# rasd3/TODA

Hardware: AMD Instinct MI355X
Metric: LiDAR training samples/sec (higher is better)
Workload: dtype f32

## Files before the change

include/toda.h:

```cpp
#ifndef TODA_H_
#define TODA_H_

#include <stddef.h>
#include <stdint.h>

#ifdef __cplusplus
extern "C" {
#endif

#define TODA_OK 0
#define TODA_EINVAL (-1)
#define TODA_EWORKSPACE (-2)
#define TODA_ELAUNCH (-3)
#define TODA_EFAULT (-4)

#define TODA_FAULT_BN2D 1u
#define TODA_FAULT_WINO 2u
#define TODA_FAULT_FPS 4u

const char* toda_last_error(void);
int toda_abi_version(void);
int toda_device_fault(void);

size_t toda_voxelize_workspace_bytes(int n_points, int max_voxels);
int toda_voxelize_hard(const float* points, int n, int c,
                       const float* range_host ,
                       const float* vsize_host ,
                       const int32_t* grid_host ,
                       int max_pts, int max_voxels,
                       float* voxels, int32_t* coords_zyx, int32_t* num_pts,
                       int32_t* m_dev, void* ws, size_t ws_bytes, void* stream);
size_t toda_voxelize_batch_workspace_bytes(int batch, int n_cap);
int toda_voxelize_batch(const float* const* points_host, const int32_t* n_points_host, int batch, int n_cap,
                        int c, int row_stride,
                        const float* range_host, const float* vsize_host, const int32_t* grid_host,
                        int max_pts, int max_voxels,
                        float* voxels, int32_t* coords_bzyx, int32_t* num_pts, int32_t* counts_dev,
                        void* ws, size_t ws_bytes, int ws_clean, void* stream);

int toda_mean_vfe_fwd(const float* voxels, const float* num_pts, int m, int p, int c,
                      float* out, void* stream);
int toda_mean_vfe_bwd(const float* grad_out, const float* num_pts, int m, int p, int c,
                      float* grad_voxels, void* stream);

size_t toda_dynvox_workspace_bytes(int n, int batch, const int32_t* grid_host, int pillar);
int toda_dynvox_count(const float* points, int n, int width, int batch, const float* range_host, const float* vsize_host,
                      const int32_t* grid_host, int pillar, int32_t* counts_dev, void* ws, size_t ws_bytes, void* stream);
int toda_dynvox_index(const float* points, int n, int width, int batch, const float* range_host, const float* vsize_host,
                      const int32_t* grid_host, int pillar, int m, int k, uint8_t* keep, int32_t* rows, int32_t* inv,
                      int32_t* seg_pts, int32_t* seg_off, int32_t* cnt, int32_t* coords, void* ws, size_t ws_bytes,
                      void* stream);
int toda_dynvox_seg_sum(const float* src, int ld, int col0, int ncol, const int32_t* rowmap, const int32_t* seg_off,
                        const int32_t* seg_pts, int m, int divide, float* out, void* stream);
int toda_dynvox_pillar_decorate(const float* points, int width, const int32_t* rows, const int32_t* inv,
                                const int32_t* coords, const float* mean, int k, const float* vsize_host,
                                const float* offset_host, int use_abs_xyz, int with_dist, float* out, int f, void* stream);
int toda_dynvox_seg_max_fwd(const float* x, int c, const int32_t* seg_off, const int32_t* seg_pts, int m, float* out,
                            int32_t* arg, void* stream);
int toda_dynvox_seg_max_bwd(const float* gout, const int32_t* arg, int m, int c, int k, float* gx, void* stream);
int toda_dynvox_gather_concat(const float* x, const float* xmax, const int32_t* inv, int k, int c, float* out, void* stream);

size_t toda_gridindex_bytes(int batch, const int32_t* shape_host );
int toda_gridindex_from_coords(const int32_t* idx, int n, const int32_t* n_dev,
                               int batch, const int32_t* shape_host,
                               void* gi, int32_t* rowof, void* stream);
int toda_gridindex_from_coords_unordered(const int32_t* idx, int n, const int32_t* n_dev,
                                         int batch, const int32_t* shape_host,
                                         void* gi, int32_t* rowof, int gi_clean, void* stream);
int toda_gridindex_clear(const int32_t* idx, int n, const int32_t* n_dev, int batch,
                         const int32_t* shape_host, void* gi, void* stream);
int toda_gridindex_from_conv(const int32_t* idx_in, int n_in, const int32_t* n_in_dev,
                             int batch, const int32_t* shape_in_host,
                             const int32_t* ksize_host, const int32_t* stride_host,
                             const int32_t* pad_host, const int32_t* shape_out_host,
                             void* gi_out, int32_t* idx_out, int32_t* n_out_dev,
                             int out_cap, void* stream);
int toda_gridindex_from_bitmap(const void* gi_in, int batch, const int32_t* shape_in_host,
                               const int32_t* ksize_host, const int32_t* stride_host,
                               const int32_t* pad_host, const int32_t* shape_out_host,
                               void* gi_out, int32_t* idx_out, int32_t* n_out_dev,
                               int out_cap, int in_rows_marked, void* stream);

int toda_rulebook_subm(const int32_t* idx, int n, int batch, const int32_t* shape_host,
                       const int32_t* ksize_host, const int32_t* dilation_host,
                       const void* gi, const int32_t* rowof,
                       int32_t* nbr, int32_t* pair_cnt, int cnt_zeroed, void* stream);
int toda_rulebook_conv(const int32_t* idx_in, int n_in, int batch,
                       const int32_t* shape_in_host, const int32_t* ksize_host,
                       const int32_t* stride_host, const int32_t* pad_host,
                       const int32_t* shape_out_host, const void* gi_out, int n_out,
                       int32_t* nbr_o2i, int32_t* nbr_i2o, int32_t* pair_cnt,
                       const int32_t* idx_out, const void* gi_in, const int32_t* rowof_in,
                       int cnt_zeroed, void* stream);

size_t toda_spconv_packed_weight_floats(int k_vol, int c_gather, int c_produce);
int toda_matrix_path(void);
int toda_set_matrix_path(int mode);
int toda_spconv_split_supported(int c_gather, int c_produce);
int toda_spconv_pack_weight(const float* w, int cout, int k_vol, int cin,
                            int transpose, int flip_k, float* wp, void* stream);
int toda_spconv_pack_weights(int n, const float* const* w_host, const int32_t* cout_host, const int32_t* k_vol_host,
                             const int32_t* cin_host, const int32_t* transpose_host, const int32_t* flip_k_host,
                             float* const* wp_host, void* stream);
int toda_spconv_gather_gemm(const float* in, int n_in, int c_gather, const float* wp,
                            const int32_t* nbr, int n_out, int k_vol, int c_produce,
                            const float* bias , float* out, void* stream);
int toda_spconv_gather_gemm_ordered(const float* in, int n_in, int c_gather, const float* wp,
                                    const int32_t* nbr, int n_out, int k_vol, int c_produce,
                                    const float* bias, float* out, const int32_t* order, void* stream);

int toda_rulebook_class_order(const int32_t* in_coords, int n_in, const int32_t* stride_host, const int32_t* padding_host,
                              int32_t* order, unsigned char* cls_sorted, void* stream);
int toda_spconv_gather_gemm_classed(const float* in, int n_in, int c_gather, const float* wp, const int32_t* nbr, int n_out,
                                    int k_vol, int c_produce, const float* bias, float* out, const int32_t* order,
                                    const unsigned char* cls_sorted, const int32_t* ksize_host, const int32_t* stride_host,
                                    const int32_t* padding_host, void* stream);
int toda_spconv_gather_gemm_compact_supported(int c_gather, int c_produce, int k_vol);
int toda_spconv_gather_gemm_compact(const float* in, int n_in, int c_gather, const float* w, int w_cout, int w_cin,
                                    int transpose, int flip_k, const int32_t* nbr, int n_out, int k_vol, int c_produce,
                                    const float* bias , float* out, void* stream);
size_t toda_spconv_gather_gemm_compact_stats_doubles(int n_out, int c_produce);
int toda_spconv_gather_gemm_compact_stats(const float* in, int n_in, int c_gather, const float* w, int w_cout, int w_cin,
                                          int transpose, int flip_k, const int32_t* nbr, int n_out, int k_vol,
                                          int c_produce, const float* bias , float* out, double* sums,
                                          size_t sums_doubles, int* blocks_out , void* stream);

size_t toda_spconv_wgrad_workspace_bytes(int n_out, int k_vol, int cin, int cout);
int toda_spconv_wgrad(const float* in, int n_in, const float* dout, const int32_t* nbr,
                      int n_out, int k_vol, int cin, int cout, float* dw,
                      void* ws, size_t ws_bytes, void* stream);
int toda_sparse_to_dense_fwd(const float* feat, const int32_t* idx, int n, int c,
                             int batch, const int32_t* shape_host, float* dense, void* stream);
int toda_sparse_to_dense_bwd(const float* grad_dense, const int32_t* idx, int n, int c,
                             int batch, const int32_t* shape_host, float* grad_feat, void* stream);

int toda_pillar_scatter_fwd(const float* feat, const int32_t* idx, int n, int c,
                            int batch, int ny, int nx, float* canvas, void* stream);
int toda_pillar_scatter_bwd(const float* grad_canvas, const int32_t* idx, int n, int c,
                            int batch, int ny, int nx, float* grad_feat, void* stream);

size_t toda_rows_reduce_doubles(int n, int c);
int toda_rows_moments(const float* x, int n, int c, double* sums ,
                      void* stream);
int toda_rows_affine_act(const float* x, const float* scale, const float* shift,
                         const float* residual , int n, int c, int relu,
                         float* y, void* stream);

int toda_bn_finalize(const double* sums , int n, int c,
                     const float* gamma, const float* beta, float* running_mean ,
                     float* running_var , float momentum, float eps, int training,
                     float* mean, float* invstd, float* scale, float* shift, void* stream);
int toda_bn_finalize_partials(double* sums, int blocks, int n, int c, const float* gamma, const float* beta,
                              float* running_mean , float* running_var , float momentum, float eps,
                              float* mean, float* invstd, float* scale, float* shift, void* stream);
int toda_rows_bn_bwd(const float* dy, const float* x, const float* stats, const float* gamma,
                     int n, int c, int relu, double* sums , float* dx,
                     void* stream);

int toda_rows_bn_bwd_res(const float* dy, const float* x, const float* residual , const float* stats,
                         const float* gamma, int n, int c, int relu, double* sums, float* dx,
                         float* dres , void* stream);
size_t toda_rows_bn_bwd_colsum_doubles(int n, int c);
int toda_rows_bn_bwd_res_colsum(const float* dy, const float* x, const float* residual , const float* stats,
                                const float* gamma, int n, int c, int relu, double* sums, float* dx,
                                float* dres , double* colsum_ws , float* dx_colsum ,
                                void* stream);

int toda_bn2d_supported(int batch, int c, int hw);
size_t toda_bn2d_sync_bytes(void);
int toda_bn2d_fwd(const float* x, int batch, int c, int hw, const float* gamma, const float* beta,
                  float* running_mean , float* running_var , float momentum, float eps, int relu,
                  float* y, float* save, void* sync , unsigned epoch, void* stream);
int toda_bn2d_bwd(const float* x, const float* dy, int batch, int c, int hw, const float* gamma, const float* beta,
                  const float* save, int relu, float* dx, float* dgamma, float* dbeta, void* sync ,
                  unsigned epoch, void* stream);
int toda_bn2d_fwd_into(const float* x, int batch, int c, int hw, const float* gamma, const float* beta,
                       float* running_mean , float* running_var , float momentum, float eps, int relu,
                       float* y, int y_channels, int y_channel0, float* save, void* sync , unsigned epoch,
                       void* stream);
int toda_bn2d_bwd_from(const float* x, const float* dy, int dy_channels, int dy_channel0, int batch, int c, int hw,
                       const float* gamma, const float* beta, const float* save, int relu, float* dx, float* dgamma,
                       float* dbeta, void* sync , unsigned epoch, void* stream);

int toda_center_assign(const float* gt_boxes, int batch, int n_gt, int code_size,
                       int num_classes, int fm_w, int fm_h,
                       const float* range_host , const float* vsize_host ,
                       int fm_stride, int max_objs, double gaussian_overlap, int min_radius,
                       float* heatmap ,
                       float* ret_boxes ,
                       int64_t* inds , int64_t* mask ,
                       void* stream);

size_t toda_anchor_assign_workspace_bytes(int batch, int n_gt);
int toda_anchor_assign(const void* const* anchors_host, const int32_t* locs_host, const int32_t* per_loc_host,
                       const float* matched_host, const float* unmatched_host, int n_classes, int anchor_stride,
                       const float* gt_boxes, int batch, int n_gt, int gt_stride, const int32_t* slot_of, int n_ids,
                       int code_size, int encode_angle_by_sincos, int multihead_order,
                       int32_t* labels , float* targets , float* weights ,
                       void* ws, size_t ws_bytes, void* stream);

int toda_boxes_iou_bev(const float* boxes_a, int na, const float* boxes_b, int nb,
                       float* iou , void* stream);
int toda_boxes_overlap_bev(const float* boxes_a, int na, const float* boxes_b, int nb,
                           float* overlap , void* stream);
size_t toda_nms_workspace_bytes(int n);
int toda_nms_rotated(const float* boxes_sorted, int n, float thresh, int64_t* keep ,
                     int32_t* n_keep_dev, void* ws, size_t ws_bytes, void* stream);

int toda_roi_grid_pool_bev(const float* feat, int B, int C, int H, int W, const float* rois, int N, int roi_stride,
                           float min_x, float min_y, float step_x, float step_y, int grid_size, float* out, void* stream);
int toda_roi_iou3d_max(const float* rois, int B, int N, int roi_stride, const int64_t* roi_labels, const float* gt, int M,
                       int gt_stride, int by_class, float* max_iou , int64_t* argmax , void* stream);

int toda_voxel_query(const float* new_xyz, const int32_t* new_coords, int M, const float* xyz, int N, const void* gi, const int32_t* rowof,
                     int batch, const int32_t* shape_host, float radius, const int32_t* ranges_host, int nsample, int32_t* idx,
                     uint8_t* empty, void* stream);
size_t toda_voxel_pool_moments_doubles(void);
int toda_voxel_pool_moments(const int32_t* idx, const uint8_t* empty, int M, int nsample, const float* xyz, int N, const float* new_xyz,
                            double* ws, void* stream);
int toda_voxel_pool_fwd(const float* f, int N, int C, const int32_t* idx, const uint8_t* empty, int M, int nsample, const float* xyz,
                        const float* new_xyz, const float* ab, float* out, uint8_t* arg, void* stream);
size_t toda_voxel_pool_table_bytes(int M, int nsample, int N);
int toda_voxel_pool_table(const int32_t* idx, const uint8_t* empty, int M, int nsample, int N, int32_t* off, int32_t* ent, void* ws,
                          size_t ws_bytes, void* stream);
int toda_voxel_pool_bwd_feat(const float* gout, const uint8_t* arg, int M, int nsample, int C, const int32_t* off, const int32_t* ent,
                             int N, float* gf, void* stream);
size_t toda_voxel_pool_bwd_pos_doubles(int C);
int toda_voxel_pool_bwd_pos(const float* gout, const uint8_t* arg, const int32_t* idx, const uint8_t* empty, int M, int nsample, int C,
                            const float* xyz, int N, const float* new_xyz, double* ws, float* gab, void* stream);

int toda_fps_resident_blocks(void);
size_t toda_fps_workspace_bytes(int batch, int npoint);
int toda_fps(const float* xyz, const int32_t* starts_host, int batch, int npoint, int mode, float* temp, int32_t* idx, void* ws,
             size_t ws_bytes, void* stream);
int toda_ball_query_stack(const float* xyz, int N, const int32_t* xyz_start, const float* new_xyz, const int32_t* new_start, int batch,
                          int M, int nr, const float* radii_host, const int32_t* nsample_host, int32_t* const* idx_host,
                          uint8_t* const* empty_host, void* stream);
int toda_sa_gather_fwd(const float* P, int N, int C, const float* wd, const int32_t* idx, const uint8_t* empty, int M, int nsample,
                       const float* xyz, const float* new_xyz, float* z, void* stream);
int toda_sa_gather_bwd_feat(const float* gz, int M, int nsample, int C, const int32_t* off, const int32_t* ent, int N, float* gP,
                            void* stream);
size_t toda_sa_gather_bwd_pos_doubles(int C);
int toda_sa_gather_bwd_pos(const float* gz, const int32_t* idx, const uint8_t* empty, int M, int nsample, int C, const float* xyz, int N,
                           const float* new_xyz, double* ws, float* gwd, void* stream);
int toda_sa_max_fwd(const float* y, int M, int nsample, int C, float* out, uint8_t* arg, void* stream);
int toda_sa_max_bwd(const float* g, const uint8_t* arg, int M, int nsample, int C, float* gy, void* stream);
int toda_bev_interp_fwd(const float* map, int B, int C, int H, int W, const float* xy, const int32_t* bidx, int K, float* out,
                        int32_t* taps, float* wts, void* stream);
int toda_bev_interp_bwd(const float* g, int K, int C, const int32_t* off, const int32_t* ent, const float* wts, int B, int H, int W,
                        float* gmap, void* stream);

int toda_points_in_boxes(const float* points, int n, const int32_t* n_dev, int c, const float* boxes,
                         int k, int box_stride, int mode, int32_t* flags, void* stream);
int toda_points_sector(const float* points, int n, const int32_t* n_dev, int c, double lo, double hi,
                       int32_t* flags, void* stream);
int toda_points_rect(const float* points, int n, const int32_t* n_dev, int c, const double* lo_xy_host,
                     const double* hi_xy_host, int closed, int32_t* flags, void* stream);
int toda_points_polar_cell(const float* points, int n, const int32_t* n_dev, int c, float phase,
                           const double* yaw_edges_host, int n_yaw, const double* dis_edges_host, int n_dis,
                           float dis_lo, float dis_hi, int32_t* cell, void* stream);
int toda_points_polar_select(const float* points, int n, const int32_t* n_dev, int c, double lo, double hi, int yaw_mode,
                             int dis_mode, double dis_th, const float* pitch_range_dev, int32_t* flags, void* stream);
size_t toda_points_pitch_range_workspace_bytes(void);
int toda_points_pitch_range(const float* points, int n, const int32_t* n_dev, int c, float* range_dev, void* ws,
                            size_t ws_bytes, void* stream);
int toda_points_pitch_band(const float* points, int n, const int32_t* n_dev, int c, float z_offset, float clip_lo,
                           float clip_hi, const double* edges_host, int n_bands, int32_t* band, void* stream);
size_t toda_rows_select_workspace_bytes(int n);
int toda_rows_select_append(const float* src, int n, const int32_t* n_dev, int c, const int32_t* keys,
                            int match, int invert, float* dst, int cap_rows, int32_t* cursor_dev,
                            void* ws, size_t ws_bytes, void* stream);
int toda_points_rotate_z(const float* src, int n, const int32_t* n_dev, int c, double cosv, double sinv,
                         float* dst, void* stream);
int toda_points_world_transform(const float* src, int n, const int32_t* n_dev, int c, int flip_x, int flip_y,
                                int rotate, float cosv, float sinv, int rescale, float scale, float* dst,
                                void* stream);

int toda_points_box_steps_chunk(void);
int toda_points_box_steps(const float* src, int n, const int32_t* n_dev, int c, const double* steps, int n_steps,
                          float* dst, int32_t* keep, void* stream);
size_t toda_points_column_range_workspace_bytes(void);
int toda_points_column_range(const float* points, int n, const int32_t* n_dev, int c, int col, float* range_dev,
                             void* ws, size_t ws_bytes, void* stream);
int toda_points_in_pyramids(const float* points, int n, const int32_t* n_dev, int c, const double* pyramids, int np,
                            uint32_t* bits, int32_t* counts, void* stream);

int toda_points_fov_flags(const float* points, int n, const int32_t* n_dev, int c, const float* m_host,
                          const float* p2_host, int img_h, int img_w, int32_t* flags, void* stream);

int toda_sweeps_merge_max_sweeps(void);
int toda_sweeps_merge(const float* rows, int n, int n_sweeps, const int32_t* offsets_host, const double* matrices_host,
                      const int32_t* has_matrix_host, const int32_t* drop_ego_host, const double* time_lags_host,
                      float radius, const float* shift_host, float* out, int32_t* flags, void* stream);

int toda_waymo_frame(const float* rows, int n, int c_in, int use_nlz, float* out, int32_t* flags, void* stream);

int toda_adv_edit_max_boxes(void);
int toda_adv_edit_chunk(void);
size_t toda_adv_edit_workspace_bytes(int n, int k);
int toda_adv_edit(const float* points, int n, int c, const double* table_host, const double* table_dev, int k,
                  const int64_t* keys, const float* grads, int m, const float* range_lo_host, const float* voxel_host,
                  const int32_t* grid_host, float eps, float* dst, int cap_rows, int32_t* cursor_dev, int32_t* counts,
                  void* ws, size_t ws_bytes, void* stream);

int toda_spconv_gather_gemm_stats_supported(int c_gather, int c_produce);
size_t toda_spconv_gather_gemm_stats_doubles(int n_out, int c_produce);
int toda_spconv_gather_gemm_stats(const float* in, int n_in, int c_gather, const float* packed_w, const int32_t* nbr,
                                  int n_out, int k_vol, int c_produce, const float* bias, float* out, double* sums,
                                  size_t sums_doubles, void* stream);
int toda_spconv_gather_gemm_stats_partials(const float* in, int n_in, int c_gather, const float* wp, const int32_t* nbr,
                                           int n_out, int k_vol, int c_produce, const float* bias , float* out,
                                           double* sums, size_t sums_doubles, int* blocks_out, void* stream);

int toda_conv3x3_supported(int batch, int cin, int cout, int H, int W);
size_t toda_conv3x3_weight_floats(int cout, int cin);
int toda_conv3x3_transform_weight(const float* w, int cout, int cin, int mode, float* u, void* stream);
typedef struct toda_conv3x3_weight_entry {
    const float* w;
    int32_t cout, cin, mode, reserved;
    float* u;
} toda_conv3x3_weight_entry;
int toda_conv3x3_transform_weight_batch(const toda_conv3x3_weight_entry* table_host, int n, void* stream);
size_t toda_conv3x3_workspace_bytes(void);
size_t toda_conv3x3_wgrad_workspace_bytes(int batch, int cin, int cout, int H, int W);
int toda_conv3x3_wgrad(const float* x, const float* dy, int batch, int cin, int cout, int H, int W, float* dw,
                       void* ws, size_t ws_bytes, void* stream);
int toda_conv3x3_fwd(const float* x, const float* u, const float* bias, int batch, int cin, int cout, int H,
                     int W, float* y, void* ws, size_t ws_bytes, void* stream);

int toda_conv3x3s2_supported(int batch, int cin, int cout, int H, int W);
int toda_conv3x3s2_fwd(const float* x, const float* w, int batch, int cin, int cout, int H, int W, float* y, void* stream);
int toda_conv3x3s2_dgrad(const float* dy, const float* w, int batch, int cin, int cout, int H, int W, float* dx, void* stream);
size_t toda_conv3x3s2_wgrad_workspace_bytes(int batch, int cin, int cout, int H, int W);
int toda_conv3x3s2_wgrad(const float* x, const float* dy, int batch, int cin, int cout, int H, int W, float* dw, void* ws,
                         size_t ws_bytes, void* stream);
int toda_deconv_supported(int batch, int cin, int cout, int H, int W, int s);
int toda_deconv_fwd(const float* x, const float* w, int batch, int cin, int cout, int H, int W, int s, float* y, void* stream);
int toda_deconv_dgrad(const float* dy, const float* w, int batch, int cin, int cout, int H, int W, int s, float* dx, void* stream);
size_t toda_deconv_wgrad_workspace_bytes(int batch, int cin, int cout, int H, int W, int s);
int toda_deconv_wgrad(const float* x, const float* dy, int batch, int cin, int cout, int H, int W, int s, float* dw, void* ws,
                      size_t ws_bytes, void* stream);

size_t toda_center_loss_workspace_bytes(int batch, int classes, int H, int W, int max_objs, int code_size);
int toda_center_loss_fwd(const float* hm_logits, const float* heatmap, int batch, int classes, int H, int W, int n_branch,
                         const float* const* reg_maps_host, const int32_t* reg_channels_host, const int64_t* inds,
                         const int64_t* mask, const float* target_boxes, int max_objs, int code_size,
                         const float* code_weights_host, float cls_weight, float loc_weight, float* hm_prob, float* out4,
                         void* ws, size_t ws_bytes, void* stream);
int toda_center_loss_bwd(const float* out4, const float* up_hm, const float* up_loc, int batch, int classes, int H, int W,
                         int n_branch, float* const* reg_grads_host, const int32_t* reg_channels_host, const int64_t* inds,
                         const int64_t* mask, int max_objs, int code_size, const float* code_weights_host, float cls_weight, float loc_weight,
                         float* hm_grad, const void* ws, size_t ws_bytes, void* stream);

int toda_conv3x3_narrow_supported(int batch, int cin, int cout, int H, int W);
int toda_conv3x3_narrow_fwd(int n, const float* const* x_host, const float* const* w_host, const float* const* bias_host,
                            const int32_t* cout_host, int batch, int cin, int H, int W, long long x_image_stride,
                            float* const* y_host, void* stream);
int toda_conv3x3_narrow_dgrad(int n, const float* const* dy_host, const float* const* w_host, const int32_t* cout_host,
                              int batch, int cin, int H, int W, long long dx_image_stride, float* const* dx_host, void* stream);
size_t toda_conv3x3_narrow_wgrad_workspace_bytes(int n, int batch, int cin, int H);
int toda_conv3x3_narrow_wgrad(int n, const float* const* x_host, const float* const* dy_host, const int32_t* cout_host,
                              int batch, int cin, int H, int W, long long x_image_stride, float* out, void* ws, size_t ws_bytes,
                              void* stream);

int toda_timing_begin(int capacity);
int toda_timing_end(float* ms_out_host, int cap, int* n_out_host);

int toda_clip_adam_chunk(void);
int toda_clip_adam_step(const unsigned long long* param, const unsigned long long* grad, const unsigned long long* exp_avg,
                        const unsigned long long* exp_avg_sq, const long long* numel, const int* chunk_tensor,
                        const long long* chunk_off, int n_chunks, double* partial, float* norm_out, float max_norm,
                        float lr, float beta1, float beta2, float eps, float weight_decay, int step, void* stream);

int toda_eval_overlaps(const float* box3d, const float* bbox, const int32_t* box_off, const float* query3d,
                       const float* query_bbox, const int32_t* query_off, const long long* out_off, int n_frames,
                       long long n_pairs, int metric, int criterion, float* out, void* stream);
size_t toda_eval_match_workspace_bytes(int n_frames, int n_thresh, int n_det_total);
int toda_eval_match_scores(const float* overlaps, const long long* ov_off, const int32_t* det_off, const int32_t* gt_off,
                           const int32_t* ign_det, const int32_t* ign_gt, const double* det_score, int n_frames,
                           int n_det_total, double min_overlap, double* scores_out, int32_t* count_out, void* ws,
                           size_t ws_bytes, void* stream);
int toda_eval_match(const float* overlaps, const long long* ov_off, const int32_t* det_off, const int32_t* gt_off,
                    const int32_t* ign_det, const int32_t* ign_gt, const double* det_score, const double* det_alpha,
                    const double* gt_alpha, const double* det_bbox, const double* dc_bbox, const int32_t* dc_off, int n_frames,
                    int n_det_total, const double* thresholds, int n_thresh, double min_overlap, int metric, int compute_aos,
                    double* pr, void* ws, size_t ws_bytes, void* stream);

#define TODA_NUSC_MAX_PRED 500
#define TODA_NUSC_MAX_GT 2048
int toda_nusc_eval_prepare(const double* rows, const int32_t* sample, const int32_t* cls, int n, const double* G,
                           const double* ego, int n_samples, double* out, int32_t* keep, void* stream);
size_t toda_nusc_eval_match_workspace_bytes(int n_seg);
int toda_nusc_eval_match(const double* pred, const double* pred_score, const int32_t* pred_attr, int n_pred, const double* gt,
                         const int32_t* gt_attr, int n_gt, const int32_t* pred_off_host, const int32_t* gt_off_host,
                         const int32_t* seg_cls_host, int n_seg, const double* thresholds_host, int tp_threshold,
                         int32_t* match, double* err, void* ws, size_t ws_bytes, void* stream);

#define TODA_WAYMO_MAX_PRED 512
#define TODA_WAYMO_MAX_GT 512
#define TODA_WAYMO_CUTOFFS 101
size_t toda_waymo_eval_match_workspace_bytes(int n_seg);
int toda_waymo_eval_iou(const double* pred, int n_pred, const double* gt, int n_gt, const int32_t* pred_off_host,
                        const int32_t* gt_off_host, const long long* iou_off_host, int n_seg, long long n_pairs, double* iou,
                        void* ws, size_t ws_bytes, void* stream);
int toda_waymo_eval_match(const double* iou, const float* pred_score, const double* pred_heading, int n_pred,
                          const double* gt_heading, const int32_t* gt_level, int n_gt, const int32_t* pred_off_host,
                          const int32_t* gt_off_host, const long long* iou_off_host, const int32_t* seg_type_host, int n_seg,
                          long long n_pairs, const float* cutoffs_host, long long* tp, long long* fn, long long* fp,
                          double* sum_ha, int32_t* match_dbg, void* ws, size_t ws_bytes, void* stream);

size_t toda_consistency_workspace_bytes(int batch, int na, int no);
int toda_consistency_loss(const float* adv, const uint8_t* adv_sel, int na, const float* org, const uint8_t* org_sel, int no,
                          int batch, int cols, float match_dist2, float* out, void* ws, size_t ws_bytes, void* stream);

#ifdef __cplusplus
}
#endif
#endif
```

toda_amd/csrc/bn_fold.cuh:

```cuda
#pragma once
#include "common.h"

namespace toda {

constexpr int DN_BLOCK = 256;

__device__ __forceinline__ double fold_column(const double* __restrict__ src, int blocks, double* part) {
    double acc = 0.0;
    for (int g = threadIdx.x; g < blocks; g += DN_BLOCK) acc += src[g];
    part[threadIdx.x] = acc;
    __syncthreads();
    for (int w = DN_BLOCK / 2; w > 0; w >>= 1) {
        if (threadIdx.x < w) part[threadIdx.x] += part[threadIdx.x + w];
        __syncthreads();
    }
    return part[0];
}

__device__ __forceinline__ void bn_write_channel(int ch, float mean, float var, float eps, const float* __restrict__ gamma,
                                                 const float* __restrict__ beta, float* __restrict__ mean_out,
                                                 float* __restrict__ invstd_out, float* __restrict__ scale_out,
                                                 float* __restrict__ shift_out) {
    const float invstd = 1.0f / sqrtf(var + eps);
    const float g = gamma ? gamma[ch] : 1.0f, b = beta ? beta[ch] : 0.0f;
    mean_out[ch] = mean;
    invstd_out[ch] = invstd;
    scale_out[ch] = g * invstd;
    shift_out[ch] = b - mean * g * invstd;
}

__device__ __forceinline__ void bn_train_channel(int ch, double sum, double sumsq, int n, const float* __restrict__ gamma,
                                                 const float* __restrict__ beta, float* __restrict__ running_mean,
                                                 float* __restrict__ running_var, float momentum, float eps,
                                                 float* __restrict__ mean_out, float* __restrict__ invstd_out,
                                                 float* __restrict__ scale_out, float* __restrict__ shift_out) {
    const double m = sum / (double)n;
    double v = sumsq / (double)n - m * m;
    if (v < 0.0) v = 0.0;
    const float mean = (float)m, var = (float)v;
    if (running_mean) {
        const double unbiased = n > 1 ? v * (double)n / (double)(n - 1) : v;
        running_mean[ch] = (1.0f - momentum) * running_mean[ch] + momentum * mean;
        running_var[ch] = (1.0f - momentum) * running_var[ch] + momentum * (float)unbiased;
    }
    bn_write_channel(ch, mean, var, eps, gamma, beta, mean_out, invstd_out, scale_out, shift_out);
}

__global__ void __launch_bounds__(DN_BLOCK) fold_partials_kernel(double* __restrict__ sums, int blocks, int cols);

}
```

toda_amd/csrc/dense.hip:

```cpp
#include "bn_fold.cuh"
#include "common.h"

namespace toda {

typedef float f32x4 __attribute__((ext_vector_type(4)));

constexpr int DN_ROWS = 64;
constexpr int DN_CH = 32;

struct DenseGeom {
    int D, H, W;
    int pillar;
};

__device__ __forceinline__ long long spatial_offset(const int4 q, const DenseGeom& g) {
    if (g.pillar) return (long long)q.y + (long long)q.z * g.W + q.w;
    return ((long long)q.y * g.H + q.z) * g.W + q.w;
}

template <bool FWD>
__global__ void __launch_bounds__(DN_BLOCK)
dense_tile_kernel(float* __restrict__ feat, const int4* __restrict__ idx, int n, int c, DenseGeom g,
                  float* __restrict__ dense) {
    __shared__ float tile[DN_CH][DN_ROWS + 1];
// ... 5 lines not shown
        long long b = -1;
        if (r < n) {
            const int4 q = idx[r];
            b = (long long)q.x * c * vol + spatial_offset(q, g);
        }
        base[threadIdx.x] = b;
    }
    const int fr = threadIdx.x >> 2, fc = (threadIdx.x & 3) * 8;
    const int dr = threadIdx.x & 63, dc = threadIdx.x >> 6;
    if (FWD) {
        if (row0 + fr < n) {
#pragma unroll
            for (int j = 0; j < 8; ++j) {
                const int ch = c0 + fc + j;
                tile[fc + j][fr] = ch < c ? feat[(size_t)(row0 + fr) * c + ch] : 0.f;
            }
        }
        __syncthreads();
        const long long b = base[dr];
        if (b >= 0) {
#pragma unroll
            for (int j = 0; j < DN_CH / 4; ++j) {
                const int ch = dc + 4 * j;
                if (c0 + ch < c) dense[b + (long long)(c0 + ch) * vol] = tile[ch][dr];
            }
        }
    } else {
        __syncthreads();
        const long long b = base[dr];
#pragma unroll
        for (int j = 0; j < DN_CH / 4; ++j) {
            const int ch = dc + 4 * j;
            tile[ch][dr] = (b >= 0 && c0 + ch < c) ? dense[b + (long long)(c0 + ch) * vol] : 0.f;
        }
        __syncthreads();
        if (row0 + fr < n) {
#pragma unroll
            for (int j = 0; j < 8; ++j) {
                const int ch = c0 + fc + j;
                if (ch < c) feat[(size_t)(row0 + fr) * c + ch] = tile[fc + j][fr];
            }
        }
    }
}

#ifndef TODA_MOM_ROWS
#define TODA_MOM_ROWS 256
#endif
constexpr int MOM_ROWS = TODA_MOM_ROWS;
constexpr int MOM_MAX_BLOCKS = 2048;

template <class Load>
__device__ __forceinline__ void rows_reduce2(int n, int c, int rows_per_block, Load load, double* __restrict__ sums) {
    __shared__ float sh[2][DN_BLOCK][4];
    const int lanes = c >> 2;
    const int rows_par = DN_BLOCK / lanes;
    const int cl = threadIdx.x % lanes, rsub = threadIdx.x / lanes;
    const int row_begin = blockIdx.x * rows_per_block;
    const int row_end = min(n, row_begin + rows_per_block);
    f32x4 s0 = f32x4{0.f, 0.f, 0.f, 0.f}, t0 = s0, s1 = s0, t1 = s0;
    int r = row_begin + rsub;
    for (; r + rows_par < row_end; r += 2 * rows_par) {
        f32x4 a, b, a2, b2;
        load(r, cl, a, b);
        load(r + rows_par, cl, a2, b2);
        s0 += a;
        t0 += b;
        s1 += a2;
        t1 += b2;
    }
    if (r < row_end) {
        f32x4 a, b;
        load(r, cl, a, b);
        s0 += a;
        t0 += b;
    }
    s0 += s1;
    t0 += t1;
#pragma unroll
    for (int j = 0; j < 4; ++j) {
        sh[0][threadIdx.x][j] = s0[j];
        sh[1][threadIdx.x][j] = t0[j];
    }
    __syncthreads();
    if (threadIdx.x < 2 * c) {
        const int q = threadIdx.x / c, ch = threadIdx.x % c;
        double acc = 0.0;
        for (int j = 0; j < rows_par; ++j) acc += sh[q][j * lanes + (ch >> 2)][ch & 3];
        sums[2 * c + (size_t)(q * c + ch) * gridDim.x + blockIdx.x] = acc;
    }
}

__global__ void __launch_bounds__(DN_BLOCK)
fold_partials_kernel(double* __restrict__ sums, int blocks, int cols) {
    __shared__ double part[DN_BLOCK];
    const double total = fold_column(sums + cols + (size_t)blockIdx.x * blocks, blocks, part);
    if (threadIdx.x == 0) sums[blockIdx.x] = total;
}

static inline void reduce_plan(int n, int* blocks, int* rows_per_block) {
    const int g = cdiv(n > 0 ? n : 1, MOM_ROWS);
    *blocks = g < MOM_MAX_BLOCKS ? g : MOM_MAX_BLOCKS;
    *rows_per_block = cdiv(n > 0 ? n : 1, *blocks);
}

__global__ void __launch_bounds__(DN_BLOCK)
rows_moments_kernel(const float* __restrict__ x, int n, int c, int rows_per_block, double* __restrict__ sums) {
    const f32x4* x4 = reinterpret_cast<const f32x4*>(x);
    const int lanes = c >> 2;
    rows_reduce2(n, c, rows_per_block, [&](int r, int cl, f32x4& a, f32x4& b) {
        a = x4[(size_t)r * lanes + cl];
        b = a * a;
    }, sums);
}

constexpr int EW_BLOCKS = 2048;

__global__ void __launch_bounds__(DN_BLOCK)
rows_affine_act_kernel(const f32x4* __restrict__ x, const float* __restrict__ scale, const float* __restrict__ shift,
                       const f32x4* __restrict__ res, long long n4, int c, int relu, f32x4* __restrict__ y) {
    const long long t0 = (long long)blockIdx.x * DN_BLOCK + threadIdx.x;
    const long long stride = (long long)gridDim.x * DN_BLOCK;
    const int ch = (int)((t0 * 4) % c);
    const f32x4 sc = *reinterpret_cast<const f32x4*>(scale + ch), sf = *reinterpret_cast<const f32x4*>(shift + ch);
    for (long long t = t0; t < n4; t += stride) {
        f32x4 v = x[t] * sc + sf;
        if (res) v += res[t];
        if (relu) {
#pragma unroll
            for (int j = 0; j < 4; ++j) v[j] = fmaxf(v[j], 0.f);
        }
        y[t] = v;
    }
}

__global__ void __launch_bounds__(DN_BLOCK)
rows_bn_bwd_reduce_kernel(const float* __restrict__ dy, const float* __restrict__ x, const float* __restrict__ res,
                          const float* __restrict__ stats, int n, int c, int relu, int rows_per_block,
                          double* __restrict__ sums) {
    const f32x4* dy4 = reinterpret_cast<const f32x4*>(dy);
    const f32x4* x4 = reinterpret_cast<const f32x4*>(x);
    const f32x4* r4 = reinterpret_cast<const f32x4*>(res);
    const int lanes = c >> 2;
    const int cl0 = threadIdx.x % lanes;
    const f32x4 mu = reinterpret_cast<const f32x4*>(stats)[cl0];
    const f32x4 is = reinterpret_cast<const f32x4*>(stats + c)[cl0];
    const f32x4 sc = reinterpret_cast<const f32x4*>(stats + 2 * c)[cl0];
    const f32x4 sf = reinterpret_cast<const f32x4*>(stats + 3 * c)[cl0];
    rows_reduce2(n, c, rows_per_block, [&](int r, int cl, f32x4& a, f32x4& b) {
        const f32x4 g = dy4[(size_t)r * lanes + cl], xv = x4[(size_t)r * lanes + cl];
        const f32x4 rv = r4 ? r4[(size_t)r * lanes + cl] : f32x4{0.f, 0.f, 0.f, 0.f};
#pragma unroll
        for (int j = 0; j < 4; ++j) {
            float pre = xv[j] * sc[j] + sf[j];
            if (r4) pre += rv[j];
            const float dz = (relu && !(pre > 0.f)) ? 0.f : g[j];
            a[j] = dz;
            b[j] = dz * ((xv[j] - mu[j]) * is[j]);
        }
    }, sums);
}

__global__ void __launch_bounds__(DN_BLOCK)
rows_bn_bwd_apply_kernel(const f32x4* __restrict__ dy, const f32x4* __restrict__ x, const f32x4* __restrict__ res,
                         const float* __restrict__ stats, const float* __restrict__ gamma, double* __restrict__ sums,
                         long long n4, int c, int n, int relu, f32x4* __restrict__ dx, f32x4* __restrict__ dres,
                         double* __restrict__ colsum_part) {
    if (blockIdx.x == 0 && threadIdx.x < 2 * c) reinterpret_cast<float*>(sums + 2 * c)[threadIdx.x] = (float)sums[threadIdx.x];
    const long long t0 = (long long)blockIdx.x * DN_BLOCK + threadIdx.x;
    const long long stride = (long long)gridDim.x * DN_BLOCK;
    const int ch = (int)((t0 * 4) % c);
    const float inv_n = 1.0f / (float)n;
    const f32x4 mu = *reinterpret_cast<const f32x4*>(stats + ch);
    const f32x4 is = *reinterpret_cast<const f32x4*>(stats + c + ch);
    const f32x4 sc = *reinterpret_cast<const f32x4*>(stats + 2 * c + ch);
    const f32x4 sf = *reinterpret_cast<const f32x4*>(stats + 3 * c + ch);
    const f32x4 ga = *reinterpret_cast<const f32x4*>(gamma + ch);
    f32x4 m1, m2;
#pragma unroll
    for (int j = 0; j < 4; ++j) {
        m1[j] = (float)(sums[ch + j] * (double)inv_n);
        m2[j] = (float)(sums[c + ch + j] * (double)inv_n);
    }
    const f32x4 k1 = ga * is, k2 = is * m2;
    f32x4 csum = {0.f, 0.f, 0.f, 0.f};
    for (long long t = t0; t < n4; t += stride) {
        const f32x4 g = dy[t], xv = x[t];
        const f32x4 rv = res ? res[t] : f32x4{0.f, 0.f, 0.f, 0.f};
        f32x4 out, dzv;
#pragma unroll
        for (int j = 0; j < 4; ++j) {
            float pre = xv[j] * sc[j] + sf[j];
            if (res) pre += rv[j];
            const float dz = (relu && !(pre > 0.f)) ? 0.f : g[j];
            dzv[j] = dz;
            out[j] = k1[j] * (dz - m1[j] - (xv[j] - mu[j]) * k2[j]);
        }
        dx[t] = out;
        csum += out;
        if (dres) dres[t] = dzv;
    }
    if (colsum_part) {
        __shared__ float cs[DN_BLOCK][4];
#pragma unroll
        for (int j = 0; j < 4; ++j) cs[threadIdx.x][j] = csum[j];
        __syncthreads();
        if (threadIdx.x < c) {
            const int lanes = c >> 2, cl = threadIdx.x >> 2, j = threadIdx.x & 3;
            double acc = 0.0;
            for (int t = cl; t < DN_BLOCK; t += lanes) acc += (double)cs[t][j];
            colsum_part[(size_t)threadIdx.x * gridDim.x + blockIdx.x] = acc;
        }
    }
}

__global__ void __launch_bounds__(DN_BLOCK)
colsum_fold_kernel(const double* __restrict__ part, int blocks, float* __restrict__ out) {
    __shared__ double sh[DN_BLOCK];
    const double total = fold_column(part + (size_t)blockIdx.x * blocks, blocks, sh);
    if (threadIdx.x == 0) out[blockIdx.x] = (float)total;
}

__global__ void __launch_bounds__(DN_BLOCK)
bn_finalize_kernel(const double* __restrict__ sums, int n, int c, const float* __restrict__ gamma,
                   const float* __restrict__ beta, float* __restrict__ running_mean, float* __restrict__ running_var,
                   float momentum, float eps, int training, float* __restrict__ mean_out, float* __restrict__ invstd_out,
                   float* __restrict__ scale_out, float* __restrict__ shift_out) {
    const int ch = threadIdx.x;
    if (ch >= c) return;
    if (training)
        bn_train_channel(ch, sums[ch], sums[c + ch], n, gamma, beta, running_mean, running_var, momentum, eps, mean_out, invstd_out,
                         scale_out, shift_out);
    else
        bn_write_channel(ch, running_mean[ch], running_var[ch], eps, gamma, beta, mean_out, invstd_out, scale_out, shift_out);
}

__global__ void __launch_bounds__(DN_BLOCK)
bn_fold_finalize_kernel(double* __restrict__ sums, int blocks, int n, int c, const float* __restrict__ gamma,
                        const float* __restrict__ beta, float* __restrict__ running_mean, float* __restrict__ running_var,
                        float momentum, float eps, float* __restrict__ mean_out, float* __restrict__ invstd_out,
                        float* __restrict__ scale_out, float* __restrict__ shift_out) {
    __shared__ double part[DN_BLOCK];
    const int ch = blockIdx.x;
    const double sum = fold_column(sums + 2 * c + (size_t)ch * blocks, blocks, part);
    __syncthreads();
    const double sumsq = fold_column(sums + 2 * c + (size_t)(c + ch) * blocks, blocks, part);
    if (threadIdx.x != 0) return;
    sums[ch] = sum;
    sums[c + ch] = sumsq;
    bn_train_channel(ch, sum, sumsq, n, gamma, beta, running_mean, running_var, momentum, eps, mean_out, invstd_out, scale_out,
                     shift_out);
}

static int ew_grid(long long n4, int c) {
    long long blocks = (n4 + DN_BLOCK - 1) / DN_BLOCK;
    if (blocks > EW_BLOCKS) blocks = EW_BLOCKS;
    while ((blocks * DN_BLOCK * 4) % c != 0) ++blocks;
    return (int)blocks;
}

static int scatter_common(bool fwd, float* feat, const int32_t* idx, int n, int c, int batch, DenseGeom g,
                          float* dense, hipStream_t s) {
    TODA_CHECK_ARG(n >= 0 && c >= 1 && batch >= 1, "sparse<->dense: bad sizes n=%d c=%d batch=%d", n, c, batch);
    const size_t total = (size_t)batch * c * g.D * g.H * g.W;
    if (fwd) TODA_HIP(hipMemsetAsync(dense, 0, total * sizeof(float), s));
    if (n == 0) return TODA_OK;
    const dim3 grid(cdiv(n, DN_ROWS), cdiv(c, DN_CH));
    if (fwd)
        hipLaunchKernelGGL(HIP_KERNEL_NAME(dense_tile_kernel<true>), grid, dim3(DN_BLOCK), 0, s, feat, (const int4*)idx, n,
                           c, g, dense);
    else
        hipLaunchKernelGGL(HIP_KERNEL_NAME(dense_tile_kernel<false>), grid, dim3(DN_BLOCK), 0, s, feat, (const int4*)idx, n,
                           c, g, dense);
    TODA_LAUNCH_CHECK();
    return TODA_OK;
}

}

using namespace toda;

extern "C" int toda_sparse_to_dense_fwd(const float* feat, const int32_t* idx, int n, int c, int batch,
                                        const int32_t* shape_host, float* dense, void* stream) {
    const DenseGeom g{shape_host[0], shape_host[1], shape_host[2], 0};
    return scatter_common(true, const_cast<float*>(feat), idx, n, c, batch, g, dense, (hipStream_t)stream);
}
extern "C" int toda_sparse_to_dense_bwd(const float* grad_dense, const int32_t* idx, int n, int c, int batch,
                                        const int32_t* shape_host, float* grad_feat, void* stream) {
    const DenseGeom g{shape_host[0], shape_host[1], shape_host[2], 0};
    return scatter_common(false, grad_feat, idx, n, c, batch, g, const_cast<float*>(grad_dense), (hipStream_t)stream);
}
extern "C" int toda_pillar_scatter_fwd(const float* feat, const int32_t* idx, int n, int c, int batch, int ny, int nx,
                                       float* canvas, void* stream) {
    const DenseGeom g{1, ny, nx, 1};
    return scatter_common(true, const_cast<float*>(feat), idx, n, c, batch, g, canvas, (hipStream_t)stream);
}
extern "C" int toda_pillar_scatter_bwd(const float* grad_canvas, const int32_t* idx, int n, int c, int batch, int ny,
                                       int nx, float* grad_feat, void* stream) {
    const DenseGeom g{1, ny, nx, 1};
    return scatter_common(false, grad_feat, idx, n, c, batch, g, const_cast<float*>(grad_canvas), (hipStream_t)stream);
}

extern "C" size_t toda_rows_reduce_doubles(int n, int c) {
    int blocks, rpb;
    reduce_plan(n, &blocks, &rpb);
    return (size_t)2 * c * (1 + (size_t)blocks);
}

extern "C" int toda_rows_moments(const float* x, int n, int c, double* sums, void* stream) {
    hipStream_t s = (hipStream_t)stream;
    TODA_CHECK_ARG(c >= 4 && c % 4 == 0 && c <= DN_BLOCK / 2 && DN_BLOCK % c == 0,
                   "rows_moments: channels must be a multiple of 4 dividing 256, <= 128 (got %d)", c);
    if (n <= 0) {
        TODA_HIP(hipMemsetAsync(sums, 0, 2 * c * sizeof(double), s));
        return TODA_OK;
    }
    int blocks, rpb;
    reduce_plan(n, &blocks, &rpb);
    hipLaunchKernelGGL(rows_moments_kernel, dim3(blocks), dim3(DN_BLOCK), 0, s, x, n, c, rpb, sums);
    hipLaunchKernelGGL(fold_partials_kernel, dim3(2 * c), dim3(DN_BLOCK), 0, s, sums, blocks, 2 * c);
    TODA_LAUNCH_CHECK();
    return TODA_OK;
}

extern "C" int toda_rows_affine_act(const float* x, const float* scale, const float* shift, const float* residual,
                                    int n, int c, int relu, float* y, void* stream) {
    TODA_CHECK_ARG(c >= 4 && c % 4 == 0 && c <= 1024, "rows_affine_act: channels must be a multiple of 4, <= 1024 (got %d)", c);
    if (n <= 0) return TODA_OK;
    const long long n4 = (long long)n * c / 4;
    hipLaunchKernelGGL(rows_affine_act_kernel, dim3(ew_grid(n4, c)), dim3(DN_BLOCK), 0, (hipStream_t)stream,
                       (const f32x4*)x, scale, shift, (const f32x4*)residual, n4, c, relu, (f32x4*)y);
    TODA_LAUNCH_CHECK();
    return TODA_OK;
}

extern "C" size_t toda_rows_bn_bwd_colsum_doubles(int n, int c) {
    if (n <= 0 || c < 4) return 1;
    return (size_t)c * ew_grid((long long)n * c / 4, c);
}

extern "C" int toda_rows_bn_bwd_res_colsum(const float* dy, const float* x, const float* residual, const float* stats,
                                           const float* gamma, int n, int c, int relu, double* sums, float* dx, float* dres,
                                           double* colsum_ws, float* dx_colsum, void* stream) {
    hipStream_t s = (hipStream_t)stream;
    TODA_CHECK_ARG((colsum_ws == nullptr) == (dx_colsum == nullptr), "rows_bn_bwd: colsum workspace and result go together");
    TODA_CHECK_ARG(c >= 4 && c % 4 == 0 && c <= DN_BLOCK / 2 && DN_BLOCK % c == 0,
                   "rows_bn_bwd: channels must be a multiple of 4 dividing 256, <= 128 (got %d)", c);
    if (n <= 0) {
        TODA_HIP(hipMemsetAsync(sums, 0, 3 * c * sizeof(double), s));
        if (dx_colsum) TODA_HIP(hipMemsetAsync(dx_colsum, 0, c * sizeof(float), s));
        return TODA_OK;
    }
    int blocks, rpb;
    reduce_plan(n, &blocks, &rpb);
    hipLaunchKernelGGL(rows_bn_bwd_reduce_kernel, dim3(blocks), dim3(DN_BLOCK), 0, s, dy, x, residual, stats, n, c, relu, rpb, sums);
    hipLaunchKernelGGL(fold_partials_kernel, dim3(2 * c), dim3(DN_BLOCK), 0, s, sums, blocks, 2 * c);
    const long long n4 = (long long)n * c / 4;
    const int grid = ew_grid(n4, c);
    hipLaunchKernelGGL(rows_bn_bwd_apply_kernel, dim3(grid), dim3(DN_BLOCK), 0, s, (const f32x4*)dy,
                       (const f32x4*)x, (const f32x4*)residual, stats, gamma, sums, n4, c, n, relu, (f32x4*)dx, (f32x4*)dres, colsum_ws);
    if (dx_colsum) hipLaunchKernelGGL(colsum_fold_kernel, dim3(c), dim3(DN_BLOCK), 0, s, (const double*)colsum_ws, grid, dx_colsum);
    TODA_LAUNCH_CHECK();
    return TODA_OK;
}

extern "C" int toda_rows_bn_bwd_res(const float* dy, const float* x, const float* residual, const float* stats,
                                    const float* gamma, int n, int c, int relu, double* sums, float* dx, float* dres,
                                    void* stream) {
    return toda_rows_bn_bwd_res_colsum(dy, x, residual, stats, gamma, n, c, relu, sums, dx, dres, nullptr, nullptr, stream);
}

extern "C" int toda_rows_bn_bwd(const float* dy, const float* x, const float* stats, const float* gamma, int n, int c,
                                int relu, double* sums, float* dx, void* stream) {
    return toda_rows_bn_bwd_res(dy, x, nullptr, stats, gamma, n, c, relu, sums, dx, nullptr, stream);
}

extern "C" int toda_bn_finalize_partials(double* sums, int blocks, int n, int c, const float* gamma, const float* beta,
                                         float* running_mean, float* running_var, float momentum, float eps, float* mean,
                                         float* invstd, float* scale, float* shift, void* stream) {
    TODA_CHECK_ARG(sums && mean && invstd && scale && shift, "bn_finalize_partials: null argument");
    TODA_CHECK_ARG(c >= 1 && c <= DN_BLOCK && blocks >= 1 && n >= 1, "bn_finalize_partials: channels must be <= 256, blocks and rows >= 1 (got %d, %d, %d)", c,
                   blocks, n);
    TODA_CHECK_ARG((running_mean == nullptr) == (running_var == nullptr), "bn_finalize_partials: running_mean and running_var go together");
    hipLaunchKernelGGL(bn_fold_finalize_kernel, dim3(c), dim3(DN_BLOCK), 0, (hipStream_t)stream, sums, blocks, n, c, gamma, beta, running_mean,
                       running_var, momentum, eps, mean, invstd, scale, shift);
    TODA_LAUNCH_CHECK();
    return TODA_OK;
}

extern "C" int toda_bn_finalize(const double* sums, int n, int c, const float* gamma, const float* beta,
                                float* running_mean, float* running_var, float momentum, float eps, int training,
                                float* mean, float* invstd, float* scale, float* shift, void* stream) {
    TODA_CHECK_ARG(c >= 1 && c <= DN_BLOCK, "bn_finalize: channels must be <= 256 (got %d)", c);
    TODA_CHECK_ARG(training || (running_mean && running_var), "bn_finalize: eval mode needs running statistics");
    TODA_CHECK_ARG(!training || n >= 1, "bn_finalize: training mode needs rows >= 1 (got %d)", n);
    hipLaunchKernelGGL(bn_finalize_kernel, dim3(1), dim3(DN_BLOCK), 0, (hipStream_t)stream, sums, n, c, gamma, beta,
                       running_mean, running_var, momentum, eps, training, mean, invstd, scale, shift);
    TODA_LAUNCH_CHECK();
    return TODA_OK;
}
```

toda_amd/csrc/spconv.hip:

```cpp
#include <stdlib.h>

#include <type_traits>

#include <hip/hip_ext.h>

#include <mutex>
#include <vector>

#include "bn_fold.cuh"
#include "common.h"


namespace toda {

typedef float f32x4 __attribute__((ext_vector_type(4)));

constexpr int SC_BLOCK = 256;

static int tiles_pow2(int channels) {
    int t = (channels + 15) / 16, p = 1;
    while (p < t) p <<= 1;
    return p;
}

// ... 24 lines not shown
}

constexpr int PACK_MAX_SEG = 48;
struct PackBatch {
    const float* w[PACK_MAX_SEG];
    float* wp[PACK_MAX_SEG];
    int cout[PACK_MAX_SEG], K[PACK_MAX_SEG], cin[PACK_MAX_SEG];
    unsigned char transpose[PACK_MAX_SEG], flip[PACK_MAX_SEG], Q[PACK_MAX_SEG], NT[PACK_MAX_SEG];
};

__global__ void __launch_bounds__(SC_BLOCK)
pack_weight_batch_kernel(const PackBatch b) {
    const int sg = blockIdx.y;
    const int K = b.K[sg], Q = b.Q[sg], NT = b.NT[sg], cin = b.cin[sg], cout = b.cout[sg];
    const long long e = (long long)blockIdx.x * SC_BLOCK + threadIdx.x;
    if (e >= (long long)K * Q * NT * 256) return;
    const int j = (int)(e & 3);
    const int lane = (int)((e >> 2) & 63);
    long long t = e >> 8;
    const int n = (int)(t % NT);
    t /= NT;
    const int q = (int)(t % Q);
    const int k = (int)(t / Q);
    const int c = lane & 15, g = lane >> 4;
    const int gch = 16 * q + 4 * g + j, pch = NT * c + n;
    const int kk = b.flip[sg] ? K - 1 - k : k;
    const float* __restrict__ w = b.w[sg];
    float v = 0.0f;
    if (!b.transpose[sg]) {
        if (gch < cin && pch < cout) v = w[((size_t)pch * K + kk) * cin + gch];
    } else {
        if (gch < cout && pch < cin) v = w[((size_t)gch * K + kk) * cin + pch];
    }
    b.wp[sg][e] = v;
}

typedef unsigned int u32x4 __attribute__((ext_vector_type(4)));
typedef int i32x4 __attribute__((ext_vector_type(4)));

__device__ __forceinline__ __amdgpu_buffer_rsrc_t table_rsrc(const float* base, unsigned bytes) {
    return __builtin_amdgcn_make_buffer_rsrc(const_cast<float*>(base), 0, bytes, 0x00020000);
}
constexpr unsigned OOB = 0xFFFFFFF0u;

template <int Q, int RT, bool VEC>
__device__ __forceinline__ void gather_rows(__amdgpu_buffer_rsrc_t rsrc, int cg, int g, const int (&src)[RT],
                                            f32x4 (&a)[RT][Q]) {
#pragma unroll
    for (int rt = 0; rt < RT; ++rt) {
        const unsigned row_off = (unsigned)src[rt] * (unsigned)cg * 4u;
#pragma unroll
        for (int q = 0; q < Q; ++q) {
            const int col = 16 * q + 4 * g;
            const bool ok = src[rt] >= 0 && col < cg;
            const unsigned off = row_off + (unsigned)col * 4u;
            f32x4 v;
            if constexpr (VEC) {
                v = __builtin_bit_cast(f32x4, __builtin_amdgcn_raw_buffer_load_b128(rsrc, ok ? off : OOB, 0, 0));
            } else {
#pragma unroll
                for (int j = 0; j < 4; ++j)
                    v[j] = __builtin_bit_cast(float, __builtin_amdgcn_raw_buffer_load_b32(
                                                         rsrc, (ok && col + j < cg) ? off + 4u * j : OOB, 0, 0));
            }
            a[rt][q] = v;
        }
    }
}

template <int RT, int NT>
__device__ __forceinline__ void gg_prologue(const float* bias, int cp, int row0, int n_out, const int* order, int r,
                                            f32x4 (&acc)[RT][NT], int (&rows)[RT], bool (&live)[RT]) {
#pragma unroll
    for (int n = 0; n < NT; ++n) {
        float b = 0.0f;
        if (bias && NT * r + n < cp) b = bias[NT * r + n];
#pragma unroll
        for (int rt = 0; rt < RT; ++rt) acc[rt][n] = f32x4{b, b, b, b};
    }
#pragma unroll
    for (int rt = 0; rt < RT; ++rt) {
        live[rt] = row0 + rt * 16 + r < n_out;
        rows[rt] = live[rt] ? (order ? order[row0 + rt * 16 + r] : row0 + rt * 16 + r) : n_out - 1;
    }
}

template <int RT, int NT>
__device__ __forceinline__ void gg_store_rows(const f32x4 (&acc)[RT][NT], const int (&rows)[RT], int row0, int n_out, int cp,
                                              float* out, int r, int g) {
    const bool full = cp == 16 * NT;
#pragma unroll
    for (int rt = 0; rt < RT; ++rt) {
#pragma unroll
        for (int reg = 0; reg < 4; ++reg) {
            const int pos = row0 + rt * 16 + 4 * g + reg;
            const int row = __shfl(rows[rt], 4 * g + reg, 64);
            if (pos >= n_out) continue;
            float* dst = out + (size_t)row * cp + NT * r;
            if (full) {
                if constexpr (NT == 1) {
                    dst[0] = acc[rt][0][reg];
                } else if constexpr (NT == 2) {
                    *reinterpret_cast<float2*>(dst) = make_float2(acc[rt][0][reg], acc[rt][1][reg]);
                } else {
#pragma unroll
                    for (int n = 0; n < NT; n += 4)
                        *reinterpret_cast<f32x4*>(dst + n) =
                            f32x4{acc[rt][n][reg], acc[rt][n + 1][reg], acc[rt][n + 2][reg], acc[rt][n + 3][reg]};
                }
            } else {
#pragma unroll
                for (int n = 0; n < NT; ++n)
                    if (NT * r + n < cp) dst[n] = acc[rt][n][reg];
            }
        }
    }
}

template <int NT, int RT, int WAVES>
__device__ __forceinline__ void gg_moments(float (*st_sh)[2][16 * NT], int wv, int blk, const f32x4 (&acc)[RT][NT], int row0, int n_out,
                                           int cp, double* stats, int r, int g) {
    float sm[NT], sq[NT];
#pragma unroll
    for (int n = 0; n < NT; ++n) {
        sm[n] = sq[n] = 0.0f;
#pragma unroll
        for (int rt = 0; rt < RT; ++rt)
#pragma unroll
            for (int reg = 0; reg < 4; ++reg)
                if (row0 + rt * 16 + 4 * g + reg < n_out) {
                    const float v = acc[rt][n][reg];
                    sm[n] += v;
                    sq[n] += v * v;
                }
        sm[n] += __shfl_xor(sm[n], 16, 64);
        sq[n] += __shfl_xor(sq[n], 16, 64);
        sm[n] += __shfl_xor(sm[n], 32, 64);
        sq[n] += __shfl_xor(sq[n], 32, 64);
        if (g == 0) {
            st_sh[wv][0][NT * r + n] = sm[n];
            st_sh[wv][1][NT * r + n] = sq[n];
        }
    }
    __syncthreads();
    if ((int)threadIdx.x < 2 * cp) {
        const int qq = threadIdx.x / cp, ch = threadIdx.x - qq * cp;
        double a = 0.0;
#pragma unroll
        for (int w = 0; w < WAVES; ++w) a += (double)st_sh[w][qq][ch];
        stats[2 * cp + (size_t)(qq * cp + ch) * gridDim.x + blk] = a;
    }
}

__device__ __forceinline__ void wg_block(int K, int& chunk, int& k) {
    const int b = blockIdx.x;
    const int xcd = b & 7, t = (b >> 3) / K;
    k = (b >> 3) - t * K;
    chunk = t * 8 + xcd;
}

template <int ROUND, class FullTag, class Round>
__device__ __forceinline__ void wg_pair_walk(int* qi, int* qo, int base0, int row_end, int bstep, const int* nbr_k, int n_out,
                                             unsigned row_a, unsigned row_b, int lane, FullTag full_tag, Round&& round) {
    int qn = 0;
    int iv_next = nbr_k[min(base0 + lane, n_out - 1)];
    for (int base = base0; base < row_end; base += bstep) {
        const int o = base + lane;
        const int iv = iv_next;
        iv_next = nbr_k[min(o + bstep, n_out - 1)];
        const int i = o < row_end ? iv : -1;
        const unsigned long long vote = __ballot(i >= 0);
        if (vote == 0) continue;
        if (i >= 0) {
            const int pos = qn + __popcll(vote & ((1ull << lane) - 1));
            qi[pos] = (int)((unsigned)i * row_a);
            qo[pos] = (int)((unsigned)o * row_b);
        }
        qn += __popcll(vote);
        __builtin_amdgcn_wave_barrier();
        int done = 0;
        while (qn - done >= ROUND) {
            round(done, qn, full_tag);
            done += ROUND;
        }
        const int left = qn - done;
        if (done > 0 && left > 0) {
            int ti = 0, to = 0;
            if (lane < left) {
                ti = qi[done + lane];
                to = qo[done + lane];
            }
            __builtin_amdgcn_wave_barrier();
            if (lane < left) {
                qi[lane] = ti;
                qo[lane] = to;
            }
        }
        qn = left;
        __builtin_amdgcn_wave_barrier();
    }
    if (qn > 0) round(0, qn, std::false_type{});
}

template <bool BOUND, int MTB, int NTB>
__device__ __forceinline__ void wg_store_slab(const f32x4 (&acc)[MTB][NTB], float* slab, int chunk, int k, int K, int MT, int NT,
                                              int m0, int n0, int cin, int cout, int ii, int g) {
    float* dst = slab + (size_t)chunk * cout * K * cin;
#pragma unroll
    for (int m = 0; m < MTB; ++m)
#pragma unroll
        for (int n = 0; n < NTB; ++n)
#pragma unroll
            for (int reg = 0; reg < 4; ++reg) {
                const int ci = MT * (4 * g + reg) + m0 + m;
                const int co = NT * ii + n0 + n;
                if (!BOUND || (ci < cin && co < cout)) dst[((size_t)co * K + k) * cin + ci] = acc[m][n][reg];
            }
}

struct GatherClasses {
    unsigned char count[8];
    unsigned char k[8][27];
};

template <int Q, int NT, int RT, bool VEC, bool CLS = false>
__global__ void __launch_bounds__(SC_BLOCK)
gather_gemm_kernel(const float* __restrict__ in, int n_in, int cg, const float* __restrict__ wp,
                   const int* __restrict__ nbr, int n_out, int K, int cp, const float* __restrict__ bias,
                   float* __restrict__ out, const int* __restrict__ order,
                   const unsigned char* __restrict__ cls_sorted, const GatherClasses classes) {
    const int lane = threadIdx.x & 63;
    const int wave = (int)blockIdx.x * (SC_BLOCK / 64) + (threadIdx.x >> 6);
    const int r = lane & 15, g = lane >> 4;
    const int row0 = wave * (16 * RT);
    if (row0 >= n_out) return;

    f32x4 acc[RT][NT];
#pragma unroll
    for (int n = 0; n < NT; ++n) {
        float b = 0.0f;
        if (bias && NT * r + n < cp) b = bias[NT * r + n];
#pragma unroll
        for (int rt = 0; rt < RT; ++rt) acc[rt][n] = f32x4{b, b, b, b};
    }
    const f32x4* __restrict__ wp4 = reinterpret_cast<const f32x4*>(wp);
    const __amdgpu_buffer_rsrc_t in_rsrc = table_rsrc(in, (unsigned)n_in * (unsigned)cg * 4u);
    int rows[RT];
    bool live[RT];
#pragma unroll
    for (int rt = 0; rt < RT; ++rt) {
        live[rt] = row0 + rt * 16 + r < n_out;
        rows[rt] = live[rt] ? (order ? order[row0 + rt * 16 + r] : row0 + rt * 16 + r) : n_out - 1;
    }

    auto load_ids = [&](int k, int (&dst)[RT]) {
        const int kk = k < K ? k : K - 1;
#pragma unroll
        for (int rt = 0; rt < RT; ++rt) {
            const int v = nbr[(size_t)kk * n_out + rows[rt]];
            dst[rt] = (k < K && live[rt]) ? v : -1;
        }
    };
    auto mma_masked = [&](auto mask_tag, int k, const f32x4 (&a)[RT][Q]) {
        constexpr unsigned MASK = decltype(mask_tag)::value;
#pragma unroll
        for (int q = 0; q < Q; ++q) {
            f32x4 b[NT];
#pragma unroll
            for (int n = 0; n < NT; ++n) b[n] = wp4[(((size_t)k * Q + q) * NT + n) * 64 + lane];
#pragma unroll
            for (int j = 0; j < 4; ++j) {
#pragma unroll
                for (int n = 0; n < NT; ++n) {
#pragma unroll
                    for (int rt = 0; rt < RT; ++rt) {
                        if ((MASK >> rt) & 1u)
                            acc[rt][n] = __builtin_amdgcn_mfma_f32_16x16x4f32(a[rt][q][j], b[n][j], acc[rt][n], 0, 0, 0);
                    }
                }
            }
        }
    };
    auto mma = [&](int k, const f32x4 (&a)[RT][Q], const bool (&hit)[RT]) {
        if constexpr (RT == 1) {
            mma_masked(std::integral_constant<unsigned, 1u>{}, k, a);
        } else if constexpr (RT == 2) {
            if (hit[0] && hit[1]) mma_masked(std::integral_constant<unsigned, 3u>{}, k, a);
            else if (hit[0]) mma_masked(std::integral_constant<unsigned, 1u>{}, k, a);
            else mma_masked(std::integral_constant<unsigned, 2u>{}, k, a);
        } else {
            mma_masked(std::integral_constant<unsigned, (1u << RT) - 1u>{}, k, a);
        }
    };

    auto offset = [&](int k) {
        int src[RT];
        load_ids(k, src);
        bool hit[RT];
        bool any = false;
#pragma unroll
        for (int rt = 0; rt < RT; ++rt) {
            hit[rt] = __any(src[rt] >= 0);
            any = any || hit[rt];
        }
        if (!any) return;
        f32x4 a[RT][Q];
        gather_rows<Q, RT, VEC>(in_rsrc, cg, g, src, a);
        mma(k, a, hit);
    };
    const unsigned char* klist = nullptr;
    int n_k = 0;
    if constexpr (CLS) {
        const int p = row0 + (lane & (16 * RT - 1) & 63);
        const int c = cls_sorted[p < n_out ? p : n_out - 1];
        const int c0 = __builtin_amdgcn_readfirstlane(c);
        if (__all(c == c0 || p >= n_out) && classes.count[c0 & 7] > 0) {
            klist = classes.k[c0 & 7];
            n_k = classes.count[c0 & 7];
        }
    }
    if (CLS && klist) {
        for (int t = 0; t < n_k; ++t) offset(klist[t]);
    } else {
        for (int k = 0; k < K; ++k) offset(k);
    }
    gg_store_rows<RT, NT>(acc, rows, row0, n_out, cp, out, r, g);
}

#ifndef GG_XCD_CHUNK
#define GG_XCD_CHUNK 32
#endif
__device__ __forceinline__ int xcd_chunked_block(int b, int nblk) {
    constexpr int C = GG_XCD_CHUNK;
    if (C <= 0) return b;
    const int per = 8 * C, full = (nblk / per) * per;
    if (b >= full) return b;
    const int xcd = b & 7, local = b >> 3;
    return ((local / C) * 8 + xcd) * C + local % C;
}

#ifndef GG_LDS_WAVES_WIDE
#define GG_LDS_WAVES_WIDE 4
#endif
#ifndef GG_LDS_WAVES_NARROW
#define GG_LDS_WAVES_NARROW 4
#endif
#ifndef GG_LDS_WAVES
#define GG_LDS_WAVES 4
#endif
template <int Q, int NT, int RT, bool VEC, bool DB = true, int BLK = SC_BLOCK, bool IDPF = false>
__global__ void __launch_bounds__(BLK, (Q * NT <= 4 && RT <= 2) ? GG_LDS_WAVES_NARROW : (Q * NT * RT <= 32 && Q * NT <= 16) ? GG_LDS_WAVES : (BLK > SC_BLOCK ? GG_LDS_WAVES_WIDE : 1))
gather_gemm_lds_kernel(const float* __restrict__ in, int n_in, int cg, const float* __restrict__ wp,
                       const int* __restrict__ nbr, int n_out, int K, int cp, const float* __restrict__ bias,
                       float* __restrict__ out, const int* __restrict__ order, double* __restrict__ stats) {
    constexpr int SLICE = Q * NT * 64;
    constexpr int PER_THREAD = (SLICE + BLK - 1) / BLK;
    __shared__ f32x4 wl[DB ? 2 : 1][SLICE];
    const int lane = threadIdx.x & 63;
    const int blk = xcd_chunked_block(blockIdx.x, gridDim.x);
    const int wave = blk * (BLK / 64) + (threadIdx.x >> 6);
    const int r = lane & 15, g = lane >> 4;
    const int row0 = wave * (16 * RT);
    const f32x4* __restrict__ wp4 = reinterpret_cast<const f32x4*>(wp);

    f32x4 acc[RT][NT];
    int rows[RT];
    bool live[RT];
    gg_prologue<RT, NT>(bias, cp, row0, n_out, order, r, acc, rows, live);
    const __amdgpu_buffer_rsrc_t in_rsrc = table_rsrc(in, (unsigned)n_in * (unsigned)cg * 4u);

#pragma unroll
    for (int t = 0; t < PER_THREAD; ++t) {
        const int e = t * BLK + threadIdx.x;
        if (e < SLICE) wl[0][e] = wp4[e];
    }
    __syncthreads();
    int id_next[RT];
    if constexpr (IDPF) {
#pragma unroll
        for (int rt = 0; rt < RT; ++rt) id_next[rt] = __builtin_nontemporal_load(nbr + rows[rt]);
    }
    for (int k = 0; k < K; ++k) {
        const int cur = DB ? (k & 1) : 0;
        int src[RT];
        if constexpr (IDPF) {
            const int kn = k + 1 < K ? k + 1 : K - 1;
#pragma unroll
            for (int rt = 0; rt < RT; ++rt) {
                src[rt] = live[rt] ? id_next[rt] : -1;
                id_next[rt] = __builtin_nontemporal_load(nbr + (size_t)kn * n_out + rows[rt]);
            }
        } else {
#pragma unroll
            for (int rt = 0; rt < RT; ++rt) {
                const int v = __builtin_nontemporal_load(nbr + (size_t)k * n_out + rows[rt]);
                src[rt] = live[rt] ? v : -1;
            }
        }
        asm volatile("" ::: "memory");
        f32x4 stage[PER_THREAD];
        {
            const int kn = k + 1 < K ? k + 1 : K - 1;
#pragma unroll
            for (int t = 0; t < PER_THREAD; ++t) {
                const int e = t * BLK + threadIdx.x;
                if (SLICE % BLK == 0 || e < SLICE) stage[t] = wp4[(size_t)kn * SLICE + e];
            }
        }
        bool hit[RT];
        bool any = false;
#pragma unroll
        for (int rt = 0; rt < RT; ++rt) {
            hit[rt] = __any(src[rt] >= 0);
            any = any || hit[rt];
        }
        if (any) {
            f32x4 a[RT][Q];
            gather_rows<Q, RT, VEC>(in_rsrc, cg, g, src, a);
#pragma unroll
            for (int q = 0; q < Q; ++q) {
                f32x4 b[NT];
#pragma unroll
                for (int n = 0; n < NT; ++n) b[n] = wl[cur][(q * NT + n) * 64 + lane];
#pragma unroll
                for (int j = 0; j < 4; ++j) {
#pragma unroll
                    for (int n = 0; n < NT; ++n) {
#pragma unroll
                        for (int rt = 0; rt < RT; ++rt) {
                            if (hit[rt])
                                acc[rt][n] = __builtin_amdgcn_mfma_f32_16x16x4f32(a[rt][q][j], b[n][j], acc[rt][n], 0, 0, 0);
                        }
                    }
                }
            }
        }
        if (!DB) __syncthreads();
        if (k + 1 < K) {
#pragma unroll
            for (int t = 0; t < PER_THREAD; ++t) {
                const int e = t * BLK + threadIdx.x;
                if (e < SLICE) wl[DB ? (cur ^ 1) : 0][e] = stage[t];
            }
        }
        __syncthreads();
    }
    if (row0 >= n_out && !stats) return;

    if (stats) {
        __shared__ float st_sh[BLK / 64][2][16 * NT];
        gg_moments<NT, RT, BLK / 64>(st_sh, threadIdx.x >> 6, blk, acc, row0, n_out, cp, stats, r, g);
    }
    gg_store_rows<RT, NT>(acc, rows, row0, n_out, cp, out, r, g);
}

#ifndef WG_WAVES
#define WG_WAVES 4
#endif
typedef float f32x2w __attribute__((ext_vector_type(2)));
template <int MTB, int NTB, bool COOP = false, bool EXACT = false>
__global__ void __launch_bounds__(SC_BLOCK, (MTB * NTB <= 16) ? WG_WAVES : 1)
wgrad_kernel(const float* __restrict__ in, int n_in, int cin, const float* __restrict__ dout, int cout,
             const int* __restrict__ nbr, int n_out, int K, int rows_per_chunk, int MT, int NT, float* __restrict__ slab) {
    constexpr int QCAP = 64 + 16;
    constexpr bool STAGE_A = EXACT && !COOP && MTB < 4, STAGE_B = EXACT && !COOP && NTB < 4;
    __shared__ float red[MTB * NTB * 4 * 64];
    __shared__ __attribute__((aligned(16))) float stage[(STAGE_A || STAGE_B) ? SC_BLOCK / 64 : 1][(STAGE_A || STAGE_B) ? 1024 : 4];
    __shared__ int q_in[SC_BLOCK / 64][QCAP], q_out[SC_BLOCK / 64][QCAP];
    const int lane = threadIdx.x & 63, wv = threadIdx.x >> 6;
    const int ii = lane & 15, g = lane >> 4;
    int chunk, k;
    wg_block(K, chunk, k);
    const int m0 = COOP ? (wv / 2) * MTB : 0, n0 = COOP ? (wv % 2) * NTB : 0;
    const int row_begin = chunk * rows_per_chunk;
    if (row_begin >= n_out) return;
    const int row_end = min(n_out, row_begin + rows_per_chunk);
    const bool exact_a = cin == 16 * MT, exact_b = cout == 16 * NT;
    int* qi = q_in[wv];
    int* qo = q_out[wv];

    f32x4 acc[MTB][NTB];
#pragma unroll
    for (int m = 0; m < MTB; ++m)
#pragma unroll
        for (int n = 0; n < NTB; ++n) acc[m][n] = f32x4{0.f, 0.f, 0.f, 0.f};

    const __amdgpu_buffer_rsrc_t in_rsrc = table_rsrc(in, (unsigned)n_in * (unsigned)cin * 4u);
    const __amdgpu_buffer_rsrc_t dout_rsrc = table_rsrc(dout, (unsigned)n_out * (unsigned)cout * 4u);
    const unsigned lane_a = (unsigned)(MT * ii + m0) * 4u, lane_b = (unsigned)(NT * ii + n0) * 4u;
    const unsigned row_a = (unsigned)cin * 4u, row_b = (unsigned)cout * 4u;
    auto round16 = [&](int d, int limit, auto full_tag) {
        constexpr bool FULL = decltype(full_tag)::value;
        float a[4][MTB], b[4][NTB];
        if constexpr (STAGE_A || STAGE_B) {
            float* const st = stage[wv];
            constexpr int LA = 4 * MTB, LB = 4 * NTB;
            constexpr int IA = STAGE_A ? LA / 4 : 0, IB = STAGE_B ? LB / 4 : 0;
            f32x4 ra[STAGE_A ? IA : 1], rb[STAGE_B ? IB : 1];
            if constexpr (STAGE_A) {
#pragma unroll
                for (int j = 0; j < IA; ++j) {
                    const int p = d + lane / LA + (64 / LA) * j;
                    const bool ok = FULL || p < limit;
                    ra[j] = __builtin_bit_cast(f32x4, __builtin_amdgcn_raw_buffer_load_b128(in_rsrc, ok ? (unsigned)qi[ok ? p : d] + (unsigned)(lane % LA) * 16u : OOB, 0, 0));
                }
            }
            if constexpr (STAGE_B) {
#pragma unroll
                for (int j = 0; j < IB; ++j) {
                    const int p = d + lane / LB + (64 / LB) * j;
                    const bool ok = FULL || p < limit;
                    rb[j] = __builtin_bit_cast(f32x4, __builtin_amdgcn_raw_buffer_load_b128(dout_rsrc, ok ? (unsigned)qo[ok ? p : d] + (unsigned)(lane % LB) * 16u : OOB, 0, 0));
                }
            }
#pragma unroll
            for (int t = 0; t < 4; ++t) {
                const int p = d + 4 * t + g;
                const bool ok = FULL || p < limit;
                const int pc = ok ? p : d;
                if constexpr (!STAGE_A) {
#pragma unroll
                    for (int m4 = 0; m4 < MTB; m4 += 4) {
                        const f32x4 v = __builtin_bit_cast(f32x4, __builtin_amdgcn_raw_buffer_load_b128(in_rsrc, ok ? (unsigned)qi[pc] + lane_a + 4u * m4 : OOB, 0, 0));
#pragma unroll
                        for (int m = 0; m < 4; ++m) a[t][m4 + m] = v[m];
                    }
                }
                if constexpr (!STAGE_B) {
#pragma unroll
                    for (int n4 = 0; n4 < NTB; n4 += 4) {
                        const f32x4 v = __builtin_bit_cast(f32x4, __builtin_amdgcn_raw_buffer_load_b128(dout_rsrc, ok ? (unsigned)qo[pc] + lane_b + 4u * n4 : OOB, 0, 0));
#pragma unroll
                        for (int n = 0; n < 4; ++n) b[t][n4 + n] = v[n];
                    }
                }
            }
            if constexpr (STAGE_A) {
#pragma unroll
                for (int j = 0; j < IA; ++j) *reinterpret_cast<f32x4*>(st + (lane / LA + (64 / LA) * j) * (16 * MTB) + (lane % LA) * 4) = ra[j];
            }
            if constexpr (STAGE_B) {
#pragma unroll
                for (int j = 0; j < IB; ++j) *reinterpret_cast<f32x4*>(st + 512 + (lane / LB + (64 / LB) * j) * (16 * NTB) + (lane % LB) * 4) = rb[j];
            }
            __builtin_amdgcn_wave_barrier();
#pragma unroll
            for (int t = 0; t < 4; ++t) {
                if constexpr (STAGE_A) {
#pragma unroll
                    for (int m = 0; m < MTB; ++m) a[t][m] = st[(4 * t + g) * (16 * MTB) + MTB * ii + m];
                }
                if constexpr (STAGE_B) {
#pragma unroll
                    for (int n = 0; n < NTB; ++n) b[t][n] = st[512 + (4 * t + g) * (16 * NTB) + NTB * ii + n];
                }
            }
            __builtin_amdgcn_wave_barrier();
        } else
#pragma unroll
        for (int t = 0; t < 4; ++t) {
            const int p = d + 4 * t + g;
            const bool ok = FULL || p < limit;
            const int pc = ok ? p : d;
            const unsigned ia = (unsigned)qi[pc] + lane_a;
            const unsigned ib = (unsigned)qo[pc] + lane_b;
            if constexpr (EXACT && MTB == 2) {
                const f32x2w v = __builtin_bit_cast(f32x2w, __builtin_amdgcn_raw_buffer_load_b64(in_rsrc, ok ? ia : OOB, 0, 0));
                a[t][0] = v[0], a[t][1] = v[1];
            } else if ((EXACT || exact_a) && MTB % 4 == 0) {
#pragma unroll
                for (int m4 = 0; m4 < MTB; m4 += 4) {
                    const f32x4 v = __builtin_bit_cast(f32x4, __builtin_amdgcn_raw_buffer_load_b128(in_rsrc, ok ? ia + 4u * m4 : OOB, 0, 0));
#pragma unroll
                    for (int m = 0; m < 4; ++m) a[t][m4 + m] = v[m];
                }
            } else {
#pragma unroll
                for (int m = 0; m < MTB; ++m)
                    a[t][m] = __builtin_bit_cast(float, __builtin_amdgcn_raw_buffer_load_b32(
                                  in_rsrc, (ok && (EXACT || MT * ii + m0 + m < cin)) ? ia + 4u * m : OOB, 0, 0));
            }
            if constexpr (EXACT && NTB == 2) {
                const f32x2w v = __builtin_bit_cast(f32x2w, __builtin_amdgcn_raw_buffer_load_b64(dout_rsrc, ok ? ib : OOB, 0, 0));
                b[t][0] = v[0], b[t][1] = v[1];
            } else if ((EXACT || exact_b) && NTB % 4 == 0) {
#pragma unroll
                for (int n4 = 0; n4 < NTB; n4 += 4) {
                    const f32x4 v = __builtin_bit_cast(f32x4, __builtin_amdgcn_raw_buffer_load_b128(dout_rsrc, ok ? ib + 4u * n4 : OOB, 0, 0));
#pragma unroll
                    for (int n = 0; n < 4; ++n) b[t][n4 + n] = v[n];
                }
            } else {
#pragma unroll
                for (int n = 0; n < NTB; ++n)
                    b[t][n] = __builtin_bit_cast(float, __builtin_amdgcn_raw_buffer_load_b32(
                                  dout_rsrc, (ok && (EXACT || NT * ii + n0 + n < cout)) ? ib + 4u * n : OOB, 0, 0));
            }
        }
#pragma unroll
        for (int t = 0; t < 4; ++t) {
            if (FULL || d + 4 * t < limit) {
#pragma unroll
                for (int m = 0; m < MTB; ++m)
#pragma unroll
// ... 432 lines not shown
            ++mine[cl & 7];
        }
        c[i] = (unsigned char)cl;
    }
#pragma unroll
    for (int k = 0; k < 8; ++k) cnt[k][t] = mine[k];
    __syncthreads();
    if (t < 8) {
        int run = 0;
        for (int j = 0; j < 256; ++j) {
            const int v = cnt[t][j];
            cnt[t][j] = run;
            run += v;
        }
        cnt[t][256] = run;
    }
    __syncthreads();
    int cls_base[8], run = 0;
#pragma unroll
    for (int k = 0; k < 8; ++k) {
        cls_base[k] = run + cnt[k][t];
        run += cnt[k][256];
    }
#pragma unroll
    for (int i = 0; i < CLS_PER; ++i) {
        const int r = base + t * CLS_PER + i;
        if (r >= n) break;
        const int k = c[i] & 7;
        int pos = 0;
#pragma unroll
        for (int q = 0; q < 8; ++q)
            if (q == k) pos = cls_base[q]++;
        order[base + pos] = r;
        cls_sorted[base + pos] = c[i];
    }
}

static int class_table(const int32_t* ksize, const int32_t* stride, const int32_t* pad, GatherClasses* out) {
    const int n_class = stride[0] * stride[1] * stride[2];
    if (n_class < 1 || n_class > 8 || ksize[0] * ksize[1] * ksize[2] > 27) return -1;
    *out = GatherClasses{};
    for (int rz = 0; rz < stride[0]; ++rz)
        for (int ry = 0; ry < stride[1]; ++ry)
            for (int rx = 0; rx < stride[2]; ++rx) {
                const int c = (rz * stride[1] + ry) * stride[2] + rx;
                int m = 0;
                for (int kz = 0; kz < ksize[0]; ++kz)
                    for (int ky = 0; ky < ksize[1]; ++ky)
                        for (int kx = 0; kx < ksize[2]; ++kx)
                            if (kz % stride[0] == rz && ky % stride[1] == ry && kx % stride[2] == rx)
                                out->k[c][m++] = (unsigned char)((kz * ksize[1] + ky) * ksize[2] + kx);
                out->count[c] = (unsigned char)m;
            }
    return 0;
}
}

extern "C" int toda_rulebook_class_order(const int32_t* in_coords, int n_in, const int32_t* stride, const int32_t* padding, int32_t* order,
                                         unsigned char* cls_sorted, void* stream) {
    TODA_CHECK_ARG(in_coords && stride && padding && order && cls_sorted && n_in >= 0, "rulebook_class_order: null argument");
    ClassGeom gm;
    for (int a = 0; a < 3; ++a) {
        TODA_CHECK_ARG(stride[a] >= 1 && stride[a] <= 2 && padding[a] >= 0, "rulebook_class_order: stride 1 or 2 per axis (got %d)", stride[a]);
        gm.stride[a] = stride[a], gm.pad[a] = padding[a];
    }
    if (n_in == 0) return TODA_OK;
    hipLaunchKernelGGL(class_order_kernel, dim3(cdiv(n_in, CLS_ROWS)), dim3(256), 0, (hipStream_t)stream, (const int4*)in_coords, n_in, gm, order,
                       cls_sorted);
    TODA_LAUNCH_CHECK();
    return TODA_OK;
}

namespace toda {
struct LaunchTimer {
    std::vector<hipEvent_t> ev;
    int used = 0;
    bool on = false;
};
static LaunchTimer g_timer;
static std::mutex g_timer_mu;
static inline void timer_next(hipEvent_t* start, hipEvent_t* stop) {
    *start = *stop = nullptr;
    if (!g_timer.on) return;
    std::lock_guard<std::mutex> lock(g_timer_mu);
    if (!g_timer.on || 2 * (g_timer.used + 1) > (int)g_timer.ev.size()) return;
    *start = g_timer.ev[2 * g_timer.used];
    *stop = g_timer.ev[2 * g_timer.used + 1];
    g_timer.used++;
}
}

#define GG_LAUNCH(kernel, grid, block, shmem, stream, ...)                                              \
    do {                                                                                               \
        hipEvent_t t0_, t1_;                                                                           \
        toda::timer_next(&t0_, &t1_);                                                                  \
        hipExtLaunchKernelGGL(kernel, grid, block, shmem, stream, t0_, t1_, 0, __VA_ARGS__);           \
    } while (0)

extern "C" int toda_timing_begin(int capacity) {
    TODA_CHECK_ARG(capacity > 0 && capacity <= (1 << 20), "timing_begin: capacity in (0, 2^20]");
    std::lock_guard<std::mutex> lock(toda::g_timer_mu);
    for (hipEvent_t e : g_timer.ev) (void)hipEventDestroy(e);
    g_timer.ev.assign((size_t)2 * capacity, nullptr);
    for (auto& e : g_timer.ev) TODA_HIP(hipEventCreate(&e));
    g_timer.used = 0;
    g_timer.on = true;
    return TODA_OK;
}

extern "C" int toda_timing_end(float* ms_out, int cap, int* n_out) {
    std::lock_guard<std::mutex> lock(toda::g_timer_mu);
    g_timer.on = false;
    const int n = g_timer.used < cap ? g_timer.used : cap;
    for (int i = 0; i < n; ++i) {
        TODA_HIP(hipEventSynchronize(g_timer.ev[2 * i + 1]));
        TODA_HIP(hipEventElapsedTime(&ms_out[i], g_timer.ev[2 * i], g_timer.ev[2 * i + 1]));
    }
    if (n_out) *n_out = g_timer.used;
    for (hipEvent_t e : g_timer.ev) (void)hipEventDestroy(e);
    g_timer.ev.clear();
    g_timer.used = 0;
    return TODA_OK;
}

namespace toda {
static bool gg_stats_supported(int c_gather, int c_produce) {
    const int Q = tiles_pow2(c_gather), NT = tiles_pow2(c_produce);
    return (c_gather & 3) == 0 && Q >= 2 && NT >= Q && Q * NT <= 32 && !(Q == 8 && NT == 8) && c_produce % 4 == 0 && c_produce == 16 * NT;
}

template <int V>
using tile_c = std::integral_constant<int, V>;
template <class F>
static void with_tiles(int tiles, F&& f) {
    switch (tiles) {
        case 1: f(tile_c<1>{}); break;
        case 2: f(tile_c<2>{}); break;
        case 4: f(tile_c<4>{}); break;
        default: f(tile_c<8>{}); break;
    }
}
template <class F>
static void with_tiles(int a, int b, F&& f) {
    with_tiles(a, [&](auto ta) { with_tiles(b, [&](auto tb) { f(ta, tb); }); });
}

struct GatherRoute {
    enum Family { SPLIT, LDS_128, LDS, REG } family;
    int rt, block, grid;
    bool vec;
};
}

static int gather_route(int c_gather, int c_produce, int n_out, bool stats, bool cls_sorted, GatherRoute* r) {
    const int Q = tiles_pow2(c_gather), NT = tiles_pow2(c_produce);
    const bool vec_ok = (c_gather & 3) == 0;
    const bool lds_faster = Q >= 2 && NT >= Q;
    r->rt = 2, r->block = SC_BLOCK, r->vec = vec_ok;
    if (use_split(c_gather, c_produce)) {
        TODA_CHECK_ARG(!(cls_sorted && stats), "gather_gemm (split path): no statistics on a class-sorted launch");
        r->family = GatherRoute::SPLIT;
    } else if (vec_ok && Q == 8 && NT == 8 && !cls_sorted) {
        r->family = GatherRoute::LDS_128, r->rt = 1, r->block = 512;
    } else if ((lds_faster || stats) && !cls_sorted && vec_ok && Q * NT <= 32) {
        r->family = GatherRoute::LDS, r->rt = NT < 8 ? 2 : 1;
    } else {
        TODA_CHECK_ARG(!stats, "gather_gemm: statistics requested on a launch shape without the fused epilogue");
        TODA_CHECK_ARG(vec_ok || Q == 1, "gather_gemm: gathered channel counts above 16 must be multiples of 4 (got %d)", c_gather);
        r->family = GatherRoute::REG;
        r->rt = NT < 8 ? 2 : (Q < 8 ? 1 : 2);
    }
    r->grid = cdiv(cdiv(n_out, 16 * r->rt), r->block / 64);
    return TODA_OK;
}

static int gather_gemm_impl(const float* in, int n_in, int c_gather, const float* wp, const int32_t* nbr, int n_out, int k_vol,
                            int c_produce, const float* bias, float* out, const int32_t* order, double* stats, int* blocks_out, void* stream,
                            const unsigned char* cls_sorted = nullptr, const toda::GatherClasses* cls_table = nullptr) {
    toda::GatherClasses classes = {};
    if (cls_sorted && cls_table) classes = *cls_table;
    else cls_sorted = nullptr;
    TODA_CHECK_ARG(c_gather >= 1 && c_gather <= 128 && c_produce >= 1 && c_produce <= 128,
                   "gather_gemm: channels must be in [1,128] (gather %d, produce %d)", c_gather, c_produce);
    TODA_CHECK_ARG(n_out >= 0 && n_in >= 0 && k_vol >= 1, "gather_gemm: bad sizes");
    TODA_CHECK_ARG((unsigned long long)n_in * c_gather * 4ull < 0xFFFFFFF0ull, "gather_gemm: gathered table must be < 4 GiB");
    if (n_out == 0) return TODA_OK;
    if (n_in == 0) {
        TODA_CHECK_ARG(bias == nullptr, "gather_gemm: empty input with bias is unsupported");
        TODA_HIP(hipMemsetAsync(out, 0, (size_t)n_out * c_produce * sizeof(float), (hipStream_t)stream));
        return TODA_OK;
    }
    GatherRoute r;
    const int rc = gather_route(c_gather, c_produce, n_out, stats != nullptr, cls_sorted != nullptr, &r);
    if (rc != TODA_OK) return rc;
    hipStream_t s = (hipStream_t)stream;
    const dim3 grid(r.grid), block(r.block);
    switch (r.family) {
        case GatherRoute::SPLIT:
            with_tiles(c_gather / 32, c_produce / 16, [&](auto kc, auto nt) {
                constexpr int KC = decltype(kc)::value, NT = decltype(nt)::value;
                if constexpr (KC <= 4 && NT >= 2)
                    GG_LAUNCH(HIP_KERNEL_NAME(gg_split_kernel<KC, NT, (NT == 8 ? 3 : 4), (NT == 2)>), grid, block, 0, s, in, n_in,
                              reinterpret_cast<const toda::u32x4*>(wp), nbr, n_out, k_vol, c_produce, bias, out, order, stats, cls_sorted, classes);
            });
            break;
        case GatherRoute::LDS_128:
            GG_LAUNCH(HIP_KERNEL_NAME(gather_gemm_lds_kernel<8, 8, 1, true, false, 512>), grid, block, 0, s, in, n_in, c_gather, wp, nbr, n_out,
                      k_vol, c_produce, bias, out, order, stats);
            break;
        case GatherRoute::LDS:
            with_tiles(tiles_pow2(c_gather), tiles_pow2(c_produce), [&](auto q, auto nt) {
                constexpr int Q = decltype(q)::value, NT = decltype(nt)::value, RT = NT < 8 ? 2 : 1;
                GG_LAUNCH(HIP_KERNEL_NAME(gather_gemm_lds_kernel<Q, NT, RT, true, true, SC_BLOCK, (Q <= 4 && NT <= 4 && RT == 2)>), grid, block, 0,
                          s, in, n_in, c_gather, wp, nbr, n_out, k_vol, c_produce, bias, out, order, stats);
            });
            break;
        case GatherRoute::REG: {
            auto reg = [&](auto q, auto nt, auto rt, auto vec) {
                constexpr int Q = decltype(q)::value, NT = decltype(nt)::value, RT = decltype(rt)::value;
                constexpr bool VEC = decltype(vec)::value;
                if (cls_sorted && VEC)
                    GG_LAUNCH(HIP_KERNEL_NAME(gather_gemm_kernel<Q, NT, RT, true, true>), grid, block, 0, s, in, n_in, c_gather, wp, nbr, n_out,
                              k_vol, c_produce, bias, out, order, cls_sorted, classes);
                else
                    GG_LAUNCH(HIP_KERNEL_NAME(gather_gemm_kernel<Q, NT, RT, VEC>), grid, block, 0, s, in, n_in, c_gather, wp, nbr, n_out, k_vol,
                              c_produce, bias, out, order, nullptr, classes);
            };
            if (!r.vec) {
                with_tiles(tiles_pow2(c_produce), [&](auto nt) {
                    reg(tile_c<1>{}, nt, tile_c<(decltype(nt)::value < 8 ? 2 : 1)>{}, std::false_type{});
                });
            } else {
                with_tiles(tiles_pow2(c_gather), tiles_pow2(c_produce), [&](auto q, auto nt) {
                    if constexpr (decltype(nt)::value < 8) reg(q, nt, tile_c<2>{}, std::true_type{});
                    else if (r.rt == 2) reg(q, nt, tile_c<2>{}, std::true_type{});
                    else reg(q, nt, tile_c<1>{}, std::true_type{});
                });
            }
            break;
        }
    }
    TODA_LAUNCH_CHECK();
    if (stats) {
        if (blocks_out) {
            *blocks_out = r.grid;
        } else {
            hipLaunchKernelGGL(toda::fold_partials_kernel, dim3(2 * c_produce), dim3(256), 0, s, stats, r.grid, 2 * c_produce);
            TODA_LAUNCH_CHECK();
        }
    }
    return TODA_OK;
}

extern "C" int toda_spconv_gather_gemm_ordered(const float* in, int n_in, int c_gather, const float* wp, const int32_t* nbr,
                                               int n_out, int k_vol, int c_produce, const float* bias, float* out,
                                               const int32_t* order, void* stream) {
    return gather_gemm_impl(in, n_in, c_gather, wp, nbr, n_out, k_vol, c_produce, bias, out, order, nullptr, nullptr, stream);
}

extern "C" int toda_spconv_gather_gemm_classed(const float* in, int n_in, int c_gather, const float* wp, const int32_t* nbr, int n_out, int k_vol,
                                               int c_produce, const float* bias, float* out, const int32_t* order,
                                               const unsigned char* cls_sorted, const int32_t* ksize, const int32_t* stride,
                                               const int32_t* padding, void* stream) {
    TODA_CHECK_ARG(order && cls_sorted && ksize && stride && padding, "gather_gemm_classed: null argument");
    TODA_CHECK_ARG(ksize[0] * ksize[1] * ksize[2] == k_vol, "gather_gemm_classed: kernel size does not match the table's %d offsets", k_vol);
    GatherClasses table;
    TODA_CHECK_ARG(class_table(ksize, stride, padding, &table) == 0, "gather_gemm_classed: needs <= 8 residue classes and <= 27 offsets");
    return gather_gemm_impl(in, n_in, c_gather, wp, nbr, n_out, k_vol, c_produce, bias, out, order, nullptr, nullptr, stream, cls_sorted, &table);
}

extern "C" int toda_spconv_gather_gemm_stats_supported(int c_gather, int c_produce) {
    return gg_stats_supported(c_gather, c_produce) ? 1 : 0;
}

extern "C" size_t toda_spconv_gather_gemm_stats_doubles(int n_out, int c_produce) {
    return (size_t)2 * c_produce * (1 + (size_t)cdiv(n_out > 0 ? n_out : 1, 64));
}

extern "C" int toda_spconv_gather_gemm_stats(const float* in, int n_in, int c_gather, const float* wp, const int32_t* nbr,
                                             int n_out, int k_vol, int c_produce, const float* bias, float* out, double* sums,
                                             size_t sums_doubles, void* stream) {
    TODA_CHECK_ARG(sums != nullptr && gg_stats_supported(c_gather, c_produce) && n_out > 0 && n_in > 0,
                   "gather_gemm_stats: unsupported channel pair (%d -> %d) or empty table", c_gather, c_produce);
    TODA_CHECK_ARG(sums_doubles >= toda_spconv_gather_gemm_stats_doubles(n_out, c_produce), "gather_gemm_stats: statistics buffer too small");
    return gather_gemm_impl(in, n_in, c_gather, wp, nbr, n_out, k_vol, c_produce, bias, out, nullptr, sums, nullptr, stream);
}

extern "C" int toda_spconv_gather_gemm_stats_partials(const float* in, int n_in, int c_gather, const float* wp, const int32_t* nbr,
                                                      int n_out, int k_vol, int c_produce, const float* bias, float* out, double* sums,
                                                      size_t sums_doubles, int* blocks_out, void* stream) {
    TODA_CHECK_ARG(sums != nullptr && blocks_out != nullptr && gg_stats_supported(c_gather, c_produce) && n_out > 0 && n_in > 0,
                   "gather_gemm_stats_partials: unsupported channel pair (%d -> %d), empty table or null argument", c_gather, c_produce);
    TODA_CHECK_ARG(sums_doubles >= toda_spconv_gather_gemm_stats_doubles(n_out, c_produce), "gather_gemm_stats_partials: statistics buffer too small");
    *blocks_out = 0;
    const int rc = gather_gemm_impl(in, n_in, c_gather, wp, nbr, n_out, k_vol, c_produce, bias, out, nullptr, sums, blocks_out, stream);
    if (rc == TODA_OK && *blocks_out <= 0) {
        set_error("gather_gemm_stats_partials: the launch took no statistics");
        return TODA_EINVAL;
    }
    return rc;
}

extern "C" int toda_spconv_gather_gemm(const float* in, int n_in, int c_gather, const float* wp, const int32_t* nbr,
                                       int n_out, int k_vol, int c_produce, const float* bias, float* out,
                                       void* stream) {
    return toda_spconv_gather_gemm_ordered(in, n_in, c_gather, wp, nbr, n_out, k_vol, c_produce, bias, out, nullptr, stream);
}

extern "C" int toda_spconv_gather_gemm_compact_supported(int c_gather, int c_produce, int k_vol) {
    return k_vol == CG_K && c_gather >= 1 && c_gather <= 32 && c_produce >= 1 && c_produce <= 32 && c_produce % 4 == 0;
}

static int gather_gemm_compact_impl(const float* in, int n_in, int c_gather, const float* w, int w_cout, int w_cin, int transpose,
                                    int flip_k, const int32_t* nbr, int n_out, int k_vol, int c_produce, const float* bias,
                                    float* out, double* stats, void* stream) {
    TODA_CHECK_ARG(toda_spconv_gather_gemm_compact_supported(c_gather, c_produce, k_vol),
                   "gather_gemm_compact: needs K = 27, <= 32 gathered and <= 32 produced channels (a multiple of 4) (got K %d, %d -> %d)", k_vol, c_gather,
                   c_produce);
    TODA_CHECK_ARG((transpose ? w_cout : w_cin) == c_gather && (transpose ? w_cin : w_cout) == c_produce,
                   "gather_gemm_compact: weight [%d][27][%d] (transpose %d) does not map %d -> %d channels", w_cout, w_cin, transpose, c_gather, c_produce);
    TODA_CHECK_ARG(n_out >= 0 && n_in >= 0, "gather_gemm_compact: bad sizes");
    TODA_CHECK_ARG((unsigned long long)n_in * c_gather * 4ull < 0xFFFFFFF0ull && (unsigned long long)n_out * CG_K * 4ull < 0xFFFFFFF0ull,
                   "gather_gemm_compact: gathered table and neighbour table must be < 4 GiB each");
    if (n_out == 0) return TODA_OK;
    hipStream_t s = (hipStream_t)stream;
    const dim3 grid(cdiv(n_out, CG_ROWS), cdiv(c_produce, 16));
    const bool vec = c_gather % 4 == 0;
#define CG_LAUNCH(QQ, VV)                                                                                                       \
    hipLaunchKernelGGL(HIP_KERNEL_NAME(gather_gemm_compact_kernel<QQ, VV>), grid, dim3(CG_BLOCK), 0, s, in, n_in, c_gather, w, w_cout, w_cin, \
                       transpose, flip_k, nbr, n_out, c_produce, bias, out, stats)
    if (c_gather <= 16) {
        if (vec) CG_LAUNCH(1, true);
        else CG_LAUNCH(1, false);
    } else {
        if (vec) CG_LAUNCH(2, true);
        else CG_LAUNCH(2, false);
    }
#undef CG_LAUNCH
    TODA_LAUNCH_CHECK();
    return TODA_OK;
}

extern "C" int toda_spconv_gather_gemm_compact(const float* in, int n_in, int c_gather, const float* w, int w_cout, int w_cin, int transpose,
                                               int flip_k, const int32_t* nbr, int n_out, int k_vol, int c_produce, const float* bias,
                                               float* out, void* stream) {
    return gather_gemm_compact_impl(in, n_in, c_gather, w, w_cout, w_cin, transpose, flip_k, nbr, n_out, k_vol, c_produce, bias, out, nullptr, stream);
}

extern "C" size_t toda_spconv_gather_gemm_compact_stats_doubles(int n_out, int c_produce) {
    return (size_t)2 * c_produce * (1 + (size_t)cdiv(n_out > 0 ? n_out : 1, CG_ROWS));
}

extern "C" int toda_spconv_gather_gemm_compact_stats(const float* in, int n_in, int c_gather, const float* w, int w_cout, int w_cin,
                                                     int transpose, int flip_k, const int32_t* nbr, int n_out, int k_vol, int c_produce,
                                                     const float* bias, float* out, double* sums, size_t sums_doubles, int* blocks_out,
                                                     void* stream) {
    TODA_CHECK_ARG(sums != nullptr && n_out > 0, "gather_gemm_compact_stats: null statistics buffer or no output rows");
    TODA_CHECK_ARG(sums_doubles >= toda_spconv_gather_gemm_compact_stats_doubles(n_out, c_produce), "gather_gemm_compact_stats: statistics buffer too small");
    const int rc = gather_gemm_compact_impl(in, n_in, c_gather, w, w_cout, w_cin, transpose, flip_k, nbr, n_out, k_vol, c_produce, bias, out, sums, stream);
    if (rc != TODA_OK) return rc;
    const int blocks = cdiv(n_out, CG_ROWS);
    if (blocks_out) {
        *blocks_out = blocks;
        return TODA_OK;
    }
    hipLaunchKernelGGL(toda::fold_partials_kernel, dim3(2 * c_produce), dim3(256), 0, (hipStream_t)stream, sums, blocks, 2 * c_produce);
    TODA_LAUNCH_CHECK();
    return TODA_OK;
}

extern "C" size_t toda_spconv_wgrad_workspace_bytes(int n_out, int k_vol, int cin, int cout) {
    int chunks, rpc;
    wgrad_plan(n_out, k_vol, cin, cout, &chunks, &rpc);
    return align_up((size_t)chunks * k_vol * cin * cout * sizeof(float), 256);
}

extern "C" int toda_spconv_wgrad(const float* in, int n_in, const float* dout, const int32_t* nbr, int n_out, int k_vol,
                                 int cin, int cout, float* dw, void* ws, size_t ws_bytes, void* stream) {
    TODA_CHECK_ARG(cin >= 1 && cin <= 128 && cout >= 1 && cout <= 128, "wgrad: channels must be in [1,128]");
    TODA_CHECK_ARG(n_out >= 0 && n_in >= 0 && k_vol >= 1, "wgrad: bad sizes");
    TODA_CHECK_ARG((unsigned long long)n_in * cin * 4ull < 0xFFFFFFF0ull && (unsigned long long)n_out * cout * 4ull < 0xFFFFFFF0ull,
                   "wgrad: feature tables must be < 4 GiB");
    hipStream_t s = (hipStream_t)stream;
    const long long elems = (long long)cout * k_vol * cin;
    if (n_out == 0 || n_in == 0) {
        TODA_HIP(hipMemsetAsync(dw, 0, elems * sizeof(float), s));
        return TODA_OK;
    }
    int chunks, rpc;
    wgrad_plan(n_out, k_vol, cin, cout, &chunks, &rpc);
    const size_t need = (size_t)chunks * elems * sizeof(float);
    if (ws_bytes < need) {
        set_error("wgrad: workspace %zu < required %zu", ws_bytes, need);
        return TODA_EWORKSPACE;
    }
    const int MT = tiles_pow2(cin), NT = tiles_pow2(cout);
    const int chunks_launch = (chunks + 7) / 8 * 8;
    const int grid = chunks_launch * k_vol;
    const bool exact = cin == 16 * MT && cout == 16 * NT;
    float* slab = (float*)ws;
    auto split = [&](auto kernel) {
        hipLaunchKernelGGL(kernel, dim3(grid), dim3(SC_BLOCK), 0, s, in, n_in, dout, nbr, n_out, k_vol, rpc, slab);
    };
    auto native = [&](auto kernel) {
        hipLaunchKernelGGL(kernel, dim3(grid), dim3(SC_BLOCK), 0, s, in, n_in, cin, dout, cout, nbr, n_out, k_vol, rpc, MT, NT, slab);
    };
    if (matrix_path() == 1 && toda::wgrad_split_shape_ok(cin, cout)) {
        if (cin == 128 && cout == 128) split(wgrad_split_kernel<4, 4, 2, 2>);
        else if (cin == 64 && cout == 128) split(wgrad_split_kernel<4, 4, 1, 2>);
        else if (cin == 128 && cout == 64) split(wgrad_split_kernel<4, 4, 2, 1>);
        else if (cin == 32 && cout == 32) split(wgrad_split_kernel<2, 2>);
        else if (cin == 32) split(wgrad_split_kernel<2, 4>);
        else if (cout == 32) split(wgrad_split_kernel<4, 2>);
        else split(wgrad_split_kernel<4, 4>);
    } else if (MT == 8 && NT == 8) {
        if (exact) native(wgrad_kernel<4, 4, true, true>);
        else native(wgrad_kernel<4, 4, true>);
    } else {
        with_tiles(MT, NT, [&](auto m, auto n) {
            constexpr int MTB = decltype(m)::value, NTB = decltype(n)::value;
            if constexpr (MTB < 8 || NTB < 8) {
                if (exact) native(wgrad_kernel<MTB, NTB, false, true>);
                else native(wgrad_kernel<MTB, NTB>);
            }
        });
    }
    hipLaunchKernelGGL(wgrad_reduce_kernel, dim3(cdiv(elems, SC_BLOCK)), dim3(SC_BLOCK), 0, s, slab, chunks, elems, dw);
    TODA_LAUNCH_CHECK();
    return TODA_OK;
}
```

toda_amd/csrc/spconv_split.cuh:

```cuda
#pragma once
#include "split_common.cuh"

namespace toda {

#ifndef WGS_ACCS
#define WGS_ACCS 2
#endif
#ifndef SP_STAMPS
#define SP_STAMPS 0
#endif
#if SP_STAMPS
#define SP_STAMP(i)                                                                               \
    do {                                                                                          \
        unsigned long long t_;                                                                    \
        __builtin_amdgcn_sched_barrier(0);                                                        \
        asm volatile("s_memtime %0\n\ts_waitcnt lgkmcnt(0)" : "=s"(t_)::"memory");                \
        __builtin_amdgcn_sched_barrier(0);                                                        \
        seg[i] += t_ - t_prev;                                                                    \
        t_prev = t_;                                                                              \
    } while (0)
#else
#define SP_STAMP(i)
#endif
#ifndef SP_ABLATE
#define SP_ABLATE 0
#endif
__device__ __forceinline__ void sp_split8(const f32x4& v0, const f32x4& v1, u32x4& h, u32x4& m, u32x4& l) {
#pragma unroll
    for (int p = 0; p < 4; ++p) {
        const float x0 = p < 2 ? v0[2 * p] : v1[2 * p - 4], x1 = p < 2 ? v0[2 * p + 1] : v1[2 * p - 3];
        h[p] = sp_pack_hi(x0, x1);
#if SP_ABLATE & 1
        m[p] = h[p] ^ 0x00010001u, l[p] = h[p] ^ 0x00020002u;
        continue;
#endif
        const float r0 = x0 - sp_trunc(x0), r1 = x1 - sp_trunc(x1);
        m[p] = sp_pack_hi(r0, r1);
        const float l0 = r0 - sp_trunc(r0), l1 = r1 - sp_trunc(r1);
        l[p] = sp_pack_hi(l0, l1);
    }
}
template <bool XOR_ONLY, int RT, int NT>
__device__ __forceinline__ void sp_six_terms(f32x4 (&acc)[RT][NT], int n, const u32x4 (&ah)[RT], const u32x4 (&am)[RT], const u32x4 (&al)[RT],
                                             const bf16x8& bh, const bf16x8& bm, const bf16x8& bl) {
    auto term = [&](const u32x4 (&a)[RT], const bf16x8& b) {
#pragma unroll
        for (int rt = 0; rt < RT; ++rt) {
            if constexpr (XOR_ONLY) acc[rt][n][0] += __builtin_bit_cast(float, a[rt][0] ^ __builtin_bit_cast(u32x4, b)[0]);
            else acc[rt][n] = __builtin_amdgcn_mfma_f32_16x16x32_bf16(__builtin_bit_cast(bf16x8, a[rt]), b, acc[rt][n], 0, 0, 0);
        }
    };
    term(al, bh);
    term(ah, bl);
    term(am, bm);
    term(am, bh);
    term(ah, bm);
    term(ah, bh);
}
__device__ __forceinline__ unsigned short sp_plane_of(float v, int plane) {
    const float h = sp_trunc(v), r = v - h, m = sp_trunc(r), l = r - m;
    const float pick = plane == 0 ? h : (plane == 1 ? m : l);
    return (unsigned short)(__builtin_bit_cast(unsigned, pick) >> 16);
}

constexpr int SPLIT_PACK_MAX_SEG = 48;
struct SplitPackBatch {
    const float* w[SPLIT_PACK_MAX_SEG];
    u32x4* wps[SPLIT_PACK_MAX_SEG];
    int cout[SPLIT_PACK_MAX_SEG], K[SPLIT_PACK_MAX_SEG], cin[SPLIT_PACK_MAX_SEG];
    unsigned char transpose[SPLIT_PACK_MAX_SEG], flip[SPLIT_PACK_MAX_SEG], KC[SPLIT_PACK_MAX_SEG], NT[SPLIT_PACK_MAX_SEG];
};
__global__ void __launch_bounds__(SC_BLOCK)
split_pack_batch_kernel(const SplitPackBatch b) {
    const int sg = blockIdx.y;
    const int K = b.K[sg], KC = b.KC[sg], NT = b.NT[sg], cin = b.cin[sg], cout = b.cout[sg];
    const long long e = (long long)blockIdx.x * SC_BLOCK + threadIdx.x;
    if (e >= (long long)K * KC * NT * 192) return;
    const int lane = (int)(e & 63);
    long long t = e >> 6;
    const int plane = (int)(t % 3);
    t /= 3;
    const int n = (int)(t % NT);
    t /= NT;
    const int kc = (int)(t % KC);
    const int k = (int)(t / KC);
    const int c = lane & 15, g = lane >> 4;
    const int pch = NT * c + n;
    const int kk = b.flip[sg] ? K - 1 - k : k;
    const float* __restrict__ w = b.w[sg];
    unsigned short v[8];
#pragma unroll
    for (int j = 0; j < 8; ++j) {
        const int gch = 32 * kc + 16 * (j >> 2) + 4 * g + (j & 3);
        float x = 0.0f;
        if (!b.transpose[sg]) {
            if (gch < cin && pch < cout) x = w[((size_t)pch * K + kk) * cin + gch];
        } else {
            if (gch < cout && pch < cin) x = w[((size_t)gch * K + kk) * cin + pch];
        }
        v[j] = sp_plane_of(x, plane);
    }
    b.wps[sg][e] = u32x4{(unsigned)v[0] | ((unsigned)v[1] << 16), (unsigned)v[2] | ((unsigned)v[3] << 16), (unsigned)v[4] | ((unsigned)v[5] << 16),
                         (unsigned)v[6] | ((unsigned)v[7] << 16)};
}

template <int KC, int NT, int WAVES, bool IL = false>
__global__ void __launch_bounds__(SC_BLOCK, WAVES)
gg_split_kernel(const float* __restrict__ in, int n_in, const u32x4* __restrict__ wps, const int* __restrict__ nbr, int n_out, int K, int cp,
                const float* __restrict__ bias, float* __restrict__ out, const int* __restrict__ order, double* __restrict__ stats,
                const unsigned char* __restrict__ cls_sorted, const GatherClasses classes) {
    constexpr int RT = 2;
    constexpr int CG = 32 * KC;
    constexpr int UNITS = NT * 3;
    constexpr int SLICE = UNITS * 64;
    static_assert(2 * SLICE * 16 >= (SC_BLOCK / 64) * 2 * 16 * NT * 4, "the statistics scratch aliases the weight buffers");
    __shared__ u32x4 wl[2 * SLICE];
    const int lane = threadIdx.x & 63, wv = threadIdx.x >> 6;
    const int blk = xcd_chunked_block(blockIdx.x, gridDim.x);
    const int wave = blk * (SC_BLOCK / 64) + wv;
    const int r = lane & 15, g = lane >> 4;
    const int row0 = wave * (16 * RT);

    f32x4 acc[RT][NT];
    int rows[RT];
    bool live[RT];
    gg_prologue<RT, NT>(bias, cp, row0, n_out, order, r, acc, rows, live);
    const __amdgpu_buffer_rsrc_t in_rsrc = table_rsrc(in, (unsigned)n_in * (unsigned)CG * 4u);
    int KE = K;
    bool listed = false;
    unsigned long long kpack = 0;
    if (cls_sorted) {
        const int p = row0 + (lane & (16 * RT - 1));
        const int c = cls_sorted[p < n_out ? p : n_out - 1], c0 = __builtin_amdgcn_readfirstlane(c);
        const bool same = __all(c == c0 || p >= n_out);
        int* cw = reinterpret_cast<int*>(wl);
        if (lane == 0) cw[wv] = same ? c0 : -1;
        __syncthreads();
        int cb = cw[0];
#pragma unroll
        for (int w = 1; w < SC_BLOCK / 64; ++w) cb = (cw[w] == cb) ? cb : -1;
        __syncthreads();
        if (cb >= 0 && classes.count[cb & 7] > 0 && classes.count[cb & 7] <= 8) {
            listed = true;
            KE = classes.count[cb & 7];
#pragma unroll
            for (int i = 0; i < 8; ++i) kpack |= (unsigned long long)classes.k[cb & 7][i] << (8 * i);
            kpack = ((unsigned long long)__builtin_amdgcn_readfirstlane((int)(kpack >> 32)) << 32) | (unsigned)__builtin_amdgcn_readfirstlane((int)kpack);
        }
    }
    auto kof = [&](int j) { return listed ? (int)((kpack >> (8 * j)) & 0xFF) : j; };
    auto load_ids = [&](int j, int (&dst)[RT]) {
        const int kk = kof(j < KE ? j : KE - 1);
#pragma unroll
        for (int rt = 0; rt < RT; ++rt) {
            dst[rt] = __builtin_nontemporal_load(nbr + (size_t)kk * n_out + rows[rt]);
        }
    };
    auto gather_rt = [&](const int (&src)[RT], int part, bool valid, f32x4 (&raw)[RT][2], int rt) {
        const bool ok = src[rt] >= 0 && valid;
        const unsigned base = (unsigned)src[rt] * (unsigned)(CG * 4) + (unsigned)(16 * g) + 128u * (unsigned)part;
#pragma unroll
        for (int i = 0; i < 2; ++i)
            raw[rt][i] = __builtin_bit_cast(f32x4, __builtin_amdgcn_raw_buffer_load_b128(in_rsrc, ok ? base + 64u * i : OOB, 0, 0));
    };
    auto gather = [&](const int (&src)[RT], int part, bool valid, f32x4 (&raw)[RT][2]) {
#pragma unroll
        for (int rt = 0; rt < RT; ++rt) gather_rt(src, part, valid, raw, rt);
    };
    auto stage = [&](int st, int buf) {
        const int sc = st < KE * KC ? st : KE * KC - 1;
        const int ss = kof(sc / KC) * KC + sc % KC;
#pragma unroll
        for (int t = 0; t < (UNITS + SC_BLOCK / 64 - 1) / (SC_BLOCK / 64); ++t) {
            const int u = t * (SC_BLOCK / 64) + wv;
            if (UNITS % (SC_BLOCK / 64) == 0 || u < UNITS)
                __builtin_amdgcn_global_load_lds(reinterpret_cast<const float*>(wps + (size_t)ss * SLICE + u * 64 + lane),
                                                 reinterpret_cast<float*>(&wl[buf * SLICE + u * 64]), 16, 0, 0);
        }
    };

    int idA[RT], idB[RT], idC[RT];
    f32x4 raw[RT][2];
    load_ids(0, idA);
    load_ids(1, idB);
    stage(0, 0);
    gather(idA, 0, true, raw);
    __syncthreads();

#if SP_STAMPS
    unsigned long long seg[6] = {0, 0, 0, 0, 0, 0}, t_prev;
    asm volatile("s_memtime %0\n\ts_waitcnt lgkmcnt(0)" : "=s"(t_prev)::"memory");
#endif
    auto body = [&](int k, const int (&ids_cur)[RT], const int (&ids_nxt)[RT], int (&ids_new)[RT]) {
        SP_STAMP(5);
        bool any = false;
#pragma unroll
        for (int rt = 0; rt < RT; ++rt) any = any || __any(ids_cur[rt] >= 0);
#pragma unroll
        for (int part = 0; part < KC; ++part) {
            const int cur = (k * KC + part) & 1;
            u32x4 ah[RT], am[RT], al[RT];
            f32x4 (&rw)[RT][2] = raw;
            if (any) {
#pragma unroll
                for (int rt = 0; rt < RT; ++rt) sp_split8(rw[rt][0], rw[rt][1], ah[rt], am[rt], al[rt]);
            }
            SP_STAMP(0);
            if constexpr (IL) {
                constexpr int PIECES = RT + 2;
                auto piece = [&](int p) {
                    if (p == 0) {
#if !(SP_ABLATE & 4)
                        stage(k * KC + part + 1, cur ^ 1);
#endif
                    } else if (p <= RT) {
                        if (part + 1 < KC) gather_rt(ids_cur, part + 1, true, raw, p - 1);
                        else gather_rt(ids_nxt, 0, k + 1 < KE, raw, p - 1);
                    } else if (part == KC - 1) load_ids(k + 2, ids_new);
                    asm volatile("" ::: "memory");
                };
                if (any) {
                    const u32x4* __restrict__ wb = wl + cur * SLICE + lane;
#pragma unroll
                    for (int n = 0; n < NT; ++n) {
                        const bf16x8 bh = __builtin_bit_cast(bf16x8, wb[(n * 3 + 0) * 64]), bm = __builtin_bit_cast(bf16x8, wb[(n * 3 + 1) * 64]),
                                     bl = __builtin_bit_cast(bf16x8, wb[(n * 3 + 2) * 64]);
#pragma unroll
                        for (int p = 0; p < PIECES; ++p)
                            if (p * NT / PIECES == n) piece(p);
                        sp_six_terms<false>(acc, n, ah, am, al, bh, bm, bl);
                    }
                } else {
#pragma unroll
                    for (int p = 0; p < PIECES; ++p) piece(p);
                }
            } else {
#if !(SP_ABLATE & 4)
            stage(k * KC + part + 1, cur ^ 1);
#endif
            asm volatile("" ::: "memory");
#if SP_ABLATE & 8
            if (k < 0)
#endif
            if (part + 1 < KC) gather(ids_cur, part + 1, true, raw);
            else gather(ids_nxt, 0, k + 1 < KE, raw);
            asm volatile("" ::: "memory");
#if !(SP_ABLATE & 16)
            if (part == KC - 1) load_ids(k + 2, ids_new);
#endif
            asm volatile("" ::: "memory");
            SP_STAMP(1);
            if (any) {
                const u32x4* __restrict__ wb = wl + cur * SLICE + lane;
#pragma unroll
                for (int n = 0; n < NT; ++n) {
                    const bf16x8 bh = __builtin_bit_cast(bf16x8, wb[(n * 3 + 0) * 64]), bm = __builtin_bit_cast(bf16x8, wb[(n * 3 + 1) * 64]),
                                 bl = __builtin_bit_cast(bf16x8, wb[(n * 3 + 2) * 64]);
                    sp_six_terms<(SP_ABLATE & 2) != 0>(acc, n, ah, am, al, bh, bm, bl);
                }
            }
            }
            SP_STAMP(2);
#if SP_ABLATE & (4 | 8 | 16)
            asm volatile("s_waitcnt vmcnt(0)" ::: "memory");
#else
            if (part == KC - 1) asm volatile("s_waitcnt vmcnt(%0)" ::"n"(RT * 2 + RT) : "memory");
            else asm volatile("s_waitcnt vmcnt(%0)" ::"n"(RT * 2) : "memory");
#endif
            SP_STAMP(3);
            __builtin_amdgcn_s_barrier();
            SP_STAMP(4);
        }
    };
    for (int k = 0;;) {
        body(k, idA, idB, idC);
        if (++k >= KE) break;
        body(k, idB, idC, idA);
        if (++k >= KE) break;
        body(k, idC, idA, idB);
        if (++k >= KE) break;
    }
    asm volatile("s_waitcnt vmcnt(0)" ::: "memory");
    if (row0 >= n_out && !stats) return;

#if SP_STAMPS
    if (stats) {
        if (lane == 0)
            for (int i = 0; i < 6; ++i) reinterpret_cast<unsigned long long*>(stats)[(size_t)wave * 6 + i] = seg[i];
        stats = nullptr;
    }
#endif
    if (stats) gg_moments<NT, RT, SC_BLOCK / 64>(reinterpret_cast<float (*)[2][16 * NT]>(wl), wv, blk, acc, row0, n_out, cp, stats, r, g);
    gg_store_rows<RT, NT>(acc, rows, row0, n_out, cp, out, r, g);
}

template <int MTB, int NTB, int QM = 1, int QN = 1>
__global__ void __launch_bounds__(SC_BLOCK, (MTB * NTB <= 4) ? 4 : ((MTB == 4 && NTB == 2) ? 3 : 2))
wgrad_split_kernel(const float* __restrict__ in, int n_in, const float* __restrict__ dout, const int* __restrict__ nbr, int n_out, int K,
                   int rows_per_chunk, float* __restrict__ slab) {
    static_assert((MTB == 2 || MTB == 4) && (NTB == 2 || NTB == 4), "32 or 64 channels a side");
    static_assert(QM * QN == 1 || (MTB == 4 && NTB == 4), "quarters are 64 x 64");
    static_assert(QM * QN == 1 || QM * QN == 2 || QM * QN == 4, "1, 2 or 4 quarters");
    constexpr int NQ = QM * QN, TEAMS = (SC_BLOCK / 64) / NQ;
    constexpr int MT = MTB * QM, NT = NTB * QN;
    constexpr int cin = 16 * MT, cout = 16 * NT;
    constexpr int QCAP = 64 + 32;
    __shared__ float red[TEAMS == 1 ? 1 : NQ * MTB * NTB * 4 * 64];
    __shared__ int q_in[SC_BLOCK / 64][QCAP], q_out[SC_BLOCK / 64][QCAP];
    const int lane = threadIdx.x & 63, wv = threadIdx.x >> 6;
    const int ii = lane & 15, g = lane >> 4;
    int chunk, k;
    wg_block(K, chunk, k);
    const int row_begin = chunk * rows_per_chunk;
    if (row_begin >= n_out) return;
    const int row_end = min(n_out, row_begin + rows_per_chunk);
    int* qi = q_in[wv];
    int* qo = q_out[wv];

    f32x4 acc[MTB][NTB];
#if WGS_ACCS >= 2
    f32x4 acc_s[MTB][NTB];
#endif
#if WGS_ACCS >= 3
    f32x4 acc_m[MTB][NTB];
#endif
#pragma unroll
    for (int m = 0; m < MTB; ++m)
#pragma unroll
        for (int n = 0; n < NTB; ++n) {
            acc[m][n] = f32x4{0.f, 0.f, 0.f, 0.f};
#if WGS_ACCS >= 2
            acc_s[m][n] = f32x4{0.f, 0.f, 0.f, 0.f};
#endif
#if WGS_ACCS >= 3
            acc_m[m][n] = f32x4{0.f, 0.f, 0.f, 0.f};
#endif
        }
    const __amdgpu_buffer_rsrc_t in_rsrc = table_rsrc(in, (unsigned)n_in * (unsigned)cin * 4u);
    const __amdgpu_buffer_rsrc_t dout_rsrc = table_rsrc(dout, (unsigned)n_out * (unsigned)cout * 4u);
    const int qd = wv % NQ, team = wv / NQ;
    const int m0 = (qd / QN) * MTB, n0 = (qd % QN) * NTB;
    const unsigned lane_a = (unsigned)(MT * ii + m0) * 4u, lane_b = (unsigned)(NT * ii + n0) * 4u;
    constexpr unsigned row_a = (unsigned)cin * 4u, row_b = (unsigned)cout * 4u;

    auto round32 = [&](int d, int limit, auto full_tag) {
        constexpr bool FULL = decltype(full_tag)::value;
        float a[8][MTB], b[8][NTB];
#pragma unroll
        for (int j = 0; j < 8; ++j) {
            const int p = d + 8 * g + j;
            const bool ok = FULL || p < limit;
            const int pc = ok ? p : d;
            const unsigned ia = (unsigned)qi[pc] + lane_a, ib = (unsigned)qo[pc] + lane_b;
            if constexpr (MTB == 4) {
                const f32x4 v = __builtin_bit_cast(f32x4, __builtin_amdgcn_raw_buffer_load_b128(in_rsrc, ok ? ia : OOB, 0, 0));
#pragma unroll
                for (int m = 0; m < 4; ++m) a[j][m] = v[m];
            } else {
                const f32x2w v = __builtin_bit_cast(f32x2w, __builtin_amdgcn_raw_buffer_load_b64(in_rsrc, ok ? ia : OOB, 0, 0));
                a[j][0] = v[0], a[j][1] = v[1];
            }
            if constexpr (NTB == 4) {
                const f32x4 v = __builtin_bit_cast(f32x4, __builtin_amdgcn_raw_buffer_load_b128(dout_rsrc, ok ? ib : OOB, 0, 0));
#pragma unroll
                for (int n = 0; n < 4; ++n) b[j][n] = v[n];
            } else {
                const f32x2w v = __builtin_bit_cast(f32x2w, __builtin_amdgcn_raw_buffer_load_b64(dout_rsrc, ok ? ib : OOB, 0, 0));
                b[j][0] = v[0], b[j][1] = v[1];
            }
        }
        u32x4 ah[MTB], am[MTB], al[MTB];
#pragma unroll
        for (int m = 0; m < MTB; ++m)
#pragma unroll
            for (int q = 0; q < 4; ++q) {
                unsigned h_, m_, l_;
                sp_split2(a[2 * q][m], a[2 * q + 1][m], h_, m_, l_);
                ah[m][q] = h_, am[m][q] = m_, al[m][q] = l_;
            }
#pragma unroll
        for (int n = 0; n < NTB; ++n) {
            u32x4 bh, bm, bl;
#pragma unroll
            for (int q = 0; q < 4; ++q) {
                unsigned h_, m_, l_;
                sp_split2(b[2 * q][n], b[2 * q + 1][n], h_, m_, l_);
                bh[q] = h_, bm[q] = m_, bl[q] = l_;
            }
#define WS_TERM(ACC, AA, BB)                                                                                             \
    _Pragma("unroll") for (int m = 0; m < MTB; ++m)                                                                       \
        ACC[m][n] = __builtin_amdgcn_mfma_f32_16x16x32_bf16(__builtin_bit_cast(bf16x8, AA[m]), __builtin_bit_cast(bf16x8, BB), ACC[m][n], 0, 0, 0)
#if WGS_ACCS == 1
            WS_TERM(acc, al, bh);
            WS_TERM(acc, ah, bl);
            WS_TERM(acc, am, bm);
            WS_TERM(acc, am, bh);
            WS_TERM(acc, ah, bm);
            WS_TERM(acc, ah, bh);
#elif WGS_ACCS == 2
            WS_TERM(acc_s, al, bh);
            WS_TERM(acc_s, ah, bl);
            WS_TERM(acc_s, am, bm);
            WS_TERM(acc, am, bh);
            WS_TERM(acc, ah, bm);
            WS_TERM(acc, ah, bh);
#else
            WS_TERM(acc_s, al, bh);
            WS_TERM(acc_s, ah, bl);
            WS_TERM(acc_s, am, bm);
            WS_TERM(acc_m, am, bh);
            WS_TERM(acc_m, ah, bm);
            WS_TERM(acc, ah, bh);
#endif
#undef WS_TERM
        }
    };

    wg_pair_walk<32>(qi, qo, row_begin + team * 64, row_end, TEAMS * 64, nbr + (size_t)k * n_out, n_out, row_a, row_b, lane, std::true_type{}, round32);
#if WGS_ACCS >= 2
#pragma unroll
    for (int m = 0; m < MTB; ++m)
#pragma unroll
        for (int n = 0; n < NTB; ++n) {
#if WGS_ACCS >= 3
            acc[m][n] = (acc_s[m][n] + acc_m[m][n]) + acc[m][n];
#else
            acc[m][n] = acc_s[m][n] + acc[m][n];
#endif
        }
#endif

    for (int src = 1; src < TEAMS; ++src) {
        float* const rq = red + qd * (MTB * NTB * 4 * 64);
        if (team == src) {
#pragma unroll
            for (int m = 0; m < MTB; ++m)
#pragma unroll
                for (int n = 0; n < NTB; ++n)
#pragma unroll
                    for (int reg = 0; reg < 4; ++reg) rq[((m * NTB + n) * 4 + reg) * 64 + lane] = acc[m][n][reg];
        }
        __syncthreads();
        if (team == 0) {
#pragma unroll
            for (int m = 0; m < MTB; ++m)
// ... 24 lines not shown
```

toda_amd/lib.py:

```python
import ctypes as C
import os

import torch

_HERE = os.path.dirname(os.path.abspath(__file__))
LIB_PATH = os.environ.get("TODA_HIP_LIB") or os.path.join(_HERE, "libtoda_hip.so")

_vp, _i, _sz, _dbl = C.c_void_p, C.c_int, C.c_size_t, C.c_double

SIGNATURES = {
    "toda_last_error": (C.c_char_p, []),
    "toda_abi_version": (_i, []),
    "toda_device_fault": (_i, []),
    "toda_voxelize_workspace_bytes": (_sz, [_i, _i]),
    "toda_voxelize_hard": (_i, [_vp, _i, _i, _vp, _vp, _vp, _i, _i, _vp, _vp, _vp, _vp, _vp, _sz, _vp]),
    "toda_mean_vfe_fwd": (_i, [_vp, _vp, _i, _i, _i, _vp, _vp]),
    "toda_mean_vfe_bwd": (_i, [_vp, _vp, _i, _i, _i, _vp, _vp]),
    "toda_dynvox_workspace_bytes": (_sz, [_i, _i, _vp, _i]),
    "toda_dynvox_count": (_i, [_vp, _i, _i, _i, _vp, _vp, _vp, _i, _vp, _vp, _sz, _vp]),
    "toda_dynvox_index": (_i, [_vp, _i, _i, _i, _vp, _vp, _vp, _i, _i, _i, _vp, _vp, _vp, _vp, _vp, _vp, _vp, _vp, _sz, _vp]),
    "toda_dynvox_seg_sum": (_i, [_vp, _i, _i, _i, _vp, _vp, _vp, _i, _i, _vp, _vp]),
    "toda_dynvox_pillar_decorate": (_i, [_vp, _i, _vp, _vp, _vp, _vp, _i, _vp, _vp, _i, _i, _vp, _i, _vp]),
    "toda_dynvox_seg_max_fwd": (_i, [_vp, _i, _vp, _vp, _i, _vp, _vp, _vp]),
    "toda_dynvox_seg_max_bwd": (_i, [_vp, _vp, _i, _i, _i, _vp, _vp]),
    "toda_dynvox_gather_concat": (_i, [_vp, _vp, _vp, _i, _i, _vp, _vp]),
    "toda_gridindex_bytes": (_sz, [_i, _vp]),
    "toda_gridindex_from_coords": (_i, [_vp, _i, _vp, _i, _vp, _vp, _vp, _vp]),
    "toda_gridindex_from_conv": (_i, [_vp, _i, _vp, _i, _vp, _vp, _vp, _vp, _vp, _vp, _vp, _vp, _i, _vp]),
    "toda_rulebook_subm": (_i, [_vp, _i, _i, _vp, _vp, _vp, _vp, _vp, _vp, _vp, _i, _vp]),
    "toda_rulebook_conv": (_i, [_vp, _i, _i, _vp, _vp, _vp, _vp, _vp, _vp, _i, _vp, _vp, _vp, _vp, _vp, _vp, _i, _vp]),
    "toda_voxelize_batch_workspace_bytes": (_sz, [_i, _i]),
    "toda_voxelize_batch": (_i, [_vp, _vp, _i, _i, _i, _i, _vp, _vp, _vp, _i, _i, _vp, _vp, _vp, _vp, _vp, _sz, _i, _vp]),
    "toda_gridindex_from_coords_unordered": (_i, [_vp, _i, _vp, _i, _vp, _vp, _vp, _i, _vp]),
    "toda_gridindex_clear": (_i, [_vp, _i, _vp, _i, _vp, _vp, _vp]),
    "toda_gridindex_from_bitmap": (_i, [_vp, _i, _vp, _vp, _vp, _vp, _vp, _vp, _vp, _vp, _i, _i, _vp]),
    "toda_spconv_packed_weight_floats": (_sz, [_i, _i, _i]),
    "toda_matrix_path": (_i, []),
    "toda_set_matrix_path": (_i, [_i]),
    "toda_spconv_split_supported": (_i, [_i, _i]),
    "toda_spconv_pack_weight": (_i, [_vp, _i, _i, _i, _i, _i, _vp, _vp]),
    "toda_spconv_pack_weights": (_i, [_i, _vp, _vp, _vp, _vp, _vp, _vp, _vp, _vp]),
    "toda_spconv_gather_gemm": (_i, [_vp, _i, _i, _vp, _vp, _i, _i, _i, _vp, _vp, _vp]),
    "toda_spconv_gather_gemm_ordered": (_i, [_vp, _i, _i, _vp, _vp, _i, _i, _i, _vp, _vp, _vp, _vp]),
    "toda_rulebook_class_order": (_i, [_vp, _i, _vp, _vp, _vp, _vp, _vp]),
    "toda_spconv_gather_gemm_classed": (_i, [_vp, _i, _i, _vp, _vp, _i, _i, _i, _vp, _vp, _vp, _vp, _vp, _vp, _vp, _vp]),
    "toda_spconv_gather_gemm_stats_supported": (_i, [_i, _i]),
    "toda_spconv_gather_gemm_stats_doubles": (_sz, [_i, _i]),
    "toda_spconv_gather_gemm_stats": (_i, [_vp, _i, _i, _vp, _vp, _i, _i, _i, _vp, _vp, _vp, _sz, _vp]),
    "toda_spconv_gather_gemm_stats_partials": (_i, [_vp, _i, _i, _vp, _vp, _i, _i, _i, _vp, _vp, _vp, _sz, _vp, _vp]),
    "toda_spconv_gather_gemm_compact_supported": (_i, [_i, _i, _i]),
    "toda_spconv_gather_gemm_compact": (_i, [_vp, _i, _i, _vp, _i, _i, _i, _i, _vp, _i, _i, _i, _vp, _vp, _vp]),
    "toda_spconv_gather_gemm_compact_stats_doubles": (_sz, [_i, _i]),
    "toda_spconv_gather_gemm_compact_stats": (_i, [_vp, _i, _i, _vp, _i, _i, _i, _i, _vp, _i, _i, _i, _vp, _vp, _vp, _sz, _vp, _vp]),
    "toda_spconv_wgrad_workspace_bytes": (_sz, [_i, _i, _i, _i]),
    "toda_spconv_wgrad": (_i, [_vp, _i, _vp, _vp, _i, _i, _i, _i, _vp, _vp, _sz, _vp]),
    "toda_sparse_to_dense_fwd": (_i, [_vp, _vp, _i, _i, _i, _vp, _vp, _vp]),
    "toda_sparse_to_dense_bwd": (_i, [_vp, _vp, _i, _i, _i, _vp, _vp, _vp]),
    "toda_pillar_scatter_fwd": (_i, [_vp, _vp, _i, _i, _i, _i, _i, _vp, _vp]),
    "toda_pillar_scatter_bwd": (_i, [_vp, _vp, _i, _i, _i, _i, _i, _vp, _vp]),
    "toda_rows_reduce_doubles": (_sz, [_i, _i]),
    "toda_rows_moments": (_i, [_vp, _i, _i, _vp, _vp]),
    "toda_rows_affine_act": (_i, [_vp, _vp, _vp, _vp, _i, _i, _i, _vp, _vp]),
    "toda_bn_finalize": (_i, [_vp, _i, _i, _vp, _vp, _vp, _vp, C.c_float, C.c_float, _i, _vp, _vp, _vp, _vp, _vp]),
    "toda_bn_finalize_partials": (_i, [_vp, _i, _i, _i, _vp, _vp, _vp, _vp, C.c_float, C.c_float, _vp, _vp, _vp, _vp, _vp]),
    "toda_rows_bn_bwd": (_i, [_vp, _vp, _vp, _vp, _i, _i, _i, _vp, _vp, _vp]),
    "toda_rows_bn_bwd_res": (_i, [_vp, _vp, _vp, _vp, _vp, _i, _i, _i, _vp, _vp, _vp, _vp]),
    "toda_rows_bn_bwd_colsum_doubles": (_sz, [_i, _i]),
    "toda_rows_bn_bwd_res_colsum": (_i, [_vp, _vp, _vp, _vp, _vp, _i, _i, _i, _vp, _vp, _vp, _vp, _vp, _vp]),
    "toda_conv3x3s2_supported": (_i, [_i, _i, _i, _i, _i]),
    "toda_conv3x3s2_fwd": (_i, [_vp, _vp, _i, _i, _i, _i, _i, _vp, _vp]),
    "toda_conv3x3s2_dgrad": (_i, [_vp, _vp, _i, _i, _i, _i, _i, _vp, _vp]),
    "toda_conv3x3s2_wgrad_workspace_bytes": (_sz, [_i, _i, _i, _i, _i]),
    "toda_conv3x3s2_wgrad": (_i, [_vp, _vp, _i, _i, _i, _i, _i, _vp, _vp, _sz, _vp]),
    "toda_deconv_supported": (_i, [_i, _i, _i, _i, _i, _i]),
    "toda_deconv_fwd": (_i, [_vp, _vp, _i, _i, _i, _i, _i, _i, _vp, _vp]),
    "toda_deconv_dgrad": (_i, [_vp, _vp, _i, _i, _i, _i, _i, _i, _vp, _vp]),
    "toda_deconv_wgrad_workspace_bytes": (_sz, [_i, _i, _i, _i, _i, _i]),
    "toda_deconv_wgrad": (_i, [_vp, _vp, _i, _i, _i, _i, _i, _i, _vp, _vp, _sz, _vp]),
    "toda_bn2d_supported": (_i, [_i, _i, _i]),
    "toda_bn2d_sync_bytes": (_sz, []),
    "toda_bn2d_fwd": (_i, [_vp, _i, _i, _i, _vp, _vp, _vp, _vp, C.c_float, C.c_float, _i, _vp, _vp, _vp, C.c_uint, _vp]),
    "toda_bn2d_bwd": (_i, [_vp, _vp, _i, _i, _i, _vp, _vp, _vp, _i, _vp, _vp, _vp, _vp, C.c_uint, _vp]),
    "toda_bn2d_fwd_into": (_i, [_vp, _i, _i, _i, _vp, _vp, _vp, _vp, C.c_float, C.c_float, _i, _vp, _i, _i, _vp, _vp, C.c_uint, _vp]),
    "toda_bn2d_bwd_from": (_i, [_vp, _vp, _i, _i, _i, _i, _i, _vp, _vp, _vp, _i, _vp, _vp, _vp, _vp, C.c_uint, _vp]),
    "toda_boxes_iou_bev": (_i, [_vp, _i, _vp, _i, _vp, _vp]),
    "toda_boxes_overlap_bev": (_i, [_vp, _i, _vp, _i, _vp, _vp]),
    "toda_nms_workspace_bytes": (_sz, [_i]),
    "toda_nms_rotated": (_i, [_vp, _i, C.c_float, _vp, _vp, _vp, _sz, _vp]),
    "toda_roi_grid_pool_bev": (_i, [_vp, _i, _i, _i, _i, _vp, _i, _i, C.c_float, C.c_float, C.c_float, C.c_float, _i, _vp, _vp]),
    "toda_roi_iou3d_max": (_i, [_vp, _i, _i, _i, _vp, _vp, _i, _i, _i, _vp, _vp, _vp]),
    "toda_voxel_query": (_i, [_vp, _vp, _i, _vp, _i, _vp, _vp, _i, _vp, C.c_float, _vp, _i, _vp, _vp, _vp]),
    "toda_voxel_pool_moments_doubles": (_sz, []),
    "toda_voxel_pool_moments": (_i, [_vp, _vp, _i, _i, _vp, _i, _vp, _vp, _vp]),
    "toda_voxel_pool_fwd": (_i, [_vp, _i, _i, _vp, _vp, _i, _i, _vp, _vp, _vp, _vp, _vp, _vp]),
    "toda_voxel_pool_table_bytes": (_sz, [_i, _i, _i]),
    "toda_voxel_pool_table": (_i, [_vp, _vp, _i, _i, _i, _vp, _vp, _vp, _sz, _vp]),
    "toda_voxel_pool_bwd_feat": (_i, [_vp, _vp, _i, _i, _i, _vp, _vp, _i, _vp, _vp]),
    "toda_voxel_pool_bwd_pos_doubles": (_sz, [_i]),
    "toda_voxel_pool_bwd_pos": (_i, [_vp, _vp, _vp, _vp, _i, _i, _i, _vp, _i, _vp, _vp, _vp, _vp]),
    "toda_fps_resident_blocks": (_i, []),
    "toda_fps_workspace_bytes": (_sz, [_i, _i]),
    "toda_fps": (_i, [_vp, _vp, _i, _i, _i, _vp, _vp, _vp, _sz, _vp]),
    "toda_ball_query_stack": (_i, [_vp, _i, _vp, _vp, _vp, _i, _i, _i, _vp, _vp, _vp, _vp, _vp]),
    "toda_sa_gather_fwd": (_i, [_vp, _i, _i, _vp, _vp, _vp, _i, _i, _vp, _vp, _vp, _vp]),
    "toda_sa_gather_bwd_feat": (_i, [_vp, _i, _i, _i, _vp, _vp, _i, _vp, _vp]),
    "toda_sa_gather_bwd_pos_doubles": (_sz, [_i]),
    "toda_sa_gather_bwd_pos": (_i, [_vp, _vp, _vp, _i, _i, _i, _vp, _i, _vp, _vp, _vp, _vp]),
    "toda_sa_max_fwd": (_i, [_vp, _i, _i, _i, _vp, _vp, _vp]),
    "toda_sa_max_bwd": (_i, [_vp, _vp, _i, _i, _i, _vp, _vp]),
    "toda_bev_interp_fwd": (_i, [_vp, _i, _i, _i, _i, _vp, _vp, _i, _vp, _vp, _vp, _vp]),
    "toda_bev_interp_bwd": (_i, [_vp, _i, _i, _vp, _vp, _vp, _i, _i, _i, _vp, _vp]),
    "toda_clip_adam_chunk": (_i, []),
    "toda_clip_adam_step": (_i, [_vp, _vp, _vp, _vp, _vp, _vp, _vp, _i, _vp, _vp, C.c_float, C.c_float, C.c_float, C.c_float, C.c_float, C.c_float, _i, _vp]),
    "toda_points_in_boxes": (_i, [_vp, _i, _vp, _i, _vp, _i, _i, _i, _vp, _vp]),
    "toda_points_sector": (_i, [_vp, _i, _vp, _i, _dbl, _dbl, _vp, _vp]),
    "toda_points_rect": (_i, [_vp, _i, _vp, _i, _vp, _vp, _i, _vp, _vp]),
    "toda_points_polar_cell": (_i, [_vp, _i, _vp, _i, C.c_float, _vp, _i, _vp, _i, C.c_float, C.c_float, _vp, _vp]),
    "toda_points_polar_select": (_i, [_vp, _i, _vp, _i, _dbl, _dbl, _i, _i, _dbl, _vp, _vp, _vp]),
    "toda_points_pitch_range_workspace_bytes": (_sz, []),
    "toda_points_pitch_range": (_i, [_vp, _i, _vp, _i, _vp, _vp, _sz, _vp]),
    "toda_points_pitch_band": (_i, [_vp, _i, _vp, _i, C.c_float, C.c_float, C.c_float, _vp, _i, _vp, _vp]),
    "toda_rows_select_workspace_bytes": (_sz, [_i]),
    "toda_rows_select_append": (_i, [_vp, _i, _vp, _i, _vp, _i, _i, _vp, _i, _vp, _vp, _sz, _vp]),
    "toda_points_rotate_z": (_i, [_vp, _i, _vp, _i, _dbl, _dbl, _vp, _vp]),
    "toda_points_world_transform": (_i, [_vp, _i, _vp, _i, _i, _i, _i, C.c_float, C.c_float, _i, C.c_float, _vp, _vp]),
    "toda_points_box_steps_chunk": (_i, []),
    "toda_points_box_steps": (_i, [_vp, _i, _vp, _i, _vp, _i, _vp, _vp, _vp]),
    "toda_points_column_range_workspace_bytes": (_sz, []),
    "toda_points_column_range": (_i, [_vp, _i, _vp, _i, _i, _vp, _vp, _sz, _vp]),
    "toda_points_in_pyramids": (_i, [_vp, _i, _vp, _i, _vp, _i, _vp, _vp, _vp]),
    "toda_points_fov_flags": (_i, [_vp, _i, _vp, _i, _vp, _vp, _i, _i, _vp, _vp]),
    "toda_sweeps_merge_max_sweeps": (_i, []),
    "toda_sweeps_merge": (_i, [_vp, _i, _i, _vp, _vp, _vp, _vp, _vp, C.c_float, _vp, _vp, _vp, _vp]),
    "toda_waymo_frame": (_i, [_vp, _i, _i, _i, _vp, _vp, _vp]),
    "toda_adv_edit_max_boxes": (_i, []),
    "toda_adv_edit_chunk": (_i, []),
    "toda_adv_edit_workspace_bytes": (_sz, [_i, _i]),
    "toda_adv_edit": (_i, [_vp, _i, _i, _vp, _vp, _i, _vp, _vp, _i, _vp, _vp, _vp, C.c_float, _vp, _i, _vp, _vp, _vp, _sz, _vp]),
    "toda_conv3x3_supported": (_i, [_i, _i, _i, _i, _i]),
    "toda_conv3x3_weight_floats": (_sz, [_i, _i]),
    "toda_conv3x3_transform_weight": (_i, [_vp, _i, _i, _i, _vp, _vp]),
    "toda_conv3x3_transform_weight_batch": (_i, [_vp, _i, _vp]),
    "toda_conv3x3_workspace_bytes": (_sz, []),
    "toda_conv3x3_wgrad_workspace_bytes": (_sz, [_i, _i, _i, _i, _i]),
    "toda_conv3x3_wgrad": (_i, [_vp, _vp, _i, _i, _i, _i, _i, _vp, _vp, _sz, _vp]),
    "toda_conv3x3_fwd": (_i, [_vp, _vp, _vp, _i, _i, _i, _i, _i, _vp, _vp, _sz, _vp]),
    "toda_conv3x3_narrow_supported": (_i, [_i, _i, _i, _i, _i]),
    "toda_conv3x3_narrow_fwd": (_i, [_i, _vp, _vp, _vp, _vp, _i, _i, _i, _i, C.c_longlong, _vp, _vp]),
    "toda_conv3x3_narrow_dgrad": (_i, [_i, _vp, _vp, _vp, _i, _i, _i, _i, C.c_longlong, _vp, _vp]),
    "toda_conv3x3_narrow_wgrad_workspace_bytes": (_sz, [_i, _i, _i, _i]),
    "toda_conv3x3_narrow_wgrad": (_i, [_i, _vp, _vp, _vp, _i, _i, _i, _i, C.c_longlong, _vp, _vp, _sz, _vp]),
    "toda_center_loss_workspace_bytes": (_sz, [_i, _i, _i, _i, _i, _i]),
    "toda_center_loss_fwd": (_i, [_vp, _vp, _i, _i, _i, _i, _i, _vp, _vp, _vp, _vp, _vp, _i, _i, _vp, C.c_float, C.c_float, _vp, _vp, _vp, _sz, _vp]),
    "toda_center_loss_bwd": (_i, [_vp, _vp, _vp, _i, _i, _i, _i, _i, _vp, _vp, _vp, _vp, _i, _i, _vp, C.c_float, C.c_float, _vp, _vp, _sz, _vp]),
    "toda_timing_begin": (_i, [_i]),
    "toda_timing_end": (_i, [_vp, _i, _vp]),
    "toda_center_assign": (_i, [_vp, _i, _i, _i, _i, _i, _i, _vp, _vp, _i, _i, _dbl, _i, _vp, _vp, _vp, _vp, _vp]),
    "toda_anchor_assign_workspace_bytes": (_sz, [_i, _i]),
    "toda_anchor_assign": (_i, [_vp, _vp, _vp, _vp, _vp, _i, _i, _vp, _i, _i, _i, _vp, _i, _i, _i, _i, _vp, _vp, _vp, _vp, _sz, _vp]),
    "toda_eval_overlaps": (_i, [_vp, _vp, _vp, _vp, _vp, _vp, _vp, _i, C.c_longlong, _i, _i, _vp, _vp]),
    "toda_eval_match_workspace_bytes": (_sz, [_i, _i, _i]),
    "toda_eval_match_scores": (_i, [_vp, _vp, _vp, _vp, _vp, _vp, _vp, _i, _i, _dbl, _vp, _vp, _vp, _sz, _vp]),
    "toda_eval_match": (_i, [_vp, _vp, _vp, _vp, _vp, _vp, _vp, _vp, _vp, _vp, _vp, _vp, _i, _i, _vp, _i, _dbl, _i, _i, _vp, _vp, _sz, _vp]),
    "toda_nusc_eval_prepare": (_i, [_vp, _vp, _vp, _i, _vp, _vp, _i, _vp, _vp, _vp]),
    "toda_nusc_eval_match_workspace_bytes": (_sz, [_i]),
    "toda_nusc_eval_match": (_i, [_vp, _vp, _vp, _i, _vp, _vp, _i, _vp, _vp, _vp, _i, _vp, _i, _vp, _vp, _vp, _sz, _vp]),
    "toda_waymo_eval_match_workspace_bytes": (_sz, [_i]),
    "toda_waymo_eval_iou": (_i, [_vp, _i, _vp, _i, _vp, _vp, _vp, _i, C.c_longlong, _vp, _vp, _sz, _vp]),
    "toda_waymo_eval_match": (_i, [_vp, _vp, _vp, _i, _vp, _vp, _i, _vp, _vp, _vp, _vp, _i, C.c_longlong, _vp, _vp, _vp, _vp, _vp, _vp, _vp, _sz, _vp]),
    "toda_consistency_workspace_bytes": (_sz, [_i, _i, _i]),
    "toda_consistency_loss": (_i, [_vp, _vp, _i, _vp, _vp, _i, _i, _i, C.c_float, _vp, _vp, _sz, _vp]),
}

_lib = None


def load():
    global _lib
    if _lib is not None:
        return _lib
    if not os.path.exists(LIB_PATH):
        raise RuntimeError(
            f"{LIB_PATH} not found: build it with `python -c 'import __graft_entry__ as g; g.build()'` "
            "(hipcc --offload-arch=gfx950).  toda_amd has no CPU fallback."
        )
    try:
        lib = C.CDLL(LIB_PATH)
    except OSError as e:
        raise RuntimeError(f"cannot load {LIB_PATH}: {e}") from e
    for name, (res, args) in SIGNATURES.items():
        try:
            fn = getattr(lib, name)
        except AttributeError as e:
            raise RuntimeError(f"{LIB_PATH} does not export {name}") from e
        fn.restype = res
        fn.argtypes = args
    _lib = lib
    return lib


def last_error():
    return load().toda_last_error().decode()


def check(rc, what):
    if rc != 0:
        raise RuntimeError(f"{what} failed (code {rc}): {last_error()}")


def ptr(t):
    if t is None:
        return None
    if not t.is_cuda:
        raise RuntimeError("toda_amd ops need tensors on the GPU (there is no CPU path)")
    if not t.is_contiguous():
        raise RuntimeError("toda_amd ops need contiguous tensors")
    return t.data_ptr()


_raw_stream = getattr(torch._C, "_cuda_getCurrentRawStream", None)
_raw_device = getattr(torch._C, "_cuda_getDevice", None)
# ... 38 lines not shown
```

toda_amd/ops.py:

```python
import numpy as np
import torch

from . import arena as _arena
from . import lib as L


def _triple(v):
    if isinstance(v, (list, tuple)):
        assert len(v) == 3
        return [int(x) for x in v]
    return [int(v)] * 3


def grid_size_xyz(pc_range, voxel_size):
    r = np.asarray(pc_range, dtype=np.float64)
    return np.round((r[3:6] - r[0:3]) / np.asarray(voxel_size, dtype=np.float64)).astype(np.int64)


import os as _os
import time as _time

_COUNT_PINNED = {}
_LAST_WAIT_S = 0.0

# ... 471 lines not shown
        ks, sd, pd = _triple(st["ksize"]), _triple(st["stride"]), _triple(st["padding"])
        out_shape = conv_out_shape(cur["shape"], ks, sd, pd)
        cap = _conv_cap(cur["n_upper"], batch, out_shape, ks, sd)
        li += 1
        shape_c = L.host_i32(out_shape)
        buf, _ = _persistent(("gi", tag, li), (int(batch), tuple(out_shape)), lib.toda_gridindex_bytes(int(batch), L.hptr(shape_c)), dev)
        gi_out = GridIndex(batch, out_shape, dev, buf=buf)
        idx_out = _alloc((max(cap, 1), 4), torch.int32, dev)
        hs = [L.host_i32(v) for v in (cur["shape"], ks, sd, pd, out_shape)]
        rc = lib.toda_gridindex_from_bitmap(L.ptr(cur["gi"].buf), int(batch), L.hptr(hs[0]), L.hptr(hs[1]), L.hptr(hs[2]), L.hptr(hs[3]),
                                            L.hptr(hs[4]), L.ptr(gi_out.buf), L.ptr(idx_out), counts.data_ptr() + 4 * (c0 + li - 1),
                                            cap, 1 if li == 1 else 0, L.stream())
        L.check(rc, "toda_gridindex_from_bitmap")
        levels.append({"idx": idx_out, "n_upper": cap, "shape": out_shape, "gi": gi_out, "cap": cap, "step": st})
    if slot is not None:
        slot.plans += 1
    return levels


def _plan_tables(levels, level_counts, batch, steps, training):
    dev = levels[0]["idx"].device
    for lv, n in zip(levels, level_counts):
        if lv.get("cap") is not None and n > lv["cap"]:
            raise RuntimeError(f"strided rulebook {lv['step']['key']}: {n} outputs exceed the bound {lv['cap']}")
        lv["n"] = int(n)
        lv["idx"] = lv["idx"][:int(n)]
    keys = []
    for st in steps:
        if st["key"] not in keys:
            keys.append(st["key"])
    cnts = torch.zeros((len(keys), 64), dtype=torch.int32, device=dev)
    out = {}
    li = 0
    for st in steps:
        cur = levels[li]
        if st["kind"] == "subm":
            if st["key"] in out:
                continue
            ks = _triple(st["ksize"])
            rb, gi = build_subm_rulebook(cur["idx"], batch, cur["shape"], st["ksize"], st.get("dilation", 1), grid_index=cur["gi"],
                                         pair_cnt=cnts[keys.index(st["key"])][:ks[0] * ks[1] * ks[2]])
            out[st["key"]] = {"kind": "subm", "rb": rb, "n_in": cur["n"]}
        else:
            nxt = levels[li + 1]
            ks, sd, pd = _triple(st["ksize"]), _triple(st["stride"]), _triple(st["padding"])
            rb = _conv_tables(cur["idx"], cur["n"], nxt["idx"], nxt["n"], batch, cur["shape"], nxt["shape"], ks, sd, pd, nxt["gi"],
                              gi_in=cur["gi"], pair_cnt=cnts[keys.index(st["key"])][:ks[0] * ks[1] * ks[2]])
            if training:
                rb.class_order()
            out[st["key"]] = {"kind": "conv", "rb": rb, "n_in": cur["n"], "out_indices": nxt["idx"],
                              "out_shape": nxt["shape"], "gi": nxt["gi"]}
            li += 1
    return out


def build_index_plan(indices, batch, shape, steps, while_waiting=None, training=None):
    indices = indices.contiguous()
    n_conv = sum(1 for st in steps if st["kind"] == "conv")
    counts = _alloc((max(n_conv, 1),), torch.int32, indices.device)
    levels = _plan_enqueue((indices, indices.shape[0], None), batch, shape, steps, counts, 0)
    got = read_counts(counts, while_waiting) if n_conv else []
    if training is None:
        training = torch.is_grad_enabled()
    return _plan_tables(levels, [indices.shape[0]] + list(got[:n_conv]), batch, steps, training)


def build_input_plan(clouds, voxel_cfg, batch, shape, steps, training=True, while_waiting=None):
    n_conv = sum(1 for st in steps if st["kind"] == "conv")
    bsz = len(clouds)
    dev = clouds[0][0].device
    slot = _arena.current_slot()
    gi0 = GridIndex.unordered_begin(batch, shape, dev, name=("gi0", slot.plans if slot is not None else 0))
    counts = _alloc((bsz + 1 + n_conv,), torch.int32, dev)
    voxels, coords, num, _ = voxelize_enqueue(clouds, voxel_cfg["point_cloud_range"], voxel_cfg["voxel_size"],
                                              voxel_cfg["max_points_per_voxel"], voxel_cfg["max_num_voxels"], counts=counts,
                                              tag=slot.plans if slot is not None else 0)
    levels = _plan_enqueue((coords, coords.shape[0], counts[bsz:bsz + 1]), batch, shape, steps, counts, bsz + 1, gi0=gi0)
    got = read_counts(counts, while_waiting)
    m = got[bsz]
    plan = _plan_tables(levels, [m] + list(got[bsz + 1:bsz + 1 + n_conv]), batch, steps, training)
    return voxels[:m], levels[0]["idx"], num[:m], plan


MATRIX_PATHS = ("native", "split")
_MM = None


def matrix_path():
    global _MM
    if _MM is None:
        _MM = MATRIX_PATHS[L.load().toda_matrix_path()]
    return _MM


def set_matrix_path(name):
    global _MM
    L.check(L.load().toda_set_matrix_path(MATRIX_PATHS.index(name)), "toda_set_matrix_path")
    _MM = name


def _tag_mm(wp, cg, cp):
    wp._toda_mm = matrix_path() if L.load().toda_spconv_split_supported(int(cg), int(cp)) else None
    return wp


def _check_mm(wp):
    mm = getattr(wp, "_toda_mm", None)
    if mm is not None and mm != matrix_path():
        raise RuntimeError(f"packed sparse-conv operand was written under matrix path {mm!r}, the current path is {matrix_path()!r}: re-pack it")


def pack_weight(weight, transpose, flip_k):
    lib = L.load()
    cout, cin = weight.shape[0], weight.shape[-1]
    K = weight.numel() // (cout * cin)
    cg, cp = (cout, cin) if transpose else (cin, cout)
    n = lib.toda_spconv_packed_weight_floats(K, cg, cp)
    wp = torch.empty((n,), dtype=torch.float32, device=weight.device)
    rc = lib.toda_spconv_pack_weight(L.ptr(weight.contiguous()), cout, K, cin, int(transpose), int(flip_k), L.ptr(wp),
                                     L.stream())
    L.check(rc, "toda_spconv_pack_weight")
    return _tag_mm(wp, cg, cp)


def pack_weights_batched(items):
    lib = L.load()
    if not items:
        return []
    dev = items[0][0].device
    sizes, couts, ks, cins, pairs = [], [], [], [], []
    for w, tr, _ in items:
        cout, cin = w.shape[0], w.shape[-1]
        K = w.numel() // (cout * cin)
        cg, cp = (cout, cin) if tr else (cin, cout)
        sizes.append(lib.toda_spconv_packed_weight_floats(K, cg, cp))
        couts.append(cout), ks.append(K), cins.append(cin), pairs.append((cg, cp))
    flat = torch.empty((sum(sizes),), dtype=torch.float32, device=dev)
    outs, off = [], 0
    for n, (cg, cp) in zip(sizes, pairs):
        outs.append(_tag_mm(flat[off:off + n], cg, cp))
        off += n
    ws = [w.contiguous() for w, _, _ in items]
    rc = lib.toda_spconv_pack_weights(len(items), L.host_ptrs(ws), L.hptr(L.host_i32(couts)), L.hptr(L.host_i32(ks)), L.hptr(L.host_i32(cins)),
                                      L.hptr(L.host_i32([int(bool(t)) for _, t, _ in items])), L.hptr(L.host_i32([int(bool(f)) for _, _, f in items])),
                                      L.host_ptrs(outs), L.stream())
    L.check(rc, "toda_spconv_pack_weights")
    return outs


def gather_gemm_stats_supported(c_gather, c_produce):
    return bool(L.load().toda_spconv_gather_gemm_stats_supported(int(c_gather), int(c_produce)))


def gather_gemm_with_stats(feat, wp, nbr, c_produce, bias=None, partials=False):
    lib = L.load()
    K, n_out = nbr.shape
    out = torch.empty((n_out, c_produce), dtype=torch.float32, device=feat.device)
    nd = lib.toda_spconv_gather_gemm_stats_doubles(n_out, c_produce)
    sums = torch.empty((nd,), dtype=torch.float64, device=feat.device)
    if partials:
        import ctypes
        blocks = ctypes.c_int(0)
        rc = lib.toda_spconv_gather_gemm_stats_partials(L.ptr(feat), feat.shape[0], feat.shape[1], L.ptr(wp), L.ptr(nbr), n_out, K, c_produce,
                                                        L.ptr(bias), L.ptr(out), L.ptr(sums), nd, ctypes.addressof(blocks), L.stream())
        L.check(rc, "toda_spconv_gather_gemm_stats_partials")
        return out, sums, int(blocks.value)
    rc = lib.toda_spconv_gather_gemm_stats(L.ptr(feat), feat.shape[0], feat.shape[1], L.ptr(wp), L.ptr(nbr), n_out, K, c_produce,
                                           L.ptr(bias), L.ptr(out), L.ptr(sums), nd, L.stream())
    L.check(rc, "toda_spconv_gather_gemm_stats")
    return out, sums


def gather_gemm(feat, wp, nbr, c_produce, bias=None, order=None):
    lib = L.load()
    K, n_out = nbr.shape
    out = torch.empty((n_out, c_produce), dtype=torch.float32, device=feat.device)
    rc = lib.toda_spconv_gather_gemm_ordered(L.ptr(feat), feat.shape[0], feat.shape[1], L.ptr(wp), L.ptr(nbr), n_out, K,
                                             c_produce, L.ptr(bias), L.ptr(out), L.ptr(order), L.stream())
    L.check(rc, "toda_spconv_gather_gemm_ordered")
    return out


RETIRED_KNOBS = ("TODA_GG_LINE", "TODA_HALO", "TODA_WG_TILE", "TODA_ROW_ORDER", "TODA_GG_WS", "TODA_GG_STAGE", "TODA_GG_WRES", "TODA_GG_LDS_PF",
                 "TODA_GG_BLK512", "TODA_GG_RT", "TODA_SPLIT_BLK", "TODA_SPLIT_KCS", "TODA_WINO_WGRAD",
                 "TODA_WGRAD_STREAM", "TODA_BN_FOLD_FINALIZE", "TODA_FUSE_BN_STATS", "TODA_GG_COMPACT", "TODA_CLASS_DGRAD", "TODA_BN_BWD_COLSUM",
                 "TODA_GG_LDS", "TODA_WG_SUB", "TODA_WG_XCD", "TODA_WG_CHUNKS", "TODA_PREFETCH_PRIORITY", "TODA_PREFETCH_ARENA",
                 "TODA_PREFETCH_STREAM_WAIT", "TODA_PREFETCH_HOST_WAIT", "TODA_PREFETCH_PHASE", "TODA_PREFETCH_POLL", "TODA_DENSE_CHANNELS_LAST")


def _refuse_retired_knobs():
    retired = [k for k in RETIRED_KNOBS if _os.environ.get(k, "0") not in ("0", "")]
    if retired:
        raise RuntimeError(f"{', '.join(retired)}: these variants were retired (profiles/EXPERIMENTS.md); unset the variable(s)")
    ablate = [k for k in ("TODA_GG_ABLATE", "TODA_WINO_ABLATE", "TODA_WINO_WG_ABLATE") if _os.environ.get(k, "0") not in ("0", "")]
    if ablate and not _os.environ.get("TODA_HIP_LIB"):
        raise RuntimeError(f"{', '.join(ablate)} only act in a measurement build (-DTODA_ABLATE=1, loaded through TODA_HIP_LIB): the library "
                           "that ships ignores them, and a run that believes it ablated something would report wrong conclusions")


_refuse_retired_knobs()


COMPACT = True


def _compact_route(c_gather, c_produce, nbr):
    return (COMPACT and nbr.shape[0] == 27 and nbr.shape[1] > 0 and c_produce in (16, 32) and c_gather <= 32
            and (c_gather <= 16 or c_produce == 16))


def gather_gemm_compact_supported(c_gather, c_produce, k_vol):
    return bool(L.load().toda_spconv_gather_gemm_compact_supported(int(c_gather), int(c_produce), int(k_vol)))


def gather_gemm_compact(feat, weight, nbr, c_produce, bias=None, transpose=False, flip_k=False, stats=False):
    lib = L.load()
    K, n_out = nbr.shape
    out = torch.empty((n_out, c_produce), dtype=torch.float32, device=feat.device)
    if stats:
        import ctypes
        nd = lib.toda_spconv_gather_gemm_compact_stats_doubles(n_out, c_produce)
        sums = torch.empty((nd,), dtype=torch.float64, device=feat.device)
        blocks = ctypes.c_int(0)
        rc = lib.toda_spconv_gather_gemm_compact_stats(L.ptr(feat), feat.shape[0], feat.shape[1], L.ptr(weight), weight.shape[0], weight.shape[-1],
                                                       int(bool(transpose)), int(bool(flip_k)), L.ptr(nbr), n_out, K, c_produce, L.ptr(bias), L.ptr(out),
                                                       L.ptr(sums), nd, ctypes.addressof(blocks), L.stream())
        L.check(rc, "toda_spconv_gather_gemm_compact_stats")
        return out, sums, int(blocks.value)
    rc = lib.toda_spconv_gather_gemm_compact(L.ptr(feat), feat.shape[0], feat.shape[1], L.ptr(weight), weight.shape[0], weight.shape[-1],
                                             int(bool(transpose)), int(bool(flip_k)), L.ptr(nbr), n_out, K, c_produce, L.ptr(bias), L.ptr(out), L.stream())
    L.check(rc, "toda_spconv_gather_gemm_compact")
    return out


def gather_gemm_classed(feat, wp, nbr, c_produce, order, cls_sorted, ksize, stride, padding):
    lib = L.load()
    K, n_out = nbr.shape
    out = torch.empty((n_out, c_produce), dtype=torch.float32, device=feat.device)
    ks, st, pd = L.host_i32(ksize), L.host_i32(stride), L.host_i32(padding)
    rc = lib.toda_spconv_gather_gemm_classed(L.ptr(feat), feat.shape[0], feat.shape[1], L.ptr(wp), L.ptr(nbr), n_out, K, c_produce, None,
                                             L.ptr(out), L.ptr(order), L.ptr(cls_sorted), L.hptr(ks), L.hptr(st), L.hptr(pd), L.stream())
    L.check(rc, "toda_spconv_gather_gemm_classed")
    return out


def wgrad(feat, dout, nbr, wshape):
    lib = L.load()
    K, n_out = nbr.shape
    cout, cin = wshape[0], wshape[-1]
    dw = torch.empty(wshape, dtype=torch.float32, device=feat.device)
    ws_bytes = lib.toda_spconv_wgrad_workspace_bytes(n_out, K, cin, cout)
    ws = torch.empty((max(ws_bytes, 16),), dtype=torch.uint8, device=feat.device)
    rc = lib.toda_spconv_wgrad(L.ptr(feat), feat.shape[0], L.ptr(dout), L.ptr(nbr), n_out, K, cin, cout, L.ptr(dw),
                               L.ptr(ws), ws_bytes, L.stream())
    L.check(rc, "toda_spconv_wgrad")
    return dw


CLASS_DGRAD_MIN_ROWS = 4096


class _SparseConv(torch.autograd.Function):

    @staticmethod
    def forward(ctx, features, weight, bias, rb, wp_fwd, want_stats=False, wp_bwd=None):
        features = features.contiguous()
        compact = _compact_route(features.shape[1], weight.shape[0], rb.nbr_fwd)
        if wp_fwd is None and not compact:
            wp_fwd = pack_weight(weight, False, False)
        if wp_fwd is not None:
            _check_mm(wp_fwd)
        if compact and want_stats:
            out, sums, blocks = gather_gemm_compact(features, weight.contiguous(), rb.nbr_fwd, weight.shape[0], bias, stats=True)
        elif want_stats:
            out, sums, blocks = gather_gemm_with_stats(features, wp_fwd, rb.nbr_fwd, weight.shape[0], bias, partials=True)
        elif compact:
            out = gather_gemm_compact(features, weight.contiguous(), rb.nbr_fwd, weight.shape[0], bias)
        else:
            out = gather_gemm(features, wp_fwd, rb.nbr_fwd, weight.shape[0], bias)
        ctx.set_materialize_grads(False)
        ctx.save_for_backward(features, weight)
        ctx.rb = rb
        ctx.wp_bwd = wp_bwd
        ctx.has_bias = bias is not None
        if want_stats:
            ctx.mark_non_differentiable(sums)
            return out, sums, blocks
        return out

    @staticmethod
    def backward(ctx, gout, *unused):
        features, weight = ctx.saved_tensors
        rb = ctx.rb
        if gout is None:
            return None, None, None, None, None, None, None
        gout = gout.contiguous()
        gfeat = gw = gb = None
        need_d, need_w = ctx.needs_input_grad[0], ctx.needs_input_grad[1]
        if need_d and _compact_route(gout.shape[1], weight.shape[-1], rb.nbr_bwd):
            gfeat = gather_gemm_compact(gout, weight.contiguous(), rb.nbr_bwd, weight.shape[-1], None, True, rb.flip_bwd)
        elif need_d:
            wp_t = ctx.wp_bwd if ctx.wp_bwd is not None else pack_weight(weight, True, rb.flip_bwd)
            _check_mm(wp_t)
            co = rb.class_order()
            if co is not None:
                gfeat = gather_gemm_classed(gout, wp_t, rb.nbr_bwd, weight.shape[-1], co[0], co[1], rb.ksize, rb.geom["stride"], rb.geom["padding"])
            else:
                gfeat = gather_gemm(gout, wp_t, rb.nbr_bwd, weight.shape[-1], None)
        if need_w:
            gw = wgrad(features, gout, rb.nbr_fwd, tuple(weight.shape))
        if ctx.has_bias and ctx.needs_input_grad[2]:
            gb = _take_colsum(gout)
            if gb is None:
                gb = gout.sum(0)
        return gfeat, gw, gb, None, None, None, None


def sparse_conv(features, weight, bias, rulebook, packed_weight=None, want_stats=False, packed_dgrad=None):
    if not want_stats:
        return _SparseConv.apply(features, weight, bias, rulebook, packed_weight, False, packed_dgrad)
    narrow = _compact_route(features.shape[1], weight.shape[0], rulebook.nbr_fwd)
    ok = (narrow or gather_gemm_stats_supported(weight.shape[-1], weight.shape[0])) and rulebook.nbr_fwd.shape[1] > 1 and features.shape[0] > 0
    if not ok:
        return _SparseConv.apply(features, weight, bias, rulebook, packed_weight, False, packed_dgrad), None
    out, sums, blocks = _SparseConv.apply(features, weight, bias, rulebook, packed_weight, True, packed_dgrad)
    return out, (sums, blocks)


class _ToDense(torch.autograd.Function):
    @staticmethod
    def forward(ctx, features, indices, batch, shape):
        lib = L.load()
        n, c = features.shape
        shape = [int(s) for s in shape]
        dense = torch.empty((batch, c, *shape), dtype=torch.float32, device=features.device)
        sh = L.host_i32(shape)
        rc = lib.toda_sparse_to_dense_fwd(L.ptr(features.contiguous()), L.ptr(indices), n, c, batch, L.hptr(sh),
                                          L.ptr(dense), L.stream())
        L.check(rc, "toda_sparse_to_dense_fwd")
        ctx.save_for_backward(indices)
        ctx.meta = (n, c, batch, shape)
        return dense

    @staticmethod
    def backward(ctx, gdense):
        (indices,) = ctx.saved_tensors
        n, c, batch, shape = ctx.meta
        g = torch.empty((n, c), dtype=torch.float32, device=gdense.device)
        sh = L.host_i32(shape)
        rc = L.load().toda_sparse_to_dense_bwd(L.ptr(gdense.contiguous()), L.ptr(indices), n, c, batch, L.hptr(sh),
                                               L.ptr(g), L.stream())
        L.check(rc, "toda_sparse_to_dense_bwd")
        return g, None, None, None


def sparse_to_dense(features, indices, batch, shape):
    return _ToDense.apply(features, indices.contiguous(), int(batch), shape)


class _PillarScatter(torch.autograd.Function):
    @staticmethod
    def forward(ctx, features, indices, batch, ny, nx):
        n, c = features.shape
        canvas = torch.empty((batch, c, ny, nx), dtype=torch.float32, device=features.device)
        rc = L.load().toda_pillar_scatter_fwd(L.ptr(features.contiguous()), L.ptr(indices), n, c, batch, ny, nx,
                                              L.ptr(canvas), L.stream())
        L.check(rc, "toda_pillar_scatter_fwd")
        ctx.save_for_backward(indices)
        ctx.meta = (n, c, batch, ny, nx)
        return canvas

    @staticmethod
    def backward(ctx, gcanvas):
        (indices,) = ctx.saved_tensors
        n, c, batch, ny, nx = ctx.meta
        g = torch.empty((n, c), dtype=torch.float32, device=gcanvas.device)
        rc = L.load().toda_pillar_scatter_bwd(L.ptr(gcanvas.contiguous()), L.ptr(indices), n, c, batch, ny, nx, L.ptr(g),
                                              L.stream())
        L.check(rc, "toda_pillar_scatter_bwd")
        return g, None, None, None, None


def pillar_scatter(features, indices, batch, ny, nx):
    return _PillarScatter.apply(features, indices.contiguous(), int(batch), int(ny), int(nx))


def rows_moments(x):
    n, c = x.shape
    lib = L.load()
    sums = torch.empty((lib.toda_rows_reduce_doubles(n, c),), dtype=torch.float64, device=x.device)
    L.check(lib.toda_rows_moments(L.ptr(x.contiguous()), n, c, L.ptr(sums), L.stream()), "toda_rows_moments")
    return sums[:2 * c]


def rows_affine_act(x, scale, shift, residual=None, relu=True):
    n, c = x.shape
    y = torch.empty_like(x)
    rc = L.load().toda_rows_affine_act(L.ptr(x.contiguous()), L.ptr(scale.contiguous()), L.ptr(shift.contiguous()),
                                       L.ptr(residual), n, c, int(bool(relu)), L.ptr(y), L.stream())
    L.check(rc, "toda_rows_affine_act")
    return y


_DX_COLSUM = {}
BN_BWD_COLSUM = True


def _take_colsum(gout):
    ent = _DX_COLSUM.pop(gout.data_ptr(), None) if _DX_COLSUM else None
    if ent is None or ent[0].shape != gout.shape or ent[0]._version != ent[2] or gout.stride() != ent[0].stride():
        return None
    return ent[1]


class _BNRows(torch.autograd.Function):

    @staticmethod
    def forward(ctx, x, weight, bias, running_mean, running_var, training, momentum, eps, relu, residual=None, sums=None, colsum=False):
        lib = L.load()
        if _DX_COLSUM:
            _DX_COLSUM.clear()
        ctx.colsum = bool(colsum) and BN_BWD_COLSUM
        x = x.contiguous()
        residual = residual.contiguous() if residual is not None else None
        n, c = x.shape
        dev = x.device
        stats = torch.empty((4, c), dtype=torch.float32, device=dev)
        if isinstance(sums, tuple) and training:
            part, blocks = sums
            rc = lib.toda_bn_finalize_partials(L.ptr(part), int(blocks), n, c, L.ptr(weight), L.ptr(bias), L.ptr(running_mean), L.ptr(running_var),
                                               float(momentum), float(eps), L.ptr(stats[0]), L.ptr(stats[1]), L.ptr(stats[2]), L.ptr(stats[3]), L.stream())
            L.check(rc, "toda_bn_finalize_partials")
            sums = part
        else:
            if isinstance(sums, tuple):
                sums = None
            sums = _BNRows._finalize(lib, x, n, c, dev, sums, training, weight, bias, running_mean, running_var, momentum, eps, stats)
        y = torch.empty_like(x)
        rc = lib.toda_rows_affine_act(L.ptr(x), L.ptr(stats[2]), L.ptr(stats[3]), L.ptr(residual), n, c, int(bool(relu)), L.ptr(y),
                                      L.stream())
        L.check(rc, "toda_rows_affine_act")
        ctx.save_for_backward(x, stats, weight, residual)
        ctx.meta = (n, c, bool(relu), bool(training))
        return y

    @staticmethod
    def _finalize(lib, x, n, c, dev, sums, training, weight, bias, running_mean, running_var, momentum, eps, stats):
        if sums is None or not training:
            sums = torch.empty((lib.toda_rows_reduce_doubles(n, c),), dtype=torch.float64, device=dev)
            if training:
                L.check(lib.toda_rows_moments(L.ptr(x), n, c, L.ptr(sums), L.stream()), "toda_rows_moments")
        rc = lib.toda_bn_finalize(L.ptr(sums), n, c, L.ptr(weight), L.ptr(bias), L.ptr(running_mean), L.ptr(running_var),
                                  float(momentum), float(eps), int(bool(training)), L.ptr(stats[0]), L.ptr(stats[1]),
                                  L.ptr(stats[2]), L.ptr(stats[3]), L.stream())
        L.check(rc, "toda_bn_finalize")
        return sums

    @staticmethod
    def backward(ctx, gy):
        x, stats, weight, residual = ctx.saved_tensors
        n, c, relu, training = ctx.meta
        gy = gy.contiguous()
        want_res = residual is not None and ctx.needs_input_grad[9]
        if not training:
            pre = x * stats[2] + stats[3]
            if residual is not None:
                pre = pre + residual
            dz = gy * (pre > 0) if relu else gy
            gx = dz * stats[2]
            xhat = (x - stats[0]) * stats[1]
            return gx, (dz * xhat).sum(0), dz.sum(0), None, None, None, None, None, None, (dz if want_res else None), None, None
        sums = torch.empty((L.load().toda_rows_reduce_doubles(n, c),), dtype=torch.float64, device=x.device)
        gx = torch.empty_like(x)
        gamma = weight if weight is not None else torch.ones(c, device=x.device)
        gres = torch.empty_like(x) if want_res else None
        if ctx.colsum:
            lib = L.load()
            cs_ws = torch.empty((lib.toda_rows_bn_bwd_colsum_doubles(n, c),), dtype=torch.float64, device=x.device)
            cs = torch.empty((c,), dtype=torch.float32, device=x.device)
            rc = lib.toda_rows_bn_bwd_res_colsum(L.ptr(gy), L.ptr(x), L.ptr(residual), L.ptr(stats), L.ptr(gamma), n, c, int(relu),
                                                 L.ptr(sums), L.ptr(gx), L.ptr(gres), L.ptr(cs_ws), L.ptr(cs), L.stream())
            L.check(rc, "toda_rows_bn_bwd_res_colsum")
            _DX_COLSUM[gx.data_ptr()] = (gx, cs, gx._version)
        else:
            rc = L.load().toda_rows_bn_bwd_res(L.ptr(gy), L.ptr(x), L.ptr(residual), L.ptr(stats), L.ptr(gamma), n, c, int(relu),
                                               L.ptr(sums), L.ptr(gx), L.ptr(gres), L.stream())
            L.check(rc, "toda_rows_bn_bwd_res")
        gs = sums[2 * c:3 * c].view(torch.float32)
        return gx, gs[c:], gs[:c], None, None, None, None, None, None, gres, None, None


def bn_rows(x, bn, relu, residual=None, sums=None, colsum=False):
    training = bn.training or not bn.track_running_stats
    bump_bn_counter(bn)
    momentum = 0.0 if bn.momentum is None else bn.momentum
    return _BNRows.apply(x, bn.weight, bn.bias, bn.running_mean, bn.running_var, training, momentum, bn.eps, relu, residual, sums, colsum)


def bn_rows_supported(x, bn):
    c = x.shape[1]
    return (type(bn) is torch.nn.BatchNorm1d and x.is_cuda and x.dtype == torch.float32 and 4 <= c <= 128 and 256 % c == 0 and bn.affine and bn.momentum is not None
            and x.shape[0] > 1)


_BN2D_SYNC = {}


def _bn2d_sync(device):
    key = (device.index, L.stream())
    ent = _BN2D_SYNC.get(key)
    if ent is None:
        ent = _BN2D_SYNC[key] = [torch.zeros((L.load().toda_bn2d_sync_bytes(),), dtype=torch.uint8, device=device), 0]
    ent[1] = ent[1] % 0xFFFFFFF0 + 1
    return ent[0], ent[1]


class _BN2d(torch.autograd.Function):

    @staticmethod
    def forward(ctx, x, weight, bias, running_mean, running_var, momentum, eps, relu):
        lib = L.load()
        x = x.contiguous()
        b, c, h, w = x.shape
        y = torch.empty_like(x)
        save = torch.empty((2, c), dtype=torch.float32, device=x.device)
        ws, epoch = _bn2d_sync(x.device)
        rc = lib.toda_bn2d_fwd(L.ptr(x), b, c, h * w, L.ptr(weight), L.ptr(bias), L.ptr(running_mean), L.ptr(running_var), float(momentum),
                               float(eps), int(bool(relu)), L.ptr(y), L.ptr(save), L.ptr(ws), epoch, L.stream())
        L.check(rc, "toda_bn2d_fwd")
        ctx.save_for_backward(x, weight, bias, save)
        ctx.relu = bool(relu)
        return y

    @staticmethod
    def backward(ctx, gy):
        x, weight, bias, save = ctx.saved_tensors
        lib = L.load()
        b, c, h, w = x.shape
        gy = gy.contiguous()
        gx = torch.empty_like(x)
        gwb = torch.empty((2, c), dtype=torch.float32, device=x.device)
        ws, epoch = _bn2d_sync(x.device)
        rc = lib.toda_bn2d_bwd(L.ptr(x), L.ptr(gy), b, c, h * w, L.ptr(weight), L.ptr(bias), L.ptr(save), int(ctx.relu), L.ptr(gx),
                               L.ptr(gwb[0]), L.ptr(gwb[1]), L.ptr(ws), epoch, L.stream())
        L.check(rc, "toda_bn2d_bwd")
        return gx, gwb[0], gwb[1], None, None, None, None, None


class _BN2dCat(torch.autograd.Function):

    @staticmethod
    def forward(ctx, relu, n, *flat):
        lib = L.load()
        items = [flat[7 * i:7 * i + 7] for i in range(n)]
        xs = [it[0].contiguous() for it in items]
        b, _, h, w = xs[0].shape
        chans = [x.shape[1] for x in xs]
        out = torch.empty((b, sum(chans), h, w), dtype=torch.float32, device=xs[0].device)
        saves, c0 = [], 0
        for x, it in zip(xs, items):
            _, weight, bias, rm, rv, momentum, eps = it
            c = x.shape[1]
            save = torch.empty((2, c), dtype=torch.float32, device=x.device)
            ws, epoch = _bn2d_sync(x.device)
            rc = lib.toda_bn2d_fwd_into(L.ptr(x), b, c, h * w, L.ptr(weight), L.ptr(bias), L.ptr(rm), L.ptr(rv), float(momentum), float(eps),
                                        int(bool(relu)), L.ptr(out), out.shape[1], c0, L.ptr(save), L.ptr(ws), epoch, L.stream())
            L.check(rc, "toda_bn2d_fwd_into")
            saves.append(save)
            c0 += c
        ctx.save_for_backward(*xs, *[it[1] for it in items], *[it[2] for it in items], *saves)
        ctx.meta = (bool(relu), n, chans)
        return out

    @staticmethod
    def backward(ctx, g):
        relu, n, chans = ctx.meta
        t = ctx.saved_tensors
        xs, weights, biases, saves = t[:n], t[n:2 * n], t[2 * n:3 * n], t[3 * n:]
        lib = L.load()
        g = g.contiguous()
        b, ctot, h, w = g.shape
        grads, c0 = [], 0
        for x, weight, bias, save, c in zip(xs, weights, biases, saves, chans):
            gx = torch.empty_like(x)
            gwb = torch.empty((2, c), dtype=torch.float32, device=x.device)
            ws, epoch = _bn2d_sync(x.device)
            rc = lib.toda_bn2d_bwd_from(L.ptr(x), L.ptr(g), ctot, c0, b, c, h * w, L.ptr(weight), L.ptr(bias), L.ptr(save), int(relu), L.ptr(gx),
                                        L.ptr(gwb[0]), L.ptr(gwb[1]), L.ptr(ws), epoch, L.stream())
            L.check(rc, "toda_bn2d_bwd_from")
            grads += [gx, gwb[0], gwb[1], None, None, None, None]
            c0 += c
        return (None, None, *grads)


FUSED_BN2D = _os.environ.get("TODA_BN2D", "1") == "1"
BN2D_CAT = _os.environ.get("TODA_BN2D_CAT", "1") == "1"


def bn2d_supported(x, bn):
    if not (FUSED_BN2D and type(bn) is torch.nn.BatchNorm2d and bn.training and bn.affine and bn.track_running_stats and bn.momentum is not None):
        return False
    if not (x.is_cuda and x.dtype == torch.float32 and x.dim() == 4 and x.is_contiguous()):
        return False
    return bool(L.load().toda_bn2d_supported(x.shape[0], x.shape[1], x.shape[2] * x.shape[3]))


def bn2d(x, bn, relu):
    bump_bn_counter(bn)
    return _BN2d.apply(x, bn.weight, bn.bias, bn.running_mean, bn.running_var, bn.momentum, bn.eps, relu)


def bn2d_cat(pairs, relu=True):
    flat = []
    for x, bn in pairs:
        bump_bn_counter(bn)
        flat += [x, bn.weight, bn.bias, bn.running_mean, bn.running_var, bn.momentum, bn.eps]
    return _BN2dCat.apply(relu, len(pairs), *flat)


def bn_relu_tail(seq):
    mods = list(seq)
    if len(mods) >= 2 and type(mods[-1]) is torch.nn.ReLU and type(mods[-2]) is torch.nn.BatchNorm2d:
        return mods[:-2], mods[-2]
    return None


def run_dense_sequential(seq, x):
    mods = list(seq)
    conv3x3_prepack(mods, x)
    i = 0
    while i < len(mods):
        m = mods[i]
# ... 1339 lines not shown
```

Baseline: 149.7.

## Fuse BN backward reductions into sparse-conv dgrad gather-GEMM epilogue

The sparse-conv data-gradient gather-GEMM now also computes the BatchNorm backward partial sums (sum of dz and dz*xhat) in its epilogue, reading x and the BN stats directly. The following BN backward then skips its own reduction kernel and only folds the partials and applies dx. This removes one full read pass over dy and x per eligible BN layer (32/64 channels, no residual, training). The cost is extra x loads, register pressure in the GEMM epilogue, and a Python-side cache keyed by data pointer that has to match tensors correctly.

```diff
diff --git a/include/toda.h b/include/toda.h
--- a/include/toda.h
+++ b/include/toda.h
@@ -165,6 +165,10 @@
                                 const float* gamma, int n, int c, int relu, double* sums, float* dx,
                                 float* dres , double* colsum_ws , float* dx_colsum ,
                                 void* stream);
+
+int toda_rows_bn_bwd_apply(const float* dy, const float* x, const float* residual , const float* stats,
+                           const float* gamma, int n, int c, int relu, double* sums, int blocks, float* dx,
+                           float* dres , double* colsum_ws , float* dx_colsum , void* stream);
 
 int toda_bn2d_supported(int batch, int c, int hw);
 size_t toda_bn2d_sync_bytes(void);
@@ -312,6 +316,14 @@
                                            int n_out, int k_vol, int c_produce, const float* bias , float* out,
                                            double* sums, size_t sums_doubles, int* blocks_out, void* stream);
 
+int toda_spconv_gather_gemm_bn_bwd_supported(int c_gather, int c_produce, int classed);
+int toda_spconv_gather_gemm_bn_bwd(const float* in, int n_in, int c_gather, const float* wp, const int32_t* nbr, int n_out,
+                                   int k_vol, int c_produce, float* out, const int32_t* order ,
+                                   const unsigned char* cls_sorted , const int32_t* ksize ,
+                                   const int32_t* stride , const int32_t* padding , const float* x,
+                                   const float* bn_stats, int relu, double* sums, size_t sums_doubles, int* blocks_out,
+                                   void* stream);
+
 int toda_conv3x3_supported(int batch, int cin, int cout, int H, int W);
 size_t toda_conv3x3_weight_floats(int cout, int cin);
 int toda_conv3x3_transform_weight(const float* w, int cout, int cin, int mode, float* u, void* stream);
diff --git a/toda_amd/csrc/bn_fold.cuh b/toda_amd/csrc/bn_fold.cuh
--- a/toda_amd/csrc/bn_fold.cuh
+++ b/toda_amd/csrc/bn_fold.cuh
@@ -46,6 +46,14 @@
     bn_write_channel(ch, mean, var, eps, gamma, beta, mean_out, invstd_out, scale_out, shift_out);
 }
 
+__device__ __forceinline__ void bn_bwd_value(float dy, float x, bool has_res, float res, float scale, float shift, float mean, float invstd,
+                                             int relu, float& dz, float& dz_xhat) {
+    float pre = x * scale + shift;
+    if (has_res) pre += res;
+    dz = (relu && !(pre > 0.f)) ? 0.f : dy;
+    dz_xhat = dz * ((x - mean) * invstd);
+}
+
 __global__ void __launch_bounds__(DN_BLOCK) fold_partials_kernel(double* __restrict__ sums, int blocks, int cols);
 
 }
diff --git a/toda_amd/csrc/dense.hip b/toda_amd/csrc/dense.hip
--- a/toda_amd/csrc/dense.hip
+++ b/toda_amd/csrc/dense.hip
@@ -181,11 +181,10 @@
         const f32x4 rv = r4 ? r4[(size_t)r * lanes + cl] : f32x4{0.f, 0.f, 0.f, 0.f};
 #pragma unroll
         for (int j = 0; j < 4; ++j) {
-            float pre = xv[j] * sc[j] + sf[j];
-            if (r4) pre += rv[j];
-            const float dz = (relu && !(pre > 0.f)) ? 0.f : g[j];
+            float dz, dz_xhat;
+            bn_bwd_value(g[j], xv[j], r4 != nullptr, rv[j], sc[j], sf[j], mu[j], is[j], relu, dz, dz_xhat);
             a[j] = dz;
-            b[j] = dz * ((xv[j] - mu[j]) * is[j]);
+            b[j] = dz_xhat;
         }
     }, sums);
 }
@@ -219,9 +218,8 @@
         f32x4 out, dzv;
 #pragma unroll
         for (int j = 0; j < 4; ++j) {
-            float pre = xv[j] * sc[j] + sf[j];
-            if (res) pre += rv[j];
-            const float dz = (relu && !(pre > 0.f)) ? 0.f : g[j];
+            float dz, dz_xhat;
+            bn_bwd_value(g[j], xv[j], res != nullptr, rv[j], sc[j], sf[j], mu[j], is[j], relu, dz, dz_xhat);
             dzv[j] = dz;
             out[j] = k1[j] * (dz - m1[j] - (xv[j] - mu[j]) * k2[j]);
         }
@@ -368,21 +366,25 @@
     return (size_t)c * ew_grid((long long)n * c / 4, c);
 }
 
-extern "C" int toda_rows_bn_bwd_res_colsum(const float* dy, const float* x, const float* residual, const float* stats,
-                                           const float* gamma, int n, int c, int relu, double* sums, float* dx, float* dres,
-                                           double* colsum_ws, float* dx_colsum, void* stream) {
-    hipStream_t s = (hipStream_t)stream;
+static int rows_bn_bwd_check(const double* colsum_ws, const float* dx_colsum, int c) {
     TODA_CHECK_ARG((colsum_ws == nullptr) == (dx_colsum == nullptr), "rows_bn_bwd: colsum workspace and result go together");
     TODA_CHECK_ARG(c >= 4 && c % 4 == 0 && c <= DN_BLOCK / 2 && DN_BLOCK % c == 0,
                    "rows_bn_bwd: channels must be a multiple of 4 dividing 256, <= 128 (got %d)", c);
+    return TODA_OK;
+}
+
+extern "C" int toda_rows_bn_bwd_apply(const float* dy, const float* x, const float* residual, const float* stats, const float* gamma,
+                                      int n, int c, int relu, double* sums, int blocks, float* dx, float* dres, double* colsum_ws,
+                                      float* dx_colsum, void* stream) {
+    hipStream_t s = (hipStream_t)stream;
+    const int rc = rows_bn_bwd_check(colsum_ws, dx_colsum, c);
+    if (rc != TODA_OK) return rc;
     if (n <= 0) {
         TODA_HIP(hipMemsetAsync(sums, 0, 3 * c * sizeof(double), s));
         if (dx_colsum) TODA_HIP(hipMemsetAsync(dx_colsum, 0, c * sizeof(float), s));
         return TODA_OK;
     }
-    int blocks, rpb;
-    reduce_plan(n, &blocks, &rpb);
-    hipLaunchKernelGGL(rows_bn_bwd_reduce_kernel, dim3(blocks), dim3(DN_BLOCK), 0, s, dy, x, residual, stats, n, c, relu, rpb, sums);
+    TODA_CHECK_ARG(blocks >= 1, "rows_bn_bwd_apply: partial sums per column must be >= 1 (got %d)", blocks);
     hipLaunchKernelGGL(fold_partials_kernel, dim3(2 * c), dim3(DN_BLOCK), 0, s, sums, blocks, 2 * c);
     const long long n4 = (long long)n * c / 4;
     const int grid = ew_grid(n4, c);
@@ -391,6 +393,20 @@
     if (dx_colsum) hipLaunchKernelGGL(colsum_fold_kernel, dim3(c), dim3(DN_BLOCK), 0, s, (const double*)colsum_ws, grid, dx_colsum);
     TODA_LAUNCH_CHECK();
     return TODA_OK;
+}
+
+extern "C" int toda_rows_bn_bwd_res_colsum(const float* dy, const float* x, const float* residual, const float* stats,
+                                           const float* gamma, int n, int c, int relu, double* sums, float* dx, float* dres,
+                                           double* colsum_ws, float* dx_colsum, void* stream) {
+    const int rc = rows_bn_bwd_check(colsum_ws, dx_colsum, c);
+    if (rc != TODA_OK) return rc;
+    int blocks = 1, rpb;
+    if (n > 0) {
+        reduce_plan(n, &blocks, &rpb);
+        hipLaunchKernelGGL(rows_bn_bwd_reduce_kernel, dim3(blocks), dim3(DN_BLOCK), 0, (hipStream_t)stream, dy, x, residual, stats, n, c, relu,
+                           rpb, sums);
+    }
+    return toda_rows_bn_bwd_apply(dy, x, residual, stats, gamma, n, c, relu, sums, blocks, dx, dres, colsum_ws, dx_colsum, stream);
 }
 
 extern "C" int toda_rows_bn_bwd_res(const float* dy, const float* x, const float* residual, const float* stats,
diff --git a/toda_amd/csrc/spconv.hip b/toda_amd/csrc/spconv.hip
--- a/toda_amd/csrc/spconv.hip
+++ b/toda_amd/csrc/spconv.hip
@@ -200,6 +200,61 @@
     }
 }
 
+struct BnBwdSrc {
+    const float* x;
+    const float* stats;
+    int relu;
+};
+
+template <int NT, int RT, int WAVES>
+__device__ __forceinline__ void gg_bn_bwd_sums(float (*st_sh)[2][16 * NT], int wv, int blk, const f32x4 (&acc)[RT][NT], const int (&rows)[RT],
+                                               int row0, int n_out, int cp, const BnBwdSrc& bn, double* stats, int r, int g) {
+    static_assert(NT == 2 || NT == 4, "32 or 64 produced channels (cp == 16 NT: whole vector loads of x)");
+    typedef float xvec __attribute__((ext_vector_type(NT)));
+    const xvec mu = *reinterpret_cast<const xvec*>(bn.stats + NT * r), is = *reinterpret_cast<const xvec*>(bn.stats + cp + NT * r),
+               sc = *reinterpret_cast<const xvec*>(bn.stats + 2 * cp + NT * r), sf = *reinterpret_cast<const xvec*>(bn.stats + 3 * cp + NT * r);
+    xvec xv[RT][4];
+#pragma unroll
+    for (int rt = 0; rt < RT; ++rt)
+#pragma unroll
+        for (int reg = 0; reg < 4; ++reg) {
+            const int row = __shfl(rows[rt], 4 * g + reg, 64);
+            xv[rt][reg] = *reinterpret_cast<const xvec*>(bn.x + (size_t)row * cp + NT * r);
+        }
+    float sm[NT], sq[NT];
+#pragma unroll
+    for (int n = 0; n < NT; ++n) {
+        sm[n] = sq[n] = 0.0f;
+#pragma unroll
+        for (int rt = 0; rt < RT; ++rt)
+#pragma unroll
+            for (int reg = 0; reg < 4; ++reg) {
+                float dz, dz_xhat;
+                bn_bwd_value(acc[rt][n][reg], xv[rt][reg][n], false, 0.f, sc[n], sf[n], mu[n], is[n], bn.relu, dz, dz_xhat);
+                if (row0 + rt * 16 + 4 * g + reg < n_out) {
+                    sm[n] += dz;
+                    sq[n] += dz_xhat;
+                }
+            }
+        sm[n] += __shfl_xor(sm[n], 16, 64);
+        sq[n] += __shfl_xor(sq[n], 16, 64);
+        sm[n] += __shfl_xor(sm[n], 32, 64);
+        sq[n] += __shfl_xor(sq[n], 32, 64);
+        if (g == 0) {
+            st_sh[wv][0][NT * r + n] = sm[n];
+            st_sh[wv][1][NT * r + n] = sq[n];
+        }
+    }
+    __syncthreads();
+    if ((int)threadIdx.x < 2 * cp) {
+        const int qq = threadIdx.x / cp, ch = threadIdx.x - qq * cp;
+        double a = 0.0;
+#pragma unroll
+        for (int w = 0; w < WAVES; ++w) a += (double)st_sh[w][qq][ch];
+        stats[2 * cp + (size_t)(qq * cp + ch) * gridDim.x + blk] = a;
+    }
+}
+
 __device__ __forceinline__ void wg_block(int K, int& chunk, int& k) {
     const int b = blockIdx.x;
     const int xcd = b & 7, t = (b >> 3) / K;
@@ -396,11 +451,11 @@
 #ifndef GG_LDS_WAVES
 #define GG_LDS_WAVES 4
 #endif
-template <int Q, int NT, int RT, bool VEC, bool DB = true, int BLK = SC_BLOCK, bool IDPF = false>
+template <int Q, int NT, int RT, bool VEC, bool DB = true, int BLK = SC_BLOCK, bool IDPF = false, class... BN>
 __global__ void __launch_bounds__(BLK, (Q * NT <= 4 && RT <= 2) ? GG_LDS_WAVES_NARROW : (Q * NT * RT <= 32 && Q * NT <= 16) ? GG_LDS_WAVES : (BLK > SC_BLOCK ? GG_LDS_WAVES_WIDE : 1))
 gather_gemm_lds_kernel(const float* __restrict__ in, int n_in, int cg, const float* __restrict__ wp,
                        const int* __restrict__ nbr, int n_out, int K, int cp, const float* __restrict__ bias,
-                       float* __restrict__ out, const int* __restrict__ order, double* __restrict__ stats) {
+                       float* __restrict__ out, const int* __restrict__ order, double* __restrict__ stats, const BN... bn) {
     constexpr int SLICE = Q * NT * 64;
     constexpr int PER_THREAD = (SLICE + BLK - 1) / BLK;
     __shared__ f32x4 wl[DB ? 2 : 1][SLICE];
@@ -497,7 +552,10 @@
 
     if (stats) {
         __shared__ float st_sh[BLK / 64][2][16 * NT];
-        gg_moments<NT, RT, BLK / 64>(st_sh, threadIdx.x >> 6, blk, acc, row0, n_out, cp, stats, r, g);
+        if constexpr (sizeof...(BN) == 1)
+            gg_bn_bwd_sums<NT, RT, BLK / 64>(st_sh, threadIdx.x >> 6, blk, acc, rows, row0, n_out, cp, bn..., stats, r, g);
+        else
+            gg_moments<NT, RT, BLK / 64>(st_sh, threadIdx.x >> 6, blk, acc, row0, n_out, cp, stats, r, g);
     }
     gg_store_rows<RT, NT>(acc, rows, row0, n_out, cp, out, r, g);
 }
@@ -1236,13 +1294,13 @@
 };
 }
 
-static int gather_route(int c_gather, int c_produce, int n_out, bool stats, bool cls_sorted, GatherRoute* r) {
+static int gather_route(int c_gather, int c_produce, int n_out, bool stats, bool cls_sorted, bool bnb, GatherRoute* r) {
     const int Q = tiles_pow2(c_gather), NT = tiles_pow2(c_produce);
     const bool vec_ok = (c_gather & 3) == 0;
     const bool lds_faster = Q >= 2 && NT >= Q;
     r->rt = 2, r->block = SC_BLOCK, r->vec = vec_ok;
     if (use_split(c_gather, c_produce)) {
-        TODA_CHECK_ARG(!(cls_sorted && stats), "gather_gemm (split path): no statistics on a class-sorted launch");
+        TODA_CHECK_ARG(!(cls_sorted && stats) || bnb, "gather_gemm (split path): no moments on a class-sorted launch");
         r->family = GatherRoute::SPLIT;
     } else if (vec_ok && Q == 8 && NT == 8 && !cls_sorted) {
         r->family = GatherRoute::LDS_128, r->rt = 1, r->block = 512;
@@ -1260,7 +1318,8 @@
 
 static int gather_gemm_impl(const float* in, int n_in, int c_gather, const float* wp, const int32_t* nbr, int n_out, int k_vol,
                             int c_produce, const float* bias, float* out, const int32_t* order, double* stats, int* blocks_out, void* stream,
-                            const unsigned char* cls_sorted = nullptr, const toda::GatherClasses* cls_table = nullptr) {
+                            const unsigned char* cls_sorted = nullptr, const toda::GatherClasses* cls_table = nullptr,
+                            const toda::BnBwdSrc* bnb = nullptr) {
     toda::GatherClasses classes = {};
     if (cls_sorted && cls_table) classes = *cls_table;
     else cls_sorted = nullptr;
@@ -1275,7 +1334,7 @@
         return TODA_OK;
     }
     GatherRoute r;
-    const int rc = gather_route(c_gather, c_produce, n_out, stats != nullptr, cls_sorted != nullptr, &r);
+    const int rc = gather_route(c_gather, c_produce, n_out, stats != nullptr, cls_sorted != nullptr, bnb != nullptr, &r);
     if (rc != TODA_OK) return rc;
     hipStream_t s = (hipStream_t)stream;
     const dim3 grid(r.grid), block(r.block);
@@ -1283,6 +1342,13 @@
         case GatherRoute::SPLIT:
             with_tiles(c_gather / 32, c_produce / 16, [&](auto kc, auto nt) {
                 constexpr int KC = decltype(kc)::value, NT = decltype(nt)::value;
+                if constexpr (KC <= 4 && NT >= 2 && NT <= 4) {
+                    if (bnb) {
+                        GG_LAUNCH(HIP_KERNEL_NAME(gg_split_kernel<KC, NT, 4, (NT == 2), toda::BnBwdSrc>), grid, block, 0, s, in, n_in,
+                                  reinterpret_cast<const toda::u32x4*>(wp), nbr, n_out, k_vol, c_produce, bias, out, order, stats, cls_sorted, classes, *bnb);
+                        return;
+                    }
+                }
                 if constexpr (KC <= 4 && NT >= 2)
                     GG_LAUNCH(HIP_KERNEL_NAME(gg_split_kernel<KC, NT, (NT == 8 ? 3 : 4), (NT == 2)>), grid, block, 0, s, in, n_in,
                               reinterpret_cast<const toda::u32x4*>(wp), nbr, n_out, k_vol, c_produce, bias, out, order, stats, cls_sorted, classes);
@@ -1295,6 +1361,13 @@
         case GatherRoute::LDS:
             with_tiles(tiles_pow2(c_gather), tiles_pow2(c_produce), [&](auto q, auto nt) {
                 constexpr int Q = decltype(q)::value, NT = decltype(nt)::value, RT = NT < 8 ? 2 : 1;
+                if constexpr (Q >= 2 && Q <= NT && NT <= 4) {
+                    if (bnb) {
+                        GG_LAUNCH(HIP_KERNEL_NAME(gather_gemm_lds_kernel<Q, NT, RT, true, true, SC_BLOCK, true, toda::BnBwdSrc>), grid, block, 0, s, in,
+                                  n_in, c_gather, wp, nbr, n_out, k_vol, c_produce, bias, out, order, stats, *bnb);
+                        return;
+                    }
+                }
                 GG_LAUNCH(HIP_KERNEL_NAME(gather_gemm_lds_kernel<Q, NT, RT, true, true, SC_BLOCK, (Q <= 4 && NT <= 4 && RT == 2)>), grid, block, 0,
                           s, in, n_in, c_gather, wp, nbr, n_out, k_vol, c_produce, bias, out, order, stats);
             });
@@ -1380,6 +1453,46 @@
     const int rc = gather_gemm_impl(in, n_in, c_gather, wp, nbr, n_out, k_vol, c_produce, bias, out, nullptr, sums, blocks_out, stream);
     if (rc == TODA_OK && *blocks_out <= 0) {
         set_error("gather_gemm_stats_partials: the launch took no statistics");
+        return TODA_EINVAL;
+    }
+    return rc;
+}
+
+static bool gg_bn_bwd_supported(int c_gather, int c_produce, bool classed) {
+    if (c_produce != 32 && c_produce != 64) return false;
+    if (classed) return (c_gather == 32 || c_gather == 64 || c_gather == 128) && use_split(c_gather, c_produce);
+    return (c_gather == 32 || c_gather == 64) && c_gather <= c_produce;
+}
+
+extern "C" int toda_spconv_gather_gemm_bn_bwd_supported(int c_gather, int c_produce, int classed) {
+    return gg_bn_bwd_supported(c_gather, c_produce, classed != 0) ? 1 : 0;
+}
+
+extern "C" int toda_spconv_gather_gemm_bn_bwd(const float* in, int n_in, int c_gather, const float* wp, const int32_t* nbr, int n_out, int k_vol,
+                                              int c_produce, float* out, const int32_t* order, const unsigned char* cls_sorted,
+                                              const int32_t* ksize, const int32_t* stride, const int32_t* padding, const float* x,
+                                              const float* bn_stats, int relu, double* sums, size_t sums_doubles, int* blocks_out, void* stream) {
+    TODA_CHECK_ARG(blocks_out != nullptr, "gather_gemm_bn_bwd: null argument");
+    *blocks_out = 0;
+    const bool classed = cls_sorted != nullptr;
+    TODA_CHECK_ARG(gg_bn_bwd_supported(c_gather, c_produce, classed), "gather_gemm_bn_bwd: unsupported channel pair (%d -> %d%s)", c_gather, c_produce,
+                   classed ? ", class-sorted, on this matrix path" : "");
+    TODA_CHECK_ARG(n_out >= 0 && n_in >= 0 && k_vol >= 1, "gather_gemm_bn_bwd: bad sizes");
+    if (n_out == 0) return TODA_OK;
+    TODA_CHECK_ARG(n_in > 0, "gather_gemm_bn_bwd: nothing to gather from");
+    TODA_CHECK_ARG(x != nullptr && bn_stats != nullptr && sums != nullptr, "gather_gemm_bn_bwd: null argument");
+    TODA_CHECK_ARG(sums_doubles >= toda_spconv_gather_gemm_stats_doubles(n_out, c_produce), "gather_gemm_bn_bwd: statistics buffer too small");
+    GatherClasses table;
+    if (classed) {
+        TODA_CHECK_ARG(order && ksize && stride && padding, "gather_gemm_bn_bwd: null argument of a class-sorted launch");
+        TODA_CHECK_ARG(ksize[0] * ksize[1] * ksize[2] == k_vol, "gather_gemm_bn_bwd: kernel size does not match the table's %d offsets", k_vol);
+        TODA_CHECK_ARG(class_table(ksize, stride, padding, &table) == 0, "gather_gemm_bn_bwd: needs <= 8 residue classes and <= 27 offsets");
+    }
+    const toda::BnBwdSrc bnb{x, bn_stats, relu};
+    const int rc = gather_gemm_impl(in, n_in, c_gather, wp, nbr, n_out, k_vol, c_produce, nullptr, out, order, sums, blocks_out, stream, cls_sorted,
+                                    classed ? &table : nullptr, &bnb);
+    if (rc == TODA_OK && *blocks_out <= 0) {
+        set_error("gather_gemm_bn_bwd: the launch took no sums");
         return TODA_EINVAL;
     }
     return rc;
diff --git a/toda_amd/csrc/spconv_split.cuh b/toda_amd/csrc/spconv_split.cuh
--- a/toda_amd/csrc/spconv_split.cuh
+++ b/toda_amd/csrc/spconv_split.cuh
@@ -104,11 +104,11 @@
                          (unsigned)v[6] | ((unsigned)v[7] << 16)};
 }
 
-template <int KC, int NT, int WAVES, bool IL = false>
+template <int KC, int NT, int WAVES, bool IL = false, class... BN>
 __global__ void __launch_bounds__(SC_BLOCK, WAVES)
 gg_split_kernel(const float* __restrict__ in, int n_in, const u32x4* __restrict__ wps, const int* __restrict__ nbr, int n_out, int K, int cp,
                 const float* __restrict__ bias, float* __restrict__ out, const int* __restrict__ order, double* __restrict__ stats,
-                const unsigned char* __restrict__ cls_sorted, const GatherClasses classes) {
+                const unsigned char* __restrict__ cls_sorted, const GatherClasses classes, const BN... bn) {
     constexpr int RT = 2;
     constexpr int CG = 32 * KC;
     constexpr int UNITS = NT * 3;
@@ -290,7 +290,11 @@
         stats = nullptr;
     }
 #endif
-    if (stats) gg_moments<NT, RT, SC_BLOCK / 64>(reinterpret_cast<float (*)[2][16 * NT]>(wl), wv, blk, acc, row0, n_out, cp, stats, r, g);
+    if (stats) {
+        float (*st_sh)[2][16 * NT] = reinterpret_cast<float (*)[2][16 * NT]>(wl);
+        if constexpr (sizeof...(BN) == 1) gg_bn_bwd_sums<NT, RT, SC_BLOCK / 64>(st_sh, wv, blk, acc, rows, row0, n_out, cp, bn..., stats, r, g);
+        else gg_moments<NT, RT, SC_BLOCK / 64>(st_sh, wv, blk, acc, row0, n_out, cp, stats, r, g);
+    }
     gg_store_rows<RT, NT>(acc, rows, row0, n_out, cp, out, r, g);
 }
 
diff --git a/toda_amd/lib.py b/toda_amd/lib.py
--- a/toda_amd/lib.py
+++ b/toda_amd/lib.py
@@ -48,6 +48,8 @@
     "toda_spconv_gather_gemm_stats_doubles": (_sz, [_i, _i]),
     "toda_spconv_gather_gemm_stats": (_i, [_vp, _i, _i, _vp, _vp, _i, _i, _i, _vp, _vp, _vp, _sz, _vp]),
     "toda_spconv_gather_gemm_stats_partials": (_i, [_vp, _i, _i, _vp, _vp, _i, _i, _i, _vp, _vp, _vp, _sz, _vp, _vp]),
+    "toda_spconv_gather_gemm_bn_bwd_supported": (_i, [_i, _i, _i]),
+    "toda_spconv_gather_gemm_bn_bwd": (_i, [_vp, _i, _i, _vp, _vp, _i, _i, _i, _vp, _vp, _vp, _vp, _vp, _vp, _vp, _vp, _i, _vp, _sz, _vp, _vp]),
     "toda_spconv_gather_gemm_compact_supported": (_i, [_i, _i, _i]),
     "toda_spconv_gather_gemm_compact": (_i, [_vp, _i, _i, _vp, _i, _i, _i, _i, _vp, _i, _i, _i, _vp, _vp, _vp]),
     "toda_spconv_gather_gemm_compact_stats_doubles": (_sz, [_i, _i]),
@@ -67,6 +69,7 @@
     "toda_rows_bn_bwd_res": (_i, [_vp, _vp, _vp, _vp, _vp, _i, _i, _i, _vp, _vp, _vp, _vp]),
     "toda_rows_bn_bwd_colsum_doubles": (_sz, [_i, _i]),
     "toda_rows_bn_bwd_res_colsum": (_i, [_vp, _vp, _vp, _vp, _vp, _i, _i, _i, _vp, _vp, _vp, _vp, _vp, _vp]),
+    "toda_rows_bn_bwd_apply": (_i, [_vp, _vp, _vp, _vp, _vp, _i, _i, _i, _vp, _i, _vp, _vp, _vp, _vp, _vp]),
     "toda_conv3x3s2_supported": (_i, [_i, _i, _i, _i, _i]),
     "toda_conv3x3s2_fwd": (_i, [_vp, _vp, _i, _i, _i, _i, _i, _vp, _vp]),
     "toda_conv3x3s2_dgrad": (_i, [_vp, _vp, _i, _i, _i, _i, _i, _vp, _vp]),
diff --git a/toda_amd/ops.py b/toda_amd/ops.py
--- a/toda_amd/ops.py
+++ b/toda_amd/ops.py
@@ -647,12 +647,21 @@
     return bool(L.load().toda_spconv_gather_gemm_stats_supported(int(c_gather), int(c_produce)))
 
 
-def gather_gemm_with_stats(feat, wp, nbr, c_produce, bias=None, partials=False):
+def gather_gemm_with_stats(feat, wp, nbr, c_produce, bias=None, partials=False, bn_bwd=None, order=None):
     lib = L.load()
     K, n_out = nbr.shape
     out = torch.empty((n_out, c_produce), dtype=torch.float32, device=feat.device)
     nd = lib.toda_spconv_gather_gemm_stats_doubles(n_out, c_produce)
     sums = torch.empty((nd,), dtype=torch.float64, device=feat.device)
+    if bn_bwd is not None:
+        import ctypes
+        x, stats, relu = bn_bwd
+        blocks = ctypes.c_int(0)
+        rc = lib.toda_spconv_gather_gemm_bn_bwd(L.ptr(feat), feat.shape[0], feat.shape[1], L.ptr(wp), L.ptr(nbr), n_out, K, c_produce, L.ptr(out),
+                                                L.ptr(order), None, None, None, None, L.ptr(x), L.ptr(stats), int(bool(relu)), L.ptr(sums), nd,
+                                                ctypes.addressof(blocks), L.stream())
+        L.check(rc, "toda_spconv_gather_gemm_bn_bwd")
+        return out, sums, int(blocks.value)
     if partials:
         import ctypes
         blocks = ctypes.c_int(0)
@@ -664,6 +673,10 @@
                                            L.ptr(bias), L.ptr(out), L.ptr(sums), nd, L.stream())
     L.check(rc, "toda_spconv_gather_gemm_stats")
     return out, sums
+
+
+def gather_gemm_bn_bwd_supported(c_gather, c_produce, classed=False):
+    return bool(L.load().toda_spconv_gather_gemm_bn_bwd_supported(int(c_gather), int(c_produce), int(bool(classed))))
 
 
 def gather_gemm(feat, wp, nbr, c_produce, bias=None, order=None):
@@ -728,11 +741,22 @@
     return out
 
 
-def gather_gemm_classed(feat, wp, nbr, c_produce, order, cls_sorted, ksize, stride, padding):
+def gather_gemm_classed(feat, wp, nbr, c_produce, order, cls_sorted, ksize, stride, padding, bn_bwd=None):
     lib = L.load()
     K, n_out = nbr.shape
     out = torch.empty((n_out, c_produce), dtype=torch.float32, device=feat.device)
     ks, st, pd = L.host_i32(ksize), L.host_i32(stride), L.host_i32(padding)
+    if bn_bwd is not None:
+        import ctypes
+        x, stats, relu = bn_bwd
+        nd = lib.toda_spconv_gather_gemm_stats_doubles(n_out, c_produce)
+        sums = torch.empty((nd,), dtype=torch.float64, device=feat.device)
+        blocks = ctypes.c_int(0)
+        rc = lib.toda_spconv_gather_gemm_bn_bwd(L.ptr(feat), feat.shape[0], feat.shape[1], L.ptr(wp), L.ptr(nbr), n_out, K, c_produce, L.ptr(out),
+                                                L.ptr(order), L.ptr(cls_sorted), L.hptr(ks), L.hptr(st), L.hptr(pd), L.ptr(x), L.ptr(stats),
+                                                int(bool(relu)), L.ptr(sums), nd, ctypes.addressof(blocks), L.stream())
+        L.check(rc, "toda_spconv_gather_gemm_bn_bwd")
+        return out, sums, int(blocks.value)
     rc = lib.toda_spconv_gather_gemm_classed(L.ptr(feat), feat.shape[0], feat.shape[1], L.ptr(wp), L.ptr(nbr), n_out, K, c_produce, None,
                                              L.ptr(out), L.ptr(order), L.ptr(cls_sorted), L.hptr(ks), L.hptr(st), L.hptr(pd), L.stream())
     L.check(rc, "toda_spconv_gather_gemm_classed")
@@ -759,6 +783,7 @@
 
     @staticmethod
     def forward(ctx, features, weight, bias, rb, wp_fwd, want_stats=False, wp_bwd=None):
+        ctx.bn_src = getattr(features, "_toda_bn_src", None) if BN_BWD_FROM_DGRAD else None
         features = features.contiguous()
         compact = _compact_route(features.shape[1], weight.shape[0], rb.nbr_fwd)
         if wp_fwd is None and not compact:
@@ -798,7 +823,16 @@
             wp_t = ctx.wp_bwd if ctx.wp_bwd is not None else pack_weight(weight, True, rb.flip_bwd)
             _check_mm(wp_t)
             co = rb.class_order()
-            if co is not None:
+            src = ctx.bn_src
+            if (src is not None and BN_BWD_FROM_DGRAD and gout.shape[0] > 0 and src[0].shape == (rb.nbr_bwd.shape[1], weight.shape[-1])
+                    and gather_gemm_bn_bwd_supported(gout.shape[1], weight.shape[-1], co is not None)):
+                if co is not None:
+                    gfeat, part, blocks = gather_gemm_classed(gout, wp_t, rb.nbr_bwd, weight.shape[-1], co[0], co[1], rb.ksize, rb.geom["stride"],
+                                                              rb.geom["padding"], src)
+                else:
+                    gfeat, part, blocks = gather_gemm_with_stats(gout, wp_t, rb.nbr_bwd, weight.shape[-1], None, bn_bwd=src)
+                _BN_BWD_SUMS[gfeat.data_ptr()] = (gfeat, gfeat._version, part, blocks, src)
+            elif co is not None:
                 gfeat = gather_gemm_classed(gout, wp_t, rb.nbr_bwd, weight.shape[-1], co[0], co[1], rb.ksize, rb.geom["stride"], rb.geom["padding"])
             else:
                 gfeat = gather_gemm(gout, wp_t, rb.nbr_bwd, weight.shape[-1], None)
@@ -901,6 +935,20 @@
 BN_BWD_COLSUM = True
 
 
+_BN_BWD_SUMS = {}
+BN_BWD_FROM_DGRAD = True
+
+
+def _take_bn_bwd_sums(gy, x, stats, relu):
+    ent = _BN_BWD_SUMS.pop(gy.data_ptr(), None) if _BN_BWD_SUMS else None
+    if ent is None or ent[0].shape != gy.shape or ent[0]._version != ent[1] or gy.stride() != ent[0].stride():
+        return None
+    src = ent[4]
+    if src[0].data_ptr() != x.data_ptr() or src[0].shape != x.shape or src[1].data_ptr() != stats.data_ptr() or bool(src[2]) != bool(relu):
+        return None
+    return ent[2], ent[3]
+
+
 def _take_colsum(gout):
     ent = _DX_COLSUM.pop(gout.data_ptr(), None) if _DX_COLSUM else None
     if ent is None or ent[0].shape != gout.shape or ent[0]._version != ent[2] or gout.stride() != ent[0].stride():
@@ -915,6 +963,8 @@
         lib = L.load()
         if _DX_COLSUM:
             _DX_COLSUM.clear()
+        if _BN_BWD_SUMS:
+            _BN_BWD_SUMS.clear()
         ctx.colsum = bool(colsum) and BN_BWD_COLSUM
         x = x.contiguous()
         residual = residual.contiguous() if residual is not None else None
@@ -937,6 +987,8 @@
         L.check(rc, "toda_rows_affine_act")
         ctx.save_for_backward(x, stats, weight, residual)
         ctx.meta = (n, c, bool(relu), bool(training))
+        if BN_BWD_FROM_DGRAD and training and residual is None and c in (32, 64) and n > 0:
+            y._toda_bn_src = (x, stats, bool(relu))
         return y
 
     @staticmethod
@@ -965,14 +1017,26 @@
             gx = dz * stats[2]
             xhat = (x - stats[0]) * stats[1]
             return gx, (dz * xhat).sum(0), dz.sum(0), None, None, None, None, None, None, (dz if want_res else None), None, None
-        sums = torch.empty((L.load().toda_rows_reduce_doubles(n, c),), dtype=torch.float64, device=x.device)
+        lib = L.load()
+        taken = _take_bn_bwd_sums(gy, x, stats, relu) if residual is None else None
         gx = torch.empty_like(x)
         gamma = weight if weight is not None else torch.ones(c, device=x.device)
         gres = torch.empty_like(x) if want_res else None
+        cs_ws = cs = None
         if ctx.colsum:
-            lib = L.load()
             cs_ws = torch.empty((lib.toda_rows_bn_bwd_colsum_doubles(n, c),), dtype=torch.float64, device=x.device)
             cs = torch.empty((c,), dtype=torch.float32, device=x.device)
+        if taken is not None:
+            sums, blocks = taken
+            rc = lib.toda_rows_bn_bwd_apply(L.ptr(gy), L.ptr(x), None, L.ptr(stats), L.ptr(gamma), n, c, int(relu), L.ptr(sums), int(blocks),
+                                            L.ptr(gx), None, L.ptr(cs_ws), L.ptr(cs), L.stream())
+            L.check(rc, "toda_rows_bn_bwd_apply")
+            if ctx.colsum:
+                _DX_COLSUM[gx.data_ptr()] = (gx, cs, gx._version)
+            gs = sums[2 * c:3 * c].view(torch.float32)
+            return gx, gs[c:], gs[:c], None, None, None, None, None, None, None, None, None
+        sums = torch.empty((lib.toda_rows_reduce_doubles(n, c),), dtype=torch.float64, device=x.device)
+        if ctx.colsum:
             rc = lib.toda_rows_bn_bwd_res_colsum(L.ptr(gy), L.ptr(x), L.ptr(residual), L.ptr(stats), L.ptr(gamma), n, c, int(relu),
                                                  L.ptr(sums), L.ptr(gx), L.ptr(gres), L.ptr(cs_ws), L.ptr(cs), L.stream())
             L.check(rc, "toda_rows_bn_bwd_res_colsum")
```

Result: no change. 150.7, median of 6 (+0.7%).
